# jasperlinthorst/reveal

Measured on AMD Instinct MI355X. Metric: Mbp/s indexed+MUM-anchored (reveal rem), higher is better.
Workload: dtype int32

## Files before the change

include/reveal_amd.h:

```cpp
#ifndef REVEAL_AMD_H
#define REVEAL_AMD_H
#include <stdint.h>

#ifdef __cplusplus
extern "C" {
#endif

typedef struct rv_index rv_index;

const char *rv_last_error(void);
int  rv_abi_version(void);
int  rv_sa_bits(void);
int  rv_device_count(void);

rv_index *rv_new(int device);
void rv_free(rv_index *h);

int rv_add_sample(rv_index *h);
int rv_add_sequence(rv_index *h, const char *seq, int64_t len, int64_t *begin, int64_t *end);
int rv_reset(rv_index *h);
int rv_reserve_text(rv_index *h, int64_t bytes);
int64_t rv_n(const rv_index *h);
int rv_nsamples(const rv_index *h);
int rv_nnodes(const rv_index *h);
// ... 32 lines not shown
int rv_sub_nodes(rv_index *h, int s, int64_t *begin_end );
int rv_sub_mums(rv_index *h, int s, uint32_t *l, int32_t *n, int64_t *off, uint16_t *so, int64_t *pos);
int64_t rv_sub_array(rv_index *h, int s, int which, void *out, int64_t cap);
int rv_sub_split(rv_index *h, int s, uint32_t l, int nsp, const int64_t *sp,
                 const int64_t *lead, int nlead, const int64_t *trail, int ntrail,
                 const int64_t *match, int nmatch, const int64_t *rest, int nrest);
int rv_frontier_commit(rv_index *h, int32_t *children);
int rv_align_end(rv_index *h);

typedef struct {
    int64_t steps;
    int64_t splits;
    int64_t anchored_bp;
    int32_t levels;
    int32_t maxdepth;
    int64_t scanned_ranks;
    double  t_scan, t_host, t_split, t_bubble;
} rv_align_stats;
int rv_align_builtin(rv_index *h, int minl, int minn, rv_align_stats *st);

int rv_align_builtin_until(rv_index *h, int minl, int minn, int stop_subs, rv_align_stats *st);
int rv_align_builtin_resume(rv_index *h, rv_align_stats *st);
int rv_align_builtin_continue(rv_index *h, int stop_subs, rv_align_stats *st);
int rv_frontier_counts(rv_index *h, int64_t *out);
int rv_frontier_export(rv_index *h, int64_t *meta, int64_t *node_first, int64_t *nodes);
int64_t rv_frontier_pack(rv_index *h, const int32_t *subs, int k, void *sa, void *lcp, void *bwt, int on_device);
int rv_frontier_import(rv_index *h, int minl, int minn, uint32_t maxlcp, int level, int nsubs, const int64_t *meta,
                       const int64_t *node_first, const int64_t *nodes, int64_t m,
                       const void *sa, const void *lcp, const void *bwt, int on_device);
int64_t rv_frontier_seeds_export(rv_index *h, const int32_t *subs, int k, int64_t *out, int64_t cap);
int rv_frontier_seeds_import(rv_index *h, int nsubs, const int64_t *words, int64_t nwords);
uint32_t rv_maxlcp(const rv_index *h);
int rv_cascade_info(const rv_index *h, int64_t *out);
const char *rv_cascade_why(const rv_index *h);
int64_t rv_anchor_count(rv_index *h, int64_t *members);
int rv_fetch_anchors(rv_index *h, uint32_t *l, int64_t *off, int64_t *pos);
int rv_set_result_buffers(rv_index *h, uint32_t *l, int64_t l_cap, int64_t *off, int64_t off_cap, int64_t *pos, int64_t pos_cap);
typedef struct {
    int64_t  key, n;
    int32_t  depth, nsamples, nnodes, picked;
    int64_t  nmums;
    uint32_t l; int32_t mn;
    int64_t  sp_min;
    uint64_t h_sa, h_lcp, h_mums;
} rv_trace;
int rv_set_trace(rv_index *h, int on);
int rv_set_preselect(rv_index *h, int64_t maxmums);
int rv_set_option(rv_index *h, const char *name, int64_t value);
int rv_get_option(rv_index *h, const char *name, int64_t *value);
int rv_set_launch_trace(int on);
int rv_option_count(void);
const char *rv_option_name(int k);
int64_t rv_trace_count(rv_index *h);
int rv_fetch_trace(rv_index *h, rv_trace *out, int64_t cap);

typedef struct rv_subindex rv_subindex;
rv_index *rv_clone(rv_index *h);
rv_subindex *rv_sx_main(rv_index *h);
rv_subindex *rv_sx_copy(rv_subindex *x);
void rv_sx_free(rv_subindex *x);
int rv_sx_info(const rv_subindex *x, rv_sub *out);
int rv_sx_nodes(const rv_subindex *x, int64_t *begin_end);
int64_t rv_sx_array(rv_subindex *x, int which, void *out, int64_t cap);
int64_t rv_sx_scan(rv_subindex *x, int minl, int minn, int64_t *members);
int rv_sx_fetch(rv_subindex *x, uint32_t *l, int32_t *n, int64_t *off, uint16_t *so, int64_t *pos);
int rv_sx_split(rv_subindex *x, const int64_t *lead, int nlead, const int64_t *trail, int ntrail,
// ... 103 lines not shown
```

reveal_amd/_index.py:

```python
import ctypes
import mmap
import os
import sys
import numpy as np

from . import _lib
from ._lib import RV_T, RV_SA, RV_SAI, RV_LCP, RV_SO, RV_NSEP


def _page_array(count, dtype):
    nbytes = max(int(count), 1) * np.dtype(dtype).itemsize
    m = mmap.mmap(-1, (nbytes + mmap.PAGESIZE - 1) // mmap.PAGESIZE * mmap.PAGESIZE)
    return np.frombuffer(m, dtype=dtype, count=max(int(count), 1))


def _pairs(iv, sa64):
    a = np.ascontiguousarray(np.array([(int(b), int(e)) for b, e in iv], dtype=np.int64).reshape(-1, 2))
    return a, len(a)


_OPTION_DEFAULTS = {}


def make_index_type(sa64, error):
# ... 544 lines not shown
            na = dll.rv_anchor_count(h, ctypes.byref(mem))
            c = self._result_buffers_free()
            if c is not None and len(c[0]) >= max(na, 1) and len(c[1]) >= na + 1 and len(c[2]) >= max(mem.value, 1):
                l, off, pos = c
            else:
                dll.rv_set_result_buffers(h, None, 0, None, 0, None, 0)
                if os.environ.get("RV_RESULT_BUFS", "") == "heap":
                    l = np.empty(max(na, 1), dtype=np.uint32); off = np.empty(na + 1, dtype=np.int64); pos = np.empty(max(mem.value, 1), dtype=np.int64)
                else:
                    l = _page_array(max(na, 1), np.uint32); off = _page_array(na + 1, np.int64); pos = _page_array(max(mem.value, 1), np.int64)
                self.__dict__["_res_bufs"] = (l, off, pos)
            c = None
            off[0] = 0
            if dll.rv_fetch_anchors(h, l.ctypes.data, off.ctypes.data, pos.ctypes.data) != 0:
                self._fail()
            tr = None
            if trace:
                nt = dll.rv_trace_count(h)
                tr = np.zeros(max(nt, 1), dtype=_lib.TRACE_DTYPE)
                if dll.rv_fetch_trace(h, tr.ctypes.data, len(tr)) != 0:
                    self._fail()
                tr = tr[:nt]
            stats = {f[0]: getattr(st, f[0]) for f in _lib.RvAlignStats._fields_}
            return dict(stats=stats, anchors=(l[:na], off[:na + 1], pos[:mem.value]), trace=tr)

        @property
        def maxlcp(self):
            return int(self._dll.rv_maxlcp(self._h))

        def cascade_info(self):
            o = np.zeros(8, dtype=np.int64)
            self._dll.rv_cascade_info(self._h, o.ctypes.data)
            return dict(done=bool(o[0]), levels=int(o[1]), matches=int(o[2]), witnesses=int(o[3]), subindices=int(o[4]), undecided=int(o[5]), rebuilt_ranks=int(o[6]), decided_from_witnesses=int(o[7]),
                        why=(self._dll.rv_cascade_why(self._h) or b"").decode())

        def align_builtin_until(self, stop_subs, minl=20, minn=2, trace=False):
            if not self._constructed:
                raise error("Index not yet constructed, alignment stopped.")
            self._dll.rv_set_trace(self._h, 1 if trace else 0)
            self._offer_result_buffers()
            self._st = _lib.RvAlignStats()
            self._trace = bool(trace)
            r = self._dll.rv_align_builtin_until(self._h, int(minl), int(minn), int(stop_subs), ctypes.byref(self._st))
            if r < 0:
                self._fail()
            self._pending = r > 0
            return r

        def align_builtin_continue(self, stop_subs):
            if not getattr(self, "_pending", False):
                return 0
            self._offer_result_buffers()
            r = self._dll.rv_align_builtin_continue(self._h, int(stop_subs), ctypes.byref(self._st))
            if r < 0:
                self._fail()
            self._pending = r > 0
            return r

        def frontier(self):
            c = np.zeros(4, dtype=np.int64)
            if self._dll.rv_frontier_counts(self._h, c.ctypes.data) != 0:
                self._fail()
            ns, m, nn, level = (int(x) for x in c)
            meta = np.zeros((max(ns, 1), 6), dtype=np.int64); nf = np.zeros(ns + 1, dtype=np.int64); nodes = np.zeros((max(nn, 1), 2), dtype=np.int64)
            if self._dll.rv_frontier_export(self._h, meta.ctypes.data, nf.ctypes.data, nodes.ctypes.data) != 0:
                self._fail()
# ... 89 lines not shown
```

reveal_amd/_lib.py:

```python
import ctypes
import importlib.util
import os
import sys
import numpy as np

_HERE = os.path.dirname(os.path.abspath(__file__))

RV_T, RV_SA, RV_SAI, RV_LCP, RV_SO, RV_NSEP, RV_NODES = range(7)
K_SCAN_PAIR, K_SCAN_MULTI, K_SA_SORT, K_LCP, K_SPLIT, K_LABEL, K_BUBBLE, K_RADIX_SCATTER, K_RADIX_HIST, K_TEXT_ROUND, K_CASCADE, K_DIAG_TABLE, K_INIT_KEYS, K_PUBLISH = range(14)

c_i64p = ctypes.POINTER(ctypes.c_int64)
V = ctypes.c_void_p


class RvSub(ctypes.Structure):
    _fields_ = [("n", ctypes.c_int64), ("depth", ctypes.c_int32), ("nsamples", ctypes.c_int32),
                ("nnodes", ctypes.c_int32), ("parent", ctypes.c_int32), ("kind", ctypes.c_int32),
                ("reserved", ctypes.c_int32), ("nmums", ctypes.c_int64), ("nmembers", ctypes.c_int64)]


class RvAlignStats(ctypes.Structure):
    _fields_ = [("steps", ctypes.c_int64), ("splits", ctypes.c_int64), ("anchored_bp", ctypes.c_int64),
                ("levels", ctypes.c_int32), ("maxdepth", ctypes.c_int32), ("scanned_ranks", ctypes.c_int64),
                ("t_scan", ctypes.c_double), ("t_host", ctypes.c_double), ("t_split", ctypes.c_double),
# ... 23 lines not shown
    "rv_node_list": (_I, [V, V]),
    "rv_construct": (_I, [V, _I, ctypes.c_char_p, ctypes.c_char_p, _I]),
    "rv_upload": (_I, [V]),
    "rv_upload_again": (_I, [V]),
    "rv_get_array": (_L, [V, _I, V, _L]),
    "rv_getmums": (_L, [V, _I]),
    "rv_fetch_mums": (_I, [V, V, V, V, _L]),
    "rv_getmultimums": (_L, [V, _I, _I, _I, c_i64p]),
    "rv_fetch_multi": (_I, [V, V, V, V, V, V]),
    "rv_align_begin": (_I, [V, _I, _I]),
    "rv_frontier_size": (_I, [V]),
    "rv_frontier_scan": (_I, [V]),
    "rv_sub_skip_scan": (_I, [V, _I]),
    "rv_sub_info": (_I, [V, _I, ctypes.POINTER(RvSub)]),
    "rv_sub_nodes": (_I, [V, _I, V]),
    "rv_sub_mums": (_I, [V, _I, V, V, V, V, V]),
    "rv_sub_array": (_L, [V, _I, _I, V, _L]),
    "rv_sub_split": (_I, [V, _I, ctypes.c_uint32, _I, V, V, _I, V, _I, V, _I, V, _I]),
    "rv_frontier_commit": (_I, [V, V]),
    "rv_align_end": (_I, [V]),
    "rv_align_builtin": (_I, [V, _I, _I, ctypes.POINTER(RvAlignStats)]),
    "rv_align_builtin_until": (_I, [V, _I, _I, _I, ctypes.POINTER(RvAlignStats)]),
    "rv_align_builtin_resume": (_I, [V, ctypes.POINTER(RvAlignStats)]),
    "rv_align_builtin_continue": (_I, [V, _I, ctypes.POINTER(RvAlignStats)]),
    "rv_frontier_counts": (_I, [V, V]),
    "rv_frontier_export": (_I, [V, V, V, V]),
    "rv_frontier_pack": (_L, [V, V, _I, V, V, V, _I]),
    "rv_frontier_import": (_I, [V, _I, _I, ctypes.c_uint32, _I, _I, V, V, V, _L, V, V, V, _I]),
    "rv_frontier_seeds_export": (_L, [V, V, _I, V, _L]),
    "rv_frontier_seeds_import": (_I, [V, _I, V, _L]),
    "rv_maxlcp": (ctypes.c_uint32, [V]),
    "rv_cascade_info": (ctypes.c_int, [V, V]),
    "rv_cascade_why": (ctypes.c_char_p, [V]),
    "rv_anchor_count": (_L, [V, c_i64p]),
    "rv_fetch_anchors": (_I, [V, V, V, V]),
    "rv_set_result_buffers": (_I, [V, V, _L, V, _L, V, _L]),
    "rv_set_trace": (_I, [V, _I]),
    "rv_set_preselect": (_I, [V, _L]),
    "rv_set_option": (_I, [V, ctypes.c_char_p, _L]),
    "rv_set_launch_trace": (_I, [_I]),
    "rv_batch_new": (V, []),
    "rv_batch_add": (_I, [V, V]),
    "rv_batch_run": (_I, [V, _I, _I, _I, V, V]),
    "rv_batch_info": (_I, [V, V]),
    "rv_batch_free": (None, [V]),
    "rv_dev_alloc": (V, [_I, _L]),
    "rv_dev_free": (_I, [_I, V]),
    "rv_ipc_export": (_I, [_I, V, V]),
    "rv_ipc_open": (V, [_I, V]),
    "rv_ipc_close": (_I, [_I, V]),
    "rv_dev_copy": (_I, [_I, V, V, _L]),
    "rv_get_option": (_I, [V, ctypes.c_char_p, c_i64p]),
    "rv_option_count": (_I, []),
    "rv_option_name": (ctypes.c_char_p, [_I]),
    "rv_trace_count": (_L, [V]),
    "rv_fetch_trace": (_I, [V, V, _L]),
    "rv_clone": (V, [V]),
    "rv_sx_main": (V, [V]),
    "rv_sx_copy": (V, [V]),
    "rv_sx_free": (None, [V]),
    "rv_sx_info": (_I, [V, ctypes.POINTER(RvSub)]),
    "rv_sx_nodes": (_I, [V, V]),
    "rv_sx_array": (_L, [V, _I, V, _L]),
    "rv_sx_scan": (_L, [V, _I, _I, c_i64p]),
    "rv_sx_fetch": (_I, [V, V, V, V, V, V]),
    "rv_sx_split": (_I, [V, V, _I, V, _I, V, _I, V, _I, V]),
# ... 124 lines not shown
```

reveal_amd/csrc/rv_align.hip:

```cpp
#include "rv_index.h"
#include "rv_split.h"
#include "rv_decide.h"
static_assert(RV_TSUB_TILE == RV_SPLIT_TILE, "one tile -> sub-index table serves the split passes and the multi-sample picker");
#include "rv_leaf.h"
#include "rv_cascade.h"
#include <string.h>
#include <algorithm>
#include <chrono>
#include <thread>
#include <atomic>
#include "rv_graphrem.h"

namespace {

double now_s() {
    return std::chrono::duration<double>(std::chrono::steady_clock::now().time_since_epoch()).count();
}

u64 hash_step(u64 acc, u64 i, int64_t v) {
    u64 x = (u64)v + (i + 1) * 0x9E3779B97F4A7C15ULL;
    x ^= x >> 30; x *= 0xbf58476d1ce4e5b9ULL;
    x ^= x >> 27; x *= 0x94d049bb133111ebULL;
    x ^= x >> 31;
    return acc + x;
// ... 84 lines not shown
    Level lv, nx;
    Decisions dec;
    bool scanned = false;
    std::vector<uint8_t> skip_scan;
    bool full_only = false;
    const u32 *d_err = nullptr;
    std::vector<RvPairRec> recs;
    std::vector<u32> ml; std::vector<int32_t> mn; std::vector<int64_t> moff, mpos; std::vector<uint16_t> mso;
    std::vector<int64_t> mum_first, nmums;
    int picker = 0; rv_picker_args pargs{};
    struct SeedList {
        std::vector<u32> l; std::vector<int32_t> n; std::vector<int64_t> off; std::vector<uint16_t> so; std::vector<int64_t> pos, score;
        size_t size() const { return l.size(); }
        void clear() { l.clear(); n.clear(); off.assign(1, 0); so.clear(); pos.clear(); score.clear(); }
        void push(u32 l_, int32_t n_, const uint16_t *so_, const int64_t *pos_, int members, int64_t sc) {
            if (off.empty()) off.assign(1, 0);
            l.push_back(l_); n.push_back(n_); score.push_back(sc);
            so.insert(so.end(), so_, so_ + members); pos.insert(pos.end(), pos_, pos_ + members); off.push_back((int64_t)pos.size());
        }
    };
    std::vector<SeedList> seeds_cur, seeds_lead, seeds_trail;
    rv_graph *ggraph = nullptr;
    rv_graph *replay_graph = nullptr; RvReplayFeed *feed = nullptr; size_t fed = 0;
    std::vector<RvGraphIv> g_left, g_right, g_newleft, g_newright;
    RvGraphAlignOut g_out;
    int64_t picker_calls = 0, picker_seeded = 0, picker_ns = 0, picker_list_ns = 0, galign_ns = 0;
    int64_t presel = 0; bool presel_on = false;
    bool pick_filter = false;
    int64_t presel_d2h = 0;
    std::vector<int64_t> sel, sel_first, sel_tmp;
    DBuf dD, dTab, dTile, dList, dFlag, dPar, dDbg, scrSA, scrLCP, scrBWT;
    RvCascadeBufs cas;
    RvCascadeOut cas_out{};
    DBuf dPbReady; u32 pb_epoch = 0;
    DBuf dNextTsub;
    DBuf dTmin;
    HBuf hLeafRoots[2], hLeafOut;
    DBuf dLeaf, dLeafRoots[2];
    hipStream_t leaf_stream = nullptr, leaf_stream2 = nullptr;
    hipStream_t bub_stream = nullptr, bub_stream2 = nullptr;
    hipEvent_t ev_fork = nullptr, ev_join = nullptr, ev_join2 = nullptr;
    hipEvent_t ev_ready = nullptr, ev_leaf[RV_LEVEL_BUFS + 1] = {}, ev_roots[2] = {nullptr, nullptr};
    bool roots_inflight[2] = {false, false};
    bool flag_clean = false;
    DBuf dDec, dErr, dTab0;
    bool next_dev_ok = false, cur_dev_ok = false, early_done = false, early_bubble = false, use_leaf = false;
    int64_t par_min_cur = RV_BUBBLE_PAR_N;
    const sa_t *d_next_nodes = nullptr; const uint8_t *d_next_flags = nullptr;
    std::vector<sa_t> next_nodes; std::vector<uint8_t> next_flags;
    bool leaf_pending[RV_LEVEL_BUFS + 1] = {};
    size_t leaf_anchor_cap = 0, leaf_trace_cap = 0;
    std::vector<uint8_t> leaf_done;
    std::vector<RvLeafRoot> leaf_roots[2];
    Packer pk;
    std::vector<int> stamp; int epoch = 0;
    std::vector<sa_t> cb, ce, mb, me, cut_lo, cut_hi, mend_pos;
    std::vector<uint8_t> cc;
    std::vector<int> ctab_first, mtab_first, cut_first, mend_first, split_subs;
    std::vector<u32> sub_off_h;
    std::vector<int> tile_sub;
    std::vector<int64_t> mpre, sub_start, woff, toff, next_ss;
    const int64_t *d_next_ss = nullptr;
    const int *d_next_want = nullptr;
    const int *d_next_tsub = nullptr;
    std::vector<int> next_tsub;
    std::vector<u32> pick_l; std::vector<sa_t> pick_pos;
// ... 391 lines not shown
        d.child_n = t.child_n; d.child_base = t.child_base; d.sub_off = t.sub_off; d.expect_total = t.expect_total;
        d.err = a->dErr.as<u32>();
        d.kid = kid;
    };
    if (a->multi) {
        RvDecideMultiArgs d;
        outputs(d);
        d.W = W; d.minl = a->minl; d.minn = a->minn;
        d.nodes = a->d_next_nodes; d.want = a->d_next_want;
        d.pick_l = h->ws.misc[13].as<u32>(); d.pick_pos = h->ws.misc[7].as<sa_t>();
        d.cand_count = h->ws.misc[1].as<u32>() + RV_MULTI_REGIONS * 64;
        d.cand_cap = (u32)std::min<size_t>(h->ws.misc[8].cap / RV_MULTI_CAND_BYTES / RV_MULTI_REGIONS, 0xffffffffu);
        RV_TRY(rv_decide_multi_launch(h->ws, d));
    } else {
        RvDecideArgs d;
        outputs(d);
        d.nodes = a->d_next_nodes; d.flags = a->d_next_flags; d.picks = h->hscan.as<RvPairRec>();
        d.ovf_cap = (u32)std::min<size_t>(h->ws.misc[4].cap / sizeof(RvPairRec), 0xffffffffu);
        RV_TRY(rv_decide_launch(h->ws, d));
    }
    RvLabelTabs lt; RvSplitArgs sa;
    split_args(h, t, nxt, lt, sa);
    int64_t biggest = 0;
    for (int s2 = 0; s2 < ns; s2++) biggest = std::max<int64_t>(biggest, lv.n[(size_t)s2]);
    if (biggest > a->par_min_cur) RV_TRY(tmin_preset(h, sa));
    int id = h->prof.begin(q, RV_K_SPLIT, (double)m * (2 * (sizeof(sa_t) + sizeof(lcp_t) + 2)) + (double)m * (sizeof(sa_t) + sizeof(lcp_t) + 1));
    RV_TRY(rv_split_launch(h->ws, cur_sa(h), cur_lcp(h), a->dD.as<uint8_t>(), cur_bwt(h), m, lt, sa, 1));
    h->prof.end(q, id);
    a->early_done = true;
    a->early_bubble = false;
    const bool all_classes = a->multi || ns > 4096;
    if (biggest <= a->par_min_cur && !h->ws.opt.no_early_bubble &&
        (a->multi || (!h->ws.opt.bubble_lds_always && (!all_classes || h->ws.opt.early_bubble_many)))) {
        RV_TRY(rv_lower_ranges_launch(h->ws, h->dT.as<uint8_t>(), t.mb, t.me, W * ns));
        RV_TRY(bubble_flags(h, m));
        RvBubbleArgs ba;
        memset(&ba, 0, sizeof ba);
        ba.flag = a->dFlag.as<uint8_t>();
        ba.SA = sa.SA_out; ba.LCP = sa.LCP_out; ba.BWT = sa.BWT_out; ba.SAi = sa.SAi; ba.cut_lo = t.cut_lo; ba.cut_hi = t.cut_hi; ba.err = a->dErr.as<u32>();
        id = h->prof.begin(q, RV_K_BUBBLE, 0.0);
        if (!all_classes) {
            RV_TRY(rv_bubble_children_dev_launch(h->ws, ba, kid, ns, a->par_min_cur));
        } else {
            RV_TRY(bubble_fork(h, true, true, true));
            Workspace wl, wk; wl.stream = a->bub_stream; wk.stream = a->bub_stream2;
            RV_TRY(rv_bubble_children_dev_classes_launch(wl, wk, ba, kid, ns, a->par_min_cur));
            RV_TRY(bubble_join(h, true, true));
        }
        h->prof.end(q, id);
        a->early_bubble = true;
    }
    return 0;
}

static int level_hook(rv_index *h) {
    Align *a = h->al;
    if (a->hook_early) RV_TRY(early_split(h));
    if (a->leaf_launch_due) RV_TRY(leaf_launch(h));
    return 0;
}

static void build_preselection(Align *a) {
    const int ns = a->lv.size();
    a->sel.clear(); a->sel_first.assign((size_t)ns + 1, 0);
    std::vector<int64_t> &tmp = a->sel_tmp;
    for (int s = 0; s < ns; s++) {
// ... 589 lines not shown
        a->d_next_tsub = a->dNextTsub.as<int>();
    }
    return 0;
}

static int commit_split(rv_index *h, const Commit &cm, RvSplitArgs &sa) {
    Align *a = h->al;
    hipStream_t q = h->ws.stream;
    const Level &lv = a->lv;
    const int nxt = cm.nxt;
    uint8_t *tb = a->dTab.as<uint8_t>();
    RV_TRY(split_reserve(h, nxt, lv.m, cm.m_next));
    RV_TRY(a->dList.reserve((size_t)a->woff.back() * 4 + 64));
    RV_TRY(leaf_wait(h, nxt));
    if (h->ws.opt.bubble_parent_scratch && !a->descs.empty()) RV_TRY(leaf_wait(h, a->level == 0 ? RV_LEVEL_BUFS : a->cur));
    SplitTabs t;
    t.sub_start = (const int64_t *)(tb + cm.o_ss); t.tile_sub = (const int *)(tb + cm.o_tsub);
    t.ctab_first = (int *)(tb + cm.o_ctf); t.mtab_first = (int *)(tb + cm.o_mtf); t.cut_first = (int *)(tb + cm.o_cf); t.mend_first = (int *)(tb + cm.o_mf);
    t.cb = (sa_t *)(tb + cm.o_cb); t.ce = (sa_t *)(tb + cm.o_ce); t.cc = tb + cm.o_cc; t.mb = (sa_t *)(tb + cm.o_mb); t.me = (sa_t *)(tb + cm.o_me);
    t.cut_lo = (sa_t *)(tb + cm.o_clo); t.cut_hi = (sa_t *)(tb + cm.o_chi); t.mend_pos = (sa_t *)(tb + cm.o_mp);
    t.child_n = (u32 *)(tb + cm.o_cn); t.child_base = (u32 *)(tb + cm.o_cbase); t.sub_off = (u32 *)(tb + cm.o_suboff); t.expect_total = (u32 *)(tb + cm.o_expect);
    t.total = (u32 *)(tb + cm.o_total);
    t.nmatch = (int)a->mb.size();
    RvLabelTabs lt;
    split_args(h, t, nxt, lt, sa);
    sa.mend_all = a->dec.host_lists ? 1 : 0;
    int id = a->early_done ? -1 : h->prof.begin(q, RV_K_SPLIT, (double)lv.m * (2 * (sizeof(sa_t) + sizeof(lcp_t) + 2)) + (double)cm.m_next * (sizeof(sa_t) + sizeof(lcp_t) + 1));
    if (!a->early_done) {
        if (!a->descs.empty()) RV_TRY(tmin_preset(h, sa));
        RV_TRY(rv_split_launch(h->ws, cur_sa(h), cur_lcp(h), a->dD.as<uint8_t>(), cur_bwt(h), lv.m, lt, sa, (int)a->split_subs.size()));
    }
    h->prof.end(q, id);
    if (!a->early_bubble) {
        if (lt.nmatch > 256 && a->mpre.back() / lt.nmatch <= 512) RV_TRY(rv_lower_ranges_launch(h->ws, h->dT.as<uint8_t>(), lt.mbegin, lt.mend, lt.nmatch));
        else RV_TRY(rv_lower_launch(h->ws, h->dT.as<uint8_t>(), lt.mbegin, lt.mend, (const int64_t *)(tb + cm.o_mpre), lt.nmatch, a->mpre.back()));
    }
    return 0;
}

static int commit_bubble(rv_index *h, const Commit &cm, const RvSplitArgs &sa) {
    Align *a = h->al;
    hipStream_t q = h->ws.stream;
    uint8_t *tb = a->dTab.as<uint8_t>();
    const int64_t m_next = cm.m_next;
    if (a->descs.empty() && a->kids_small.empty() && a->kids_big.empty() && a->kids_lds.empty()) return 0;
    RvBubbleArgs ba;
    ba.desc = (const RvBubbleDesc *)(tb + cm.o_desc); ba.woff = (const int64_t *)(tb + cm.o_woff);
    ba.cnt = (u32 *)(tb + cm.o_bcnt); ba.list = a->dList.as<u32>();
    RV_TRY(bubble_flags(h, m_next));
    ba.flag = a->dFlag.as<uint8_t>();
    ba.SA = sa.SA_out; ba.LCP = sa.LCP_out; ba.BWT = sa.BWT_out; ba.SAi = sa.SAi; ba.cut_lo = sa.cut_lo; ba.cut_hi = sa.cut_hi; ba.err = sa.err;
    ba.state = (RvBubbleState *)(tb + cm.o_bstate);
    ba.dbg = nullptr;
    if (h->ws.opt.level_log) { if (!a->dDbg.p) { RV_TRY(a->dDbg.reserve(64)); RV_HIP(hipMemsetAsync(a->dDbg.p, 0, 64, q)); } ba.dbg = a->dDbg.as<unsigned long long>(); }
    ba.scrSA = const_cast<sa_t *>(cur_sa(h)); ba.scrLCP = const_cast<lcp_t *>(cur_lcp(h)); ba.scrBWT = const_cast<uint8_t *>(cur_bwt(h));
    if (!a->descs.empty() && !h->ws.opt.bubble_parent_scratch) {
        RV_TRY(a->scrSA.reserve((size_t)(m_next + 64) * sizeof(sa_t)));
        RV_TRY(a->scrLCP.reserve((size_t)(m_next + 64) * sizeof(lcp_t)));
        RV_TRY(a->scrBWT.reserve((size_t)m_next + 64));
        ba.scrSA = a->scrSA.as<sa_t>(); ba.scrLCP = a->scrLCP.as<lcp_t>(); ba.scrBWT = a->scrBWT.as<uint8_t>();
    }
    if (!a->descs.empty()) {
        const size_t W = (size_t)a->woff.back() + 16, TT = (size_t)a->toff.back() + 16;
        RV_TRY(a->dPar.reserve(TT * 4 + W * (8 + 7 * 4 + sizeof(sa_t) + 2) + 256));
        uint8_t *pb = a->dPar.as<uint8_t>();
        ba.par.toff = (const int64_t *)(tb + cm.o_toff);
// ... 498 lines not shown
    }
    RV_HIP(hipStreamSynchronize(q));
    if (a->lv.size() > 0) {
        u32 err = 0;
        RV_HIP(hipMemcpy(&err, a->dErr.p, 4, hipMemcpyDeviceToHost));
        if (err & 1u) { rv_set_error("split: the intervals returned by graphalign do not partition the sub-index (child size mismatch)"); return -1; }
        if (err) { rv_set_error("device-side error %u in the level before the hand-off", err); return -1; }
    }
    return 0;
}

static void fill_offsets(int64_t *off, size_t na, int64_t base) {
    const int nt = na > ((size_t)1 << 18) ? 4 : 1;
    std::vector<std::thread> th;
    for (int t = 1; t < nt; t++) {
        const size_t lo = na / nt * t, hi = t + 1 == nt ? na : na / nt * (t + 1);
        th.emplace_back([=]() { for (size_t k = lo; k < hi; k++) off[k] = base + 2 * (int64_t)(k + 1); });
    }
    for (size_t k = 0; k < na / nt; k++) off[k] = base + 2 * (int64_t)(k + 1);
    for (auto &x : th) x.join();
}
static int builtin_finish(rv_index *h, rv_align_stats *out) {
    Align *a = h->al;
    hipStream_t q = h->ws.stream;
    h->rb.direct = false;
    if (a->use_leaf && a->running) {
        u32 *lf_counters = a->lf_counters; u32 *lf_l = a->lf_l; int64_t *lf_pos = a->lf_pos; rv_trace *lf_tr = a->lf_tr;
        RV_HIP(hipStreamSynchronize(a->leaf_stream));
        RV_HIP(hipStreamSynchronize(a->leaf_stream2));
        for (int k = 0; k <= RV_LEVEL_BUFS; k++) a->leaf_pending[k] = false;
        RV_TRY(a->hLeafOut.reserve(256));
        RV_HIP(hipMemcpyAsync(a->hLeafOut.p, lf_counters, 128, hipMemcpyDeviceToHost, q));
        RV_HIP(hipStreamSynchronize(q));
        u32 cnt[4]; unsigned long long stv[8];
        memcpy(cnt, a->hLeafOut.p, sizeof cnt); memcpy(stv, a->hLeafOut.as<uint8_t>() + 64, sizeof stv);
        if (h->ws.opt.leaf_prof)
            fprintf(stderr, "leaf: steps %llu splits %llu | cycles idle %llu scan %llu split %llu bubble %llu\n", stv[0], stv[1], stv[4], stv[5], stv[6], stv[7]);
        if (cnt[2]) { rv_set_error(cnt[2] & 4u ? "leaf kernel: recursion stack overflow" : "leaf kernel: a sub-index does not match its intervals"); return -1; }
        if (cnt[0] > a->leaf_anchor_cap || cnt[1] > a->leaf_trace_cap) { rv_set_error("leaf kernel: output buffer too small"); return -1; }
        a->leaf_na = 0;
        if (cnt[0]) {
            const size_t na = cnt[0];
            const size_t nl = a->an_l.size(), np = a->an_pos.size();
            rv_index::ResultBufs &rb = h->rb;
            rb.direct = rb.l && (int64_t)(nl + na) <= rb.l_cap && (int64_t)(nl + na + 1) <= rb.off_cap && (int64_t)(np + 2 * na) <= rb.pos_cap;
            int64_t *pp; u32 *pl;
            if (rb.direct) { pp = rb.pos + np; pl = rb.l + nl; }
            else { RV_TRY(a->hLeafOut.reserve(na * 20 + 64)); pp = a->hLeafOut.as<int64_t>(); pl = (u32 *)(pp + 2 * na); }
            RV_HIP(hipMemcpyAsync(pp, lf_pos, na * 16, hipMemcpyDeviceToHost, a->leaf_stream));
            RV_HIP(hipMemcpyAsync(pl, lf_l, na * 4, hipMemcpyDeviceToHost, a->leaf_stream));
            RV_TRY(rv_leaf_lower_launch(h->ws, h->dT.as<uint8_t>(), lf_pos, lf_l, (u32)na));
            if (rb.direct) fill_offsets(rb.off + nl + 1, na, (int64_t)np);
            RV_HIP(hipStreamSynchronize(a->leaf_stream));
            RV_HIP(hipStreamSynchronize(q));
            a->leaf_na = na;
        }
        if (a->trace_on && cnt[1]) {
            const size_t at = a->trace.size();
            a->trace.resize(at + cnt[1]);
            RV_HIP(hipMemcpy(a->trace.data() + at, lf_tr, (size_t)cnt[1] * sizeof(rv_trace), hipMemcpyDeviceToHost));
        }
        a->st.steps += (int64_t)stv[0]; a->st.splits += (int64_t)stv[1]; a->st.anchored_bp += (int64_t)stv[2];
        if ((int64_t)stv[3] > a->st.maxdepth) a->st.maxdepth = (int32_t)stv[3];
    }
    a->running = false;
    if (out) *out = a->st;
    return 0;
}

static int install_frontier(rv_index *h, int level, int nsubs, const int64_t *meta, const int64_t *node_first, const int64_t *nodes, int64_t m,
                            const void *sa, const void *lcp, const void *bwt, int on_device);
static int builtin_cascade(rv_index *h) {
    Align *a = h->al;
    memset(&a->cas_out, 0, sizeof a->cas_out);
    if (a->trace_on || h->rc != 0 || h->n <= RV_LEAF_N || a->minl < 4 || h->ws.opt.no_cascade || a->picker != 0) return 0;
    const bool second_try = !a->multi && a->use_leaf && h->ws.opt.cascade_second == 2;
    auto interval_cascade = [&]() -> int {
        RvCascadeMultiOut mo;
        RV_TRY(rv_cascade_multi_run(h, a->cas, a->minl, &mo));
        a->cas_out.done = mo.done; a->cas_out.levels = mo.levels; a->cas_out.cands = mo.cands; a->cas_out.witnesses = mo.witnesses; a->cas_out.children = mo.children;
        a->cas_out.undecided = mo.undecided; a->cas_out.rebuilt_ranks = mo.rebuilt_ranks; a->cas_out.why = mo.why;
        if (!mo.done) return 0;
        const int k = h->nsamples;
        a->st.splits += (int64_t)mo.an_l.size(); a->st.steps += mo.steps; a->st.levels += mo.levels; a->st.scanned_ranks += h->n;
        if (mo.maxdepth > a->st.maxdepth) a->st.maxdepth = mo.maxdepth;
        h->main_arrays_freed = true;
        if (mo.undecided > 0) {
            RV_TRY(install_frontier(h, 1, (int)mo.undecided, mo.meta.data(), mo.node_first.data(), mo.nodes.data(), mo.rebuilt_ranks, mo.d_sa, mo.d_lcp, mo.d_bwt, 1));
        } else {
            a->lv.clear();
            a->level = 1;
        }
        {
            const size_t na = mo.an_l.size(), l0 = a->an_l.size(), p0 = a->an_pos.size(), o0 = a->an_off.size();
            a->an_l.insert(a->an_l.end(), mo.an_l.begin(), mo.an_l.end());
            a->an_pos.resize(p0 + na * (size_t)k);
            for (size_t x = 0; x < na * (size_t)k; x++) a->an_pos[p0 + x] = (int64_t)mo.an_pos[x];
            a->an_off.resize(o0 + na);
            for (size_t x = 0; x < na; x++) a->an_off[o0 + x] = (int64_t)(p0 + (x + 1) * (size_t)k);
            int64_t bp = 0;
            for (size_t x = 0; x < na; x++) bp += mo.an_l[x];
            a->st.anchored_bp += bp;
            (void)l0;
        }
        return 0;
    };
    if (a->multi || second_try) return interval_cascade();
    if (!a->use_leaf) return 0;
    RvCascadeIO io;
    io.anchor_count = a->lf_counters; io.anchor_cap = (u32)a->leaf_anchor_cap; io.anchor_l = a->lf_l; io.anchor_pos = a->lf_pos;
    io.stats = a->lf_stats; io.leaf_err = a->lf_counters + 2;
    io.stage_cap = (u32)h->ws.opt.leaf_acap;
    io.lvSA = &a->lvSA[0]; io.lvLCP = &a->lvLCP[0]; io.lvBWT = &a->lvBWT[0]; io.roots = &a->dLeafRoots[0];
    const int dmode = (int)h->ws.opt.cascade_danger;
    RV_TRY(rv_cascade_run(h, a->cas, io, a->minl, &a->cas_out, dmode == 2 ? 1 : 0, 0));
    if (!a->cas_out.done && a->cas_out.undecided > 0 && dmode == 1) {
        RV_HIP(hipMemsetAsync(a->dLeaf.p, 0, 256, h->ws.stream));
        RV_TRY(rv_cascade_run(h, a->cas, io, a->minl, &a->cas_out, 1, 1));
    }
    if (!a->cas_out.done) {
        RV_HIP(hipMemsetAsync(a->dLeaf.p, 0, 256, h->ws.stream));
        if (a->cas_out.undecided > 0 && !h->ws.opt.cascade_second_off) return interval_cascade();
        return 0;
    }
    a->st.levels += a->cas_out.levels;
    a->st.scanned_ranks += h->n;
    if (!a->cas.lin_rest.empty() && h->nodes.size() > 2) {
        std::vector<RvIntv> rest, gone;
        for (size_t k = 0; k + 1 < a->cas.lin_rest.size(); k += 2) rest.push_back({a->cas.lin_rest[k], a->cas.lin_rest[k + 1]});
        std::sort(rest.begin(), rest.end(), intv_less);
        for (const RvIntv &v : h->nodes) {
            if (v.end <= v.begin) continue;
            const auto it = std::lower_bound(rest.begin(), rest.end(), v, intv_less);
            if (it == rest.end() || it->begin != v.begin) gone.push_back(v);
        }
        RV_TRY(add_decision(h, 0, 0, nullptr, 0, gone.data(), (int)gone.size(), nullptr, 0, nullptr, 0, rest.data(), (int)rest.size()));
        a->dec.drop_lead = true;
        RV_TRY(rv_frontier_commit(h, nullptr));
        for (size_t s2 = 0; s2 < a->lv.depth.size(); s2++) a->lv.depth[s2] = a->cas.lin_rest_depth;
        return 0;
    }
    h->main_arrays_freed = true;
    a->level = 1;
    a->lv.clear();
    return 0;
}

int rv_cascade_info(const rv_index *h, int64_t *out) {
    for (int k = 0; k < 8; k++) out[k] = 0;
    if (!h->al) return 0;
    const RvCascadeOut &c = h->al->cas_out;
    out[0] = c.done ? 1 : 0; out[1] = c.levels; out[2] = c.cands; out[3] = c.witnesses; out[4] = c.children; out[5] = c.undecided; out[6] = c.rebuilt_ranks; out[7] = c.solved;
    return 0;
}

const char *rv_cascade_why(const rv_index *h) {
    if (!h->al || h->al->cas_out.done || !h->al->cas_out.why) return "";
    return h->al->cas_out.why;
}

int rv_align_builtin(rv_index *h, int minl, int minn, rv_align_stats *out) {
    RV_TRY(builtin_setup(h, minl, minn));
    Align *a = h->al;
    if (a->replay_graph && a->picker == 1) {
        a->feed = rv_replay_feed_start(a->replay_graph);
        a->fed = 0;
        a->replay_graph = nullptr;
        if (!a->feed) return -1;
    }
    int rc = builtin_cascade(h);
    if (rc == 0) rc = builtin_levels(h, 0);
    if (rc == 0) rc = builtin_finish(h, out);
    if (a->feed) {
        RvReplayFeed *f = a->feed; a->feed = nullptr;
        if (rc == 0) { if (rv_replay_feed_finish(f) != 0) return -1; }
        else { const std::string keep = rv_last_error(); (void)rv_replay_feed_finish(f); rv_set_error("%s", keep.c_str()); }
    }
    return rc;
}

int rv_align_builtin_until(rv_index *h, int minl, int minn, int stop_subs, rv_align_stats *out) {
    RV_TRY(builtin_setup(h, minl, minn));
    RV_TRY(builtin_cascade(h));
    RV_TRY(builtin_levels(h, stop_subs));
    Align *a = h->al;
    if (a->lv.size() == 0) { RV_TRY(builtin_finish(h, out)); return 0; }
    if (out) *out = a->st;
// ... 552 lines not shown
```

reveal_amd/csrc/rv_api.hip:

```cpp
#include "rv_index.h"
#include "rv_cascade.h"
#include <limits>
#include <stdarg.h>
#include <stdio.h>
#include <string.h>
#include <limits.h>
#include <algorithm>
#include <thread>

static thread_local char g_err[1024] = "";

void rv_set_error(const char *fmt, ...) {
    va_list ap;
    va_start(ap, fmt);
    vsnprintf(g_err, sizeof g_err, fmt, ap);
    va_end(ap);
}

static std::vector<rv_index *> &live_handles() { static std::vector<rv_index *> v; return v; }
std::mutex &rv_trim_mutex() { static std::mutex *m = new std::mutex(); return *m; }
bool rv_oom_trim() {
    size_t got = 0;
    bool log = false;
    int caller_dev = 0;
// ... 34 lines not shown
    if (nd <= 0) { rv_set_error("no HIP device visible: reveal_amd has no CPU fallback"); return nullptr; }
    if (device < 0 || device >= nd) { rv_set_error("device %d out of range (%d visible)", device, nd); return nullptr; }
    if (hipSetDevice(device) != hipSuccess) { rv_set_error("hipSetDevice(%d) failed", device); return nullptr; }
    hipDeviceProp_t prop;
    if (hipGetDeviceProperties(&prop, device) != hipSuccess) { rv_set_error("hipGetDeviceProperties failed"); return nullptr; }
    if (strncmp(prop.gcnArchName, "gfx950", 6) != 0) {
        rv_set_error("device %d is %s; this library is built for gfx950 (MI355X) only", device, prop.gcnArchName);
        return nullptr;
    }
    rv_index *h = new rv_index();
    h->device = device;
    if (rv_stream_get(&h->ws.stream) != hipSuccess) {
        rv_set_error("hipStreamCreate failed");
        delete h;
        return nullptr;
    }
    h->T.push_back('\0');
    h->ws.prof_ctx = &h->prof;
    h->ws.prof_begin_fn = [](void *c, hipStream_t st, int k, double b) { return ((RvProf *)c)->begin(st, k, b); };
    h->ws.prof_end_fn = [](void *c, hipStream_t st, int id) { ((RvProf *)c)->end(st, id); };
    { std::lock_guard<std::mutex> g(rv_trim_mutex()); live_handles().push_back(h); }
    return h;
}

void rv_free(rv_index *h) {
    if (!h) return;
    { std::lock_guard<std::mutex> g(rv_trim_mutex()); auto &v = live_handles(); v.erase(std::remove(v.begin(), v.end(), h), v.end()); }
    (void)hipSetDevice(h->device);
    if (h->ws.stream) (void)hipStreamSynchronize(h->ws.stream);
    h->rb.direct = false;
    (void)rv_set_result_buffers(h, nullptr, 0, nullptr, 0, nullptr, 0);
    rv_align_free(h);
    h->prof.release();
    h->dT.release(); h->dT0.release(); h->dSA.release(); h->dSAi.release(); h->dLCP.release(); h->dBWT.release(); h->dNsep.release();
    h->ws.release();
    h->hscan.release();
    for (auto &b : h->ps) b.release();
    h->hupload.release();
    if (h->ev_picks) { (void)hipEventDestroy(h->ev_picks); h->ev_picks = nullptr; }
    if (h->ws.stream) rv_stream_put(h->ws.stream);
    delete h;
}

int rv_set_option(rv_index *h, const char *name, int64_t value) {
    if (!h || !name) { rv_set_error("rv_set_option: null argument"); return -1; }
    int64_t *f = h->ws.opt.find(name);
    if (!f) { rv_set_error("rv_set_option: unknown option %s", name); return -1; }
    *f = value;
    return 0;
}
int rv_set_launch_trace(int on) {
    const int was = g_rv_launch_trace;
    g_rv_launch_trace = on != 0;
    return was;
}
int rv_get_option(rv_index *h, const char *name, int64_t *value) {
    if (!h || !name || !value) { rv_set_error("rv_get_option: null argument"); return -1; }
    const int64_t *f = h->ws.opt.find(name);
    if (!f) { rv_set_error("rv_get_option: unknown option %s", name); return -1; }
    *value = *f;
    return 0;
}
int rv_option_count(void) {
    int c = 0;
#define RV_X_(f, nm, def) c++;
    RV_OPTION_LIST(RV_X_)
#undef RV_X_
    return c;
}
const char *rv_option_name(int k) {
    static const char *const names[] = {
#define RV_X_(f, nm, def) nm,
        RV_OPTION_LIST(RV_X_)
#undef RV_X_
    };
    return k >= 0 && k < rv_option_count() ? names[k] : nullptr;
}

rv_index *rv_clone(rv_index *h) {
    if (!h->constructed || h->main_arrays_freed) { rv_set_error("Index not yet constructed."); return nullptr; }
    if (rv_need_sai(h)) return nullptr;
    rv_index *c = rv_new(h->device);
    if (!c) return nullptr;
    try { c->T = h->T; c->nsep = h->nsep; c->nodes = h->nodes; }
    catch (...) { rv_set_error("copy of the index: out of host memory"); rv_free(c); return nullptr; }
    if (c->T.size() != h->T.size()) { rv_free(c); return nullptr; }
    c->nsamples = h->nsamples; c->n = h->n; c->nT = h->nT; c->rc = h->rc;
    c->maxlcp = h->maxlcp; c->sa_stats = h->sa_stats; c->text_dirty = true;
    c->ws.opt = h->ws.opt;
    const int64_t n = h->n;
    hipStream_t q = c->ws.stream;
    bool ok = rv_upload(c) == 0;
    ok = ok && c->dT.reserve((size_t)n + 64) == 0 && c->dSA.reserve((size_t)(n + 64) * sizeof(sa_t)) == 0 && c->dSAi.reserve((size_t)(n + 64) * sizeof(sa_t)) == 0
            && c->dLCP.reserve((size_t)(n + 64) * sizeof(lcp_t)) == 0 && c->dBWT.reserve((size_t)n + 64) == 0 && c->dNsep.reserve((h->nsep.size() + 1) * sizeof(sa_t)) == 0;
    ok = ok && hipStreamSynchronize(h->ws.stream) == hipSuccess;
    ok = ok && hipMemcpyAsync(c->dT.p, h->dT.p, (size_t)n + 64, hipMemcpyDeviceToDevice, q) == hipSuccess;
    ok = ok && hipMemcpyAsync(c->dSA.p, h->dSA.p, (size_t)n * sizeof(sa_t), hipMemcpyDeviceToDevice, q) == hipSuccess;
    ok = ok && hipMemcpyAsync(c->dSAi.p, h->dSAi.p, (size_t)n * sizeof(sa_t), hipMemcpyDeviceToDevice, q) == hipSuccess;
    ok = ok && hipMemcpyAsync(c->dLCP.p, h->dLCP.p, (size_t)n * sizeof(lcp_t), hipMemcpyDeviceToDevice, q) == hipSuccess;
    ok = ok && hipMemcpyAsync(c->dBWT.p, h->dBWT.p, (size_t)n, hipMemcpyDeviceToDevice, q) == hipSuccess;
    ok = ok && hipMemcpyAsync(c->dNsep.p, h->dNsep.p, (h->nsep.size() + 1) * sizeof(sa_t), hipMemcpyDeviceToDevice, q) == hipSuccess;
    ok = ok && hipStreamSynchronize(q) == hipSuccess;
    if (!ok) { rv_set_error("copy of the index failed"); rv_free(c); return nullptr; }
    c->nsep_dev = h->nsep_dev;
    c->constructed = true; c->sai_valid = true;
    return c;
}

int rv_add_sample(rv_index *h) {
    if (h->nsamples > 0) h->nsep.push_back(h->n - 1);
    h->nsamples++;
    h->constructed = false; h->text_only = false;
    return 0;
}

int rv_add_sequence(rv_index *h, const char *seq, int64_t len, int64_t *begin, int64_t *end) {
    if (len < 0 || !seq) { rv_set_error("addsequence: bad sequence"); return -1; }
#ifndef RV_SA64
    if ((uint64_t)h->n + (uint64_t)(len + 1) + 1 > (uint64_t)INT_MAX) {
        rv_set_error("Total amount of sequence too large, use \"reveal <subcommand> --64\" to use 64 bit suffix arrays instead.");
        return -1;
    }
#endif
    const int64_t s = h->n;
    if ((size_t)(h->n + len + 2) > h->T.cap) (void)hipSetDevice(h->device);
    if (h->T.resize((size_t)(h->n + len + 2)) != 0) return -1;
    char *dst = h->T.data() + h->n;
    auto copy_check = [dst, seq](int64_t lo, int64_t hi) -> uint64_t {
        uint64_t acc = 0;
// ... 196 lines not shown
            used[slot] = true;
        }
        RV_HIP(hipStreamSynchronize(q));
    }
    RV_HIP(hipStreamSynchronize(q));
    h->text_dirty = false;
    return 0;
}

int rv_upload_again(rv_index *h) {
    h->text_dirty = true;
    return rv_upload(h);
}

int rv_construct(rv_index *h, int rc, const char *safile, const char *lcpfile, int cache) {
    RV_HIP(hipSetDevice(h->device));
    if (rc == 1) {
        if (h->nsep.empty()) { rv_set_error("construct(rc=1) needs at least two samples"); return -1; }
        h->rc = 1;
        revcomp(h->T.data() + h->nsep[0], h->n - h->nsep[0]);
        h->text_dirty = true;
    } else {
        h->rc = 0;
    }
    if (h->n == 0) { rv_set_error("No text to index."); return -1; }
    const int64_t n = h->n;
    if (n >= ((int64_t)1 << 32) - 2) { rv_set_error("index of %lld positions: this build carries ranks in 32 bits (n < 2^32 - 2)", (long long)n); return -1; }
    if (cache == 1) RV_TRY(write_raw(".reveal.t", h->T.data(), (size_t)n));
    if (h->al) (void)rv_align_end(h);
    h->nT = n;
    hipStream_t q = h->ws.stream;
    RV_TRY(rv_upload(h));
    RV_TRY(h->dT.reserve((size_t)n + 64));
    RV_HIP(hipMemcpyAsync(h->dT.p, h->dT0.p, (size_t)n + 64, hipMemcpyDeviceToDevice, q));
    RV_TRY(h->dSA.reserve((size_t)(n + 64) * sizeof(sa_t)));
    RV_TRY(h->dSAi.reserve((size_t)(n + 64) * sizeof(sa_t)));
    RV_TRY(h->dLCP.reserve((size_t)(n + 64) * sizeof(lcp_t)));
    RV_TRY(h->dBWT.reserve((size_t)n + 64));
    memset(&h->sa_stats, 0, sizeof h->sa_stats);
    RV_TRY(h->ws.misc[0].reserve(64));
    u32 *d_max = h->ws.misc[0].as<u32>();
    const sa_t side_sep = !h->nsep.empty() ? (sa_t)h->nsep[0] : std::numeric_limits<sa_t>::max();
    const bool lcp_from_file = lcpfile && lcpfile[0];
    bool lcp_done = false;
    SaScratchInUse in_use(h->ws);
    if (!safile || !safile[0]) {
        int id = h->prof.begin(q, RV_K_SA_SORT, 5.0 * (double)n);
        if (lcp_from_file) RV_TRY(rv_build_sa(h->ws, h->dT.as<uint8_t>(), n, h->dSA.as<sa_t>(), &h->sa_stats));
        else RV_TRY(rv_build_sa(h->ws, h->dT.as<uint8_t>(), n, h->dSA.as<sa_t>(), &h->sa_stats, h->dLCP.as<lcp_t>(), h->dBWT.as<uint8_t>(), side_sep, d_max, &lcp_done,
                                 h->nsep.data(), (int)h->nsep.size()));
        h->prof.end(q, id);
    } else {
        std::vector<sa_t> tmp((size_t)n);
        RV_TRY(read_raw(safile, tmp.data(), (size_t)n * sizeof(sa_t)));
        RV_HIP(hipMemcpyAsync(h->dSA.p, tmp.data(), (size_t)n * sizeof(sa_t), hipMemcpyHostToDevice, q));
        RV_HIP(hipStreamSynchronize(q));
    }
    h->sai_valid = false;
    if (safile && safile[0]) { RV_TRY(rv_build_inverse_checked(h->ws, h->dSA.as<sa_t>(), h->dSAi.as<sa_t>(), n)); h->sai_valid = true; }
    if (!lcp_from_file) {
        if (!lcp_done) {
            int id = h->prof.begin(q, RV_K_LCP, 13.0 * (double)n);
            RV_TRY(rv_build_lcp(h->ws, h->dT.as<uint8_t>(), h->dSA.as<sa_t>(), false, h->dLCP.as<lcp_t>(), n, d_max, h->dBWT.as<uint8_t>(), side_sep));
            h->prof.end(q, id);
        }
        RV_TRY(rv_read_back(h->ws, &h->maxlcp, d_max, 4));
    } else {
        std::vector<lcp_t> tmp((size_t)n);
        RV_TRY(read_raw(lcpfile, tmp.data(), (size_t)n * sizeof(lcp_t)));
        u32 mx = 0;
        for (int64_t i = 0; i < n; i++) if ((u32)tmp[(size_t)i] > mx) mx = (u32)tmp[(size_t)i];
        h->maxlcp = mx;
        RV_HIP(hipMemcpyAsync(h->dLCP.p, tmp.data(), (size_t)n * sizeof(lcp_t), hipMemcpyHostToDevice, q));
        RV_TRY(rv_build_bwt(h->ws, h->dT.as<uint8_t>(), h->dSA.as<sa_t>(), n, h->dBWT.as<uint8_t>(), side_sep));
        RV_HIP(hipStreamSynchronize(q));
    }
    if (cache == 1) {
        std::vector<sa_t> sa((size_t)n);
        std::vector<lcp_t> lc((size_t)n);
        RV_HIP(hipMemcpy(sa.data(), h->dSA.p, (size_t)n * sizeof(sa_t), hipMemcpyDeviceToHost));
        RV_HIP(hipMemcpy(lc.data(), h->dLCP.p, (size_t)n * sizeof(lcp_t), hipMemcpyDeviceToHost));
        RV_TRY(write_raw(".reveal.sa", sa.data(), (size_t)n * sizeof(sa_t)));
        RV_TRY(write_raw(".reveal.lcp", lc.data(), (size_t)n * sizeof(lcp_t)));
    }
    {
        if (h->nsep_dev != h->nsep || !h->dNsep.p) {
            std::vector<sa_t> ns(h->nsep.size() + 1, 0);
            for (size_t k = 0; k < h->nsep.size(); k++) ns[k] = (sa_t)h->nsep[k];
            RV_TRY(h->dNsep.reserve(ns.size() * sizeof(sa_t)));
            RV_HIP(hipMemcpy(h->dNsep.p, ns.data(), ns.size() * sizeof(sa_t), hipMemcpyHostToDevice));
            h->nsep_dev = h->nsep;
        }
    }
    h->constructed = true;
    h->main_arrays_freed = false;
    h->text_only = false;
    return 0;
}

int64_t rv_get_array(rv_index *h, int which, void *out, int64_t cap) {
    (void)hipSetDevice(h->device);
    const int64_t n = h->n;
    switch (which) {
    case RV_T:
        if (cap < n) { rv_set_error("buffer too small"); return -1; }
        if (h->constructed || h->text_only) {
            if (hipMemcpy(out, h->dT.p, (size_t)n, hipMemcpyDeviceToHost) != hipSuccess) { rv_set_error("D2H failed"); return -1; }
        } else {
            memcpy(out, h->T.data(), (size_t)n);
        }
        return n;
    case RV_SA: case RV_SAI: case RV_LCP: {
        if (!h->constructed || (which != RV_SAI && h->main_arrays_freed)) { rv_set_error("Index not yet constructed."); return -2; }
        if (which == RV_SAI && rv_need_sai(h)) return -2;
        if (cap < h->nT && which == RV_SAI) { rv_set_error("buffer too small"); return -1; }
        if (cap < n && which != RV_SAI) { rv_set_error("buffer too small"); return -1; }
        const void *src = which == RV_SA ? h->dSA.p : which == RV_SAI ? h->dSAi.p : h->dLCP.p;
        const size_t esz = which == RV_LCP ? sizeof(lcp_t) : sizeof(sa_t);
        const int64_t cnt = which == RV_SAI ? h->nT : n;
        (void)hipStreamSynchronize(h->ws.stream);
        if (hipMemcpy(out, src, (size_t)cnt * esz, hipMemcpyDeviceToHost) != hipSuccess) { rv_set_error("D2H failed"); return -1; }
        return cnt;
    }
    case RV_SO: {
        if (!h->constructed || h->nsamples <= 2) { rv_set_error("SO not available."); return -2; }
        if (cap < h->nT) { rv_set_error("buffer too small"); return -1; }
        uint16_t *so = (uint16_t *)out;
        int64_t j = 0;
        for (int i = 0; i < h->nsamples; i++) {
            const int64_t hi = (i == h->nsamples - 1) ? h->nT - 1 : h->nsep[(size_t)i];
            for (; j <= hi; j++) so[j] = (uint16_t)i;
        }
        return h->nT;
    }
    case RV_NSEP:
        if (cap < (int64_t)h->nsep.size()) { rv_set_error("buffer too small"); return -1; }
        for (size_t k = 0; k < h->nsep.size(); k++) ((int64_t *)out)[k] = h->nsep[k];
        return (int64_t)h->nsep.size();
    case RV_NODES:
        if (cap < (int64_t)h->nodes.size() * 2) { rv_set_error("buffer too small"); return -1; }
        for (size_t k = 0; k < h->nodes.size(); k++) { ((int64_t *)out)[2 * k] = h->nodes[k].begin; ((int64_t *)out)[2 * k + 1] = h->nodes[k].end; }
        return (int64_t)h->nodes.size() * 2;
    }
    rv_set_error("unknown array id %d", which);
    return -1;
}

}

int rv_need_sai(rv_index *h) {
    if (h->sai_valid) return 0;
    if (!h->constructed || h->main_arrays_freed) { rv_set_error("the inverse suffix array was not requested before align() consumed the main index"); return -1; }
    RV_HIP(hipSetDevice(h->device));
    RV_TRY(rv_build_inverse(h->ws, h->dSA.as<sa_t>(), h->dSAi.as<sa_t>(), h->n));
    h->sai_valid = true;
    return 0;
}

int rv_text_only(rv_index *h, u32 maxlcp) {
    RV_HIP(hipSetDevice(h->device));
    if (h->n == 0) { rv_set_error("No text to index."); return -1; }
    if (h->nsep.empty()) { rv_set_error("a worker index needs at least two samples"); return -1; }
    const int64_t n = h->n;
    hipStream_t q = h->ws.stream;
    h->rc = 0; h->nT = n;
    RV_TRY(rv_upload(h));
    RV_TRY(h->dT.reserve((size_t)n + 64));
    RV_HIP(hipMemcpyAsync(h->dT.p, h->dT0.p, (size_t)n + 64, hipMemcpyDeviceToDevice, q));
    RV_TRY(h->dSAi.reserve((size_t)(n + 64) * sizeof(sa_t)));
    std::vector<sa_t> ns(h->nsep.size() + 1, 0);
    for (size_t k = 0; k < h->nsep.size(); k++) ns[k] = (sa_t)h->nsep[k];
    RV_TRY(h->dNsep.reserve(ns.size() * sizeof(sa_t)));
    RV_HIP(hipMemcpy(h->dNsep.p, ns.data(), ns.size() * sizeof(sa_t), hipMemcpyHostToDevice));
    h->nsep_dev = h->nsep;
    RV_HIP(hipStreamSynchronize(q));
    h->maxlcp = maxlcp;
    h->constructed = false; h->main_arrays_freed = true; h->text_only = true; h->sai_valid = false;
    return 0;
}

namespace {
__global__ __launch_bounds__(256) void k_ps_keys(const RvPairRec *__restrict__ recs, u32 total, const int64_t *__restrict__ ss, int ns, u64 *__restrict__ keys, u32 *__restrict__ vals) {
    const u32 i = blockIdx.x * 256u + threadIdx.x;
    if (i >= total) return;
    const int64_t r = (int64_t)recs[i].rank;
    int lo = 0, hi = ns;
    while (hi - lo > 1) { const int mid = (lo + hi) >> 1; if (ss[mid] <= r) lo = mid; else hi = mid; }
    keys[i] = ((u64)(u32)lo << 32) | (u64)recs[i].l;
    vals[i] = i;
}
__global__ __launch_bounds__(256) void k_ps_mark(const u64 *__restrict__ skeys, const u32 *__restrict__ svals, u32 total, u32 presel, u32 *__restrict__ flag) {
    const u32 p = blockIdx.x * 256u + threadIdx.x;
    if (p >= total) return;
    const u64 next = ((skeys[p] >> 32) + 1ull) << 32;
    u32 lo = p, hi = total;
    while (hi - lo > 1) { const u32 mid = lo + ((hi - lo) >> 1); if (skeys[mid] < next) lo = mid; else hi = mid; }
    flag[svals[p]] = (hi - p <= presel) ? 1u : 0u;
}
__global__ __launch_bounds__(256) void k_ps_emit(const RvPairRec *__restrict__ recs, const u32 *__restrict__ flag, const u32 *__restrict__ off, u32 total, RvPairRec *__restrict__ out) {
    const u32 i = blockIdx.x * 256u + threadIdx.x;
    if (i < total && flag[i]) out[off[i]] = recs[i];
// ... 588 lines not shown
```

reveal_amd/csrc/rv_cascade.h:

```cpp
#pragma once
#include "rv_common.h"
#include <vector>

struct RvCascadeBufs {
    DBuf d[40];
    HBuf hstage, hstage2;
    u32 M = 0, NW = 0;
    u32 lin_roots = 0, lin_picks = 0, lin_nA = 0, lin_nB = 0;
    int64_t lin_steps = 0; int lin_maxdepth = 0; size_t lin_off[6] = {0, 0, 0, 0, 0, 0};
    std::vector<int64_t> lin_rest; int lin_rest_depth = 0;
    hipStream_t prio_stream = nullptr; hipEvent_t ev_in = nullptr, ev_out = nullptr;
    void release() {
        for (auto &b : d) b.release(); hstage.release(); hstage2.release();
        if (prio_stream) { (void)hipStreamDestroy(prio_stream); prio_stream = nullptr; }
        if (ev_in) { (void)hipEventDestroy(ev_in); ev_in = nullptr; }
        if (ev_out) { (void)hipEventDestroy(ev_out); ev_out = nullptr; }
    }
};

struct RvCascadeIO {
    u32 *anchor_count; u32 anchor_cap; u32 *anchor_l; int64_t *anchor_pos;
    unsigned long long *stats;
    u32 *leaf_err;
    u32 stage_cap;
    DBuf *lvSA, *lvLCP, *lvBWT, *roots;
};

struct RvCascadeOut {
    bool done;
    int levels;
    int64_t cands, witnesses, children, undecided, rebuilt_ranks;
    int64_t solved, unsolved;
    const char *why;
};

#define RV_CASM_K 16
struct RvCascadeMultiOut {
    bool done; int levels; int64_t cands, witnesses, children, undecided, rebuilt_ranks, steps; int maxdepth; const char *why;
    int64_t big, big_ranks;
    std::vector<u32> an_l; std::vector<int64_t> an_pos;
    std::vector<int64_t> meta, node_first, nodes;
    const void *d_sa, *d_lcp, *d_bwt;
};

struct rv_index;
struct RvBatchGroup;
RvBatchGroup *rv_batch_group_new(int device);
void rv_batch_group_begin(RvBatchGroup *g, int total);
void rv_batch_group_leave(RvBatchGroup *g);
void rv_batch_group_free(RvBatchGroup *g);
void rv_batch_group_info(const RvBatchGroup *g, int64_t *out);
int rv_cascade_multi_run(rv_index *h, RvCascadeBufs &cb, int minl, RvCascadeMultiOut *out);
int rv_cascade_run(rv_index *h, RvCascadeBufs &cb, const RvCascadeIO &io, int minl, RvCascadeOut *out, int danger = 0, int reuse = 0);
```

reveal_amd/csrc/rv_cascade.hip:

```cpp
#include "rv_index.h"
#include "rv_cascade.h"
#include "rv_leaf.h"
#include <algorithm>
#include <string.h>
#include <stdio.h>
#include <stdlib.h>
#include <chrono>

namespace {

constexpr int TB = 256;
constexpr u32 NONE = 0xFFFFFFFFu;
#ifdef RV_SA64
constexpr int KEY_SHIFT = 40;
#else
constexpr int KEY_SHIFT = 32;
#endif
constexpr u64 KEY_LOW = (1ull << KEY_SHIFT) - 1;

struct CasIv { sa_t a0, a1, b0, b1; };
struct CasRes { sa_t qa, qb; u32 ql, lead, trail, state; };
enum { C_NCHILD = 0, C_NUND = 1, C_NWIT = 2, C_ERR = 3, C_MAXN = 4, C_LO = 5, C_HI = 6, C_LEVELS = 7, C_NSOLVED = 8, C_NUNSOLVED = 9, C_NRETRY = 10, C_TICKET = 11 };

__device__ inline bool cas_cut(const CasIv &iv, int64_t pa, int64_t pb, int64_t len, int64_t minl, int64_t *qa, int64_t *qb, int64_t *ql) {
    const int64_t ka = (int64_t)iv.a0 - pa, kb = (int64_t)iv.b0 - pb;
    int64_t k = ka > kb ? ka : kb;
    k = k > 0 ? k : 0;
    const int64_t a = pa + k, b = pb + k;
    int64_t l = len - k;
    const int64_t ra = (int64_t)iv.a1 - a, rb = (int64_t)iv.b1 - b;
    l = l < ra ? l : ra;
    l = l < rb ? l : rb;
    *qa = a; *qb = b; *ql = l;
    return l >= minl;
}
__device__ inline u64 cas_key(int64_t qa, int64_t ql) { return ((u64)ql << KEY_SHIFT) | (KEY_LOW - (u64)qa); }

__device__ inline u64 shfl_up64(u64 v, int d) {
    const u32 lo = __shfl_up((u32)v, d, 64), hi = __shfl_up((u32)(v >> 32), d, 64);
    return ((u64)hi << 32) | lo;
}
__device__ inline void seg_atomic_max64(u64 *__restrict__ dst, u32 child, u64 val, bool active) {
    const int lane = threadIdx.x & 63;
    if (!active) { child = NONE; val = 0; }
    val = rv_wave_seg_max_u64(child, val);
    const u32 nc = __shfl_down(child, 1, 64);
    const bool last = lane == 63 || nc != child;
    if (active && last && val > dst[child]) atomicMax((unsigned long long *)&dst[child], (unsigned long long)val);
}
__device__ inline void seg_atomic_max32(u32 *__restrict__ dst, u32 child, u32 val, bool active) {
    const int lane = threadIdx.x & 63;
    if (!active) { child = NONE; val = 0; }
    val = rv_wave_seg_max_u32(child, val);
    const u32 nc = __shfl_down(child, 1, 64);
    const bool last = lane == 63 || nc != child;
// ... 501 lines not shown
                    iv[slot] = c; best[slot] = 0; wmax[slot] = 0; depth[slot] = dp + 1; res[slot] = nr;
                    if (danger) { dg.best[slot] = 0; dg.flag[slot] = 0; dg.ceil[slot] = 0; }
                    r.lead = slot;
                } else atomicOr(&counters[C_ERR], 1u);
                slot++;
            }
            if (trail) {
                if (slot < child_cap) {
                    CasIv c; c.a0 = (sa_t)((int64_t)r.qa + r.ql); c.a1 = p.a1; c.b0 = (sa_t)((int64_t)r.qb + r.ql); c.b1 = p.b1;
                    iv[slot] = c; best[slot] = 0; wmax[slot] = 0; depth[slot] = dp + 1; res[slot] = nr;
                    if (danger) { dg.best[slot] = 0; dg.flag[slot] = 0; dg.ceil[slot] = 0; }
                    r.trail = slot;
                } else atomicOr(&counters[C_ERR], 1u);
            }
            const u32 as = base_a + (u32)__popcll(b_split & lt);
            if (as < io.anchor_cap) { io.anchor_l[as] = r.ql; io.anchor_pos[2 * (size_t)as] = (int64_t)r.qa; io.anchor_pos[2 * (size_t)as + 1] = (int64_t)r.qb; }
            else atomicOr(&counters[C_ERR], 4u);
            r.state = 1;
        } else {
            r.state = 2;
        }
        if (in) res[id] = r;
        if (und) {
            und_list[base_u + (u32)__popcll(b_und & lt)] = id;
            if ((u64)(la + lb) > (u64)leaf_n) atomicMax(&counters[C_MAXN], (u32)((la + lb) > 0xFFFFFFFFll ? 0xFFFFFFFFll : (la + lb)));
        }
        __syncthreads();
    }
    if (threadIdx.x == 0) {
        __threadfence();
        if (atomicAdd(&counters[C_TICKET], 1u) == gridDim.x - 1) {
            if (hi > lo) counters[C_LEVELS]++;
            counters[C_LO] = hi; counters[C_HI] = atomicAdd(&counters[C_NCHILD], 0u);
            counters[C_TICKET] = 0;
        }
    }
}
__global__ __launch_bounds__(TB) void k_cas_stats(const u32 *__restrict__ counters, const int32_t *__restrict__ depth, RvCascadeIO io) {
    __shared__ unsigned long long s_bp[TB / 64];
    __shared__ u32 s_md[TB / 64];
    const u32 nchild = counters[C_NCHILD], na = *io.anchor_count;
    unsigned long long bp = 0; u32 md = 0;
    for (u32 i = blockIdx.x * TB + threadIdx.x; i < na; i += gridDim.x * TB) bp += io.anchor_l[i];
    for (u32 i = blockIdx.x * TB + threadIdx.x; i < nchild; i += gridDim.x * TB) { const u32 d = (u32)depth[i]; md = d > md ? d : md; }
#pragma unroll
    for (int d = 32; d >= 1; d >>= 1) {
        bp += ((unsigned long long)(u32)__shfl_down((u32)(bp >> 32), d, 64) << 32) + (unsigned long long)(u32)__shfl_down((u32)bp, d, 64);
        const u32 om = __shfl_down(md, d, 64);
        md = om > md ? om : md;
    }
    if ((threadIdx.x & 63) == 0) { s_bp[threadIdx.x >> 6] = bp; s_md[threadIdx.x >> 6] = md; }
    __syncthreads();
    if (threadIdx.x == 0) {
        for (int k = 1; k < TB / 64; k++) { bp += s_bp[k]; md = s_md[k] > md ? s_md[k] : md; }
        if (bp) atomicAdd(&io.stats[2], bp);
        if (md) atomicMax(&io.stats[3], (unsigned long long)md);
        if (blockIdx.x == 0) { atomicAdd(&io.stats[0], (unsigned long long)(nchild - counters[C_NUND] - counters[C_NRETRY])); atomicAdd(&io.stats[1], (unsigned long long)na); }
    }
}

__global__ __launch_bounds__(TB) void k_cas_sizes(const u32 *__restrict__ und_list, u32 U, const CasIv *__restrict__ iv, u64 *__restrict__ sizes) {
    const u32 u = blockIdx.x * TB + threadIdx.x;
    if (u < U) { const CasIv p = iv[und_list[u]]; sizes[u] = (u64)(((int64_t)p.a1 - p.a0) + ((int64_t)p.b1 - p.b0)); }
    if (u == U) sizes[u] = 0;
}
__global__ __launch_bounds__(TB) void k_cas_roots(const u32 *__restrict__ und_list, u32 U, const CasIv *__restrict__ iv, const int32_t *__restrict__ depth,
// ... 187 lines not shown
    if (nLiveA + nLiveB > 0) {
        if (stalled || (nLiveA && nLiveB && chain_wmax() >= minl)) {
            for (size_t c = 0; c < nA; c++) if (liveA[c]) { cb.lin_rest.push_back(CA[c].begin); cb.lin_rest.push_back(CA[c].end); }
            for (size_t c = 0; c < nB; c++) if (liveB[c]) { cb.lin_rest.push_back(CB[c].begin); cb.lin_rest.push_back(CB[c].end); }
        } else { steps++; maxdepth = depth; }
    }
    const u32 R = (u32)roots.size(), P = (u32)anl.size();
    RV_TRY(broots.reserve((size_t)std::max<u32>(R, 1) * sizeof(CasIv))); RV_TRY(bdepth.reserve((size_t)std::max<u32>(R, 1) * 4));
    const size_t tab_bytes = (nA + nB) * (sizeof(sa_t) + 4) + (size_t)P * 8 + 64;
    RV_TRY(btabs.reserve(tab_bytes + 64)); RV_TRY(banch.reserve((size_t)P * (4 + 16) + 64));
    std::vector<uint8_t> stage(tab_bytes + 64, 0);
    size_t o = 0;
    auto put = [&](const void *src, size_t bytes) { memcpy(stage.data() + o, src, bytes); const size_t at = o; o += (bytes + 15) / 16 * 16; return at; };
    std::vector<sa_t> bA(nA), bB(nB);
    for (size_t c = 0; c < nA; c++) bA[c] = (sa_t)CA[c].begin;
    for (size_t c = 0; c < nB; c++) bB[c] = (sa_t)CB[c].begin;
    stage.resize((nA + nB) * (sizeof(sa_t) + 4) + (size_t)P * 8 + 16 * 8 + 64);
    const size_t oA = put(bA.data(), nA * sizeof(sa_t)), oB = put(bB.data(), nB * sizeof(sa_t)), opA = put(pickA.data(), nA * 4), opB = put(pickB.data(), nB * 4),
                 oL = put(rootLead.data(), (size_t)P * 4), oT = put(rootTrail.data(), (size_t)P * 4);
    RV_TRY(btabs.reserve(o + 64));
    RV_HIP(hipMemcpyAsync(btabs.p, stage.data(), o, hipMemcpyHostToDevice, q));
    if (R) {
        RV_HIP(hipMemcpyAsync(broots.p, roots.data(), (size_t)R * sizeof(CasIv), hipMemcpyHostToDevice, q));
        RV_HIP(hipMemcpyAsync(bdepth.p, rdepth.data(), (size_t)R * 4, hipMemcpyHostToDevice, q));
    }
    RV_HIP(hipMemcpyAsync(banch.p, anp.data(), (size_t)P * 16, hipMemcpyHostToDevice, q));
    RV_HIP(hipMemcpyAsync((uint8_t *)banch.p + (size_t)P * 16, anl.data(), (size_t)P * 4, hipMemcpyHostToDevice, q));
    RV_HIP(hipStreamSynchronize(q));
    cb.lin_roots = R; cb.lin_picks = P; cb.lin_nA = (u32)nA; cb.lin_nB = (u32)nB; cb.lin_steps = steps; cb.lin_maxdepth = maxdepth;
    cb.lin_off[0] = oA; cb.lin_off[1] = oB; cb.lin_off[2] = opA; cb.lin_off[3] = opB; cb.lin_off[4] = oL; cb.lin_off[5] = oT;
    return 0;
}

int rv_cascade_run(rv_index *h, RvCascadeBufs &cb, const RvCascadeIO &io, int minl_in, RvCascadeOut *out, int danger, int reuse) {
    memset(out, 0, sizeof *out);
    out->done = false;
    Workspace &ws = h->ws;
    hipStream_t q = ws.stream;
    const int64_t n = h->n;
    const u32 minl = (u32)std::max(minl_in, 1);
    const bool verbose = (ws.opt.cascade_log != 0);
    double tp[6] = {0, 0, 0, 0, 0, 0};
    if (verbose) { (void)hipStreamSynchronize(q); tp[0] = cas_now(); }
#define GIVE_UP(msg) do { out->why = msg; if (verbose) fprintf(stderr, "cascade: gave up: %s\n", msg); return 0; } while (0)
    if (h->nsamples != 2 || h->nsep.size() != 1 || h->nodes.size() < 2) GIVE_UP("not two samples");
    std::vector<RvIntv> CA, CB;
    for (const RvIntv &v : h->nodes) if (v.end > v.begin) (v.begin < h->nsep[0] ? CA : CB).push_back(v);
    std::sort(CA.begin(), CA.end(), [](const RvIntv &x, const RvIntv &y) { return x.begin < y.begin; });
    std::sort(CB.begin(), CB.end(), [](const RvIntv &x, const RvIntv &y) { return x.begin < y.begin; });
    if (CA.empty() || CB.empty()) GIVE_UP("an empty sample");
    const bool chain = CA.size() > 1 || CB.size() > 1;
    if (chain && ws.opt.no_cascade_chain) GIVE_UP("several sequences per sample (switched off)");
    if (n >= ((int64_t)1 << 32) - 2) GIVE_UP("index above 2^32 positions");
#ifdef RV_SA64
    if ((u64)h->maxlcp >= (1ull << 24) || n >= ((int64_t)1 << 40)) GIVE_UP("bid word too narrow");
#endif
    CasIv root; root.a0 = root.a1 = root.b0 = root.b1 = 0;
    root.a0 = (sa_t)CA[0].begin; root.a1 = (sa_t)CA[0].end; root.b0 = (sa_t)CB[0].begin; root.b1 = (sa_t)CB[0].end;
    if (root.a0 >= root.a1 || root.b0 >= root.b1 || (int64_t)root.a1 > h->nsep[0] || (int64_t)root.b0 <= h->nsep[0]) GIVE_UP("an empty sample");

    const sa_t *SA = h->dSA.as<sa_t>(); const lcp_t *LCP = h->dLCP.as<lcp_t>(); const uint8_t *BWT = h->dBWT.as<uint8_t>();

    const int64_t ntile = ceil_div(n, RV_PAIR_TILE);
    DBuf &bcnt = ws.misc[14], &btab = ws.misc[2], &bslot = ws.misc[3], &bovf = ws.misc[4], &bout = ws.misc[5];
    if (bcnt.cap == 0) { RV_TRY(bcnt.reserve(64)); RV_HIP(hipMemsetAsync(bcnt.p, 0, 64, q)); }
    RV_TRY(btab.reserve((size_t)(ntile + 1) * 3 * sizeof(u32)));
    RV_TRY(bslot.reserve((size_t)ntile * RV_PAIR_SLOTS * sizeof(RvPairRec)));
// ... 161 lines not shown
        RV_HIP(hipMemcpyAsync(io.anchor_pos, cb.d[33].p, (size_t)P * 16, hipMemcpyDeviceToDevice, q));
        RV_HIP(hipMemcpyAsync(io.anchor_l, (const uint8_t *)cb.d[33].p + (size_t)P * 16, (size_t)P * 4, hipMemcpyDeviceToDevice, q));
        RV_HIP(hipMemcpyAsync(io.anchor_count, &cb.lin_picks, 4, hipMemcpyHostToDevice, q));
    }

    if (verbose) { (void)hipStreamSynchronize(q); tp[2] = cas_now(); }
    const unsigned agrid = (unsigned)(ceil_div((int64_t)M, TB * CAS_ITEMS) + ceil_div((int64_t)NW, TB * CAS_ITEMS));
    const int batch = std::max(1, (int)ws.opt.cascade_batch);
    int queued = 0;
    struct PrioScope {
        Workspace &w; hipStream_t home; RvCascadeBufs &cb; bool on = false;
        ~PrioScope() { leave(); }
        void leave() {
            if (!on) return;
            on = false;
            (void)hipEventRecord(cb.ev_out, w.stream);
            w.stream = home;
            (void)hipStreamWaitEvent(home, cb.ev_out, 0);
        }
    } prio{ws, q, cb};
    if (ws.opt.cascade_prio) {
        if (!cb.prio_stream) {
            int plo = 0, phi = 0;
            RV_HIP(hipDeviceGetStreamPriorityRange(&plo, &phi));
            RV_HIP(hipStreamCreateWithPriority(&cb.prio_stream, hipStreamNonBlocking, phi));
            RV_HIP(hipEventCreateWithFlags(&cb.ev_in, hipEventDisableTiming));
            RV_HIP(hipEventCreateWithFlags(&cb.ev_out, hipEventDisableTiming));
        }
        RV_HIP(hipEventRecord(cb.ev_in, q));
        RV_HIP(hipStreamWaitEvent(cb.prio_stream, cb.ev_in, 0));
        ws.stream = cb.prio_stream; prio.on = true;
        q = cb.prio_stream;
    }
    for (;;) {
        for (int b = 0; b < batch; b++, queued++) {
            hipLaunchKernelGGL(k_cas_assign, dim3(agrid), dim3(TB), 0, q, (const sa_t *)bpa.as<sa_t>(), (const sa_t *)bpb.as<sa_t>(), (const u32 *)blen.as<u32>(), bcc.as<u32>(), M,
                               wp, wv, bwc.as<u32>(), NW, (const CasIv *)biv.as<CasIv>(), (const CasRes *)bres.as<CasRes>(),
                               bbest.as<u64>(), bwm.as<u32>(), (int64_t)minl, queued == 0 ? 1 : 0, (const u64 *)((danger && NW) ? dg.ceil : nullptr));
            RV_LAUNCH_CHECK();
            hipLaunchKernelGGL(k_cas_winner, dim3((unsigned)ceil_div((int64_t)M, TB)), dim3(TB), 0, q, (const sa_t *)bpa.as<sa_t>(), (const sa_t *)bpb.as<sa_t>(),
                               (const u32 *)blen.as<u32>(), (const u32 *)bcc.as<u32>(), M, (const CasIv *)biv.as<CasIv>(), bres.as<CasRes>(), (const u64 *)bbest.as<u64>(), (int64_t)minl);
            RV_LAUNCH_CHECK();
            if (danger && NW) {
                const unsigned wb = (unsigned)ceil_div((int64_t)NW, TB);
                hipLaunchKernelGGL(k_cas_dmark, dim3(256), dim3(TB), 0, q, (const CasIv *)biv.as<CasIv>(), (const u64 *)bbest.as<u64>(), (const u32 *)bwm.as<u32>(), minl, (const u32 *)counters, dg);
                RV_LAUNCH_CHECK();
                hipLaunchKernelGGL(k_cas_dwalk, dim3(wb), dim3(TB), 0, q, wp, wv, (const u32 *)bwc.as<u32>(), NW, (const CasIv *)biv.as<CasIv>(), (const u64 *)bbest.as<u64>(),
                                   (const u32 *)bwm.as<u32>(), minl, dg);
                RV_LAUNCH_CHECK();
                if (dwalk_nmed) {
                    hipLaunchKernelGGL(k_cas_dwalk_blk, dim3((unsigned)dwalk_nmed), dim3(TB), 0, q, wp, wv, (const u32 *)bwc.as<u32>(), dwalk_boff, dwalk_mlist, dwalk_nmed,
                                       (const CasIv *)biv.as<CasIv>(), (const u64 *)bbest.as<u64>(), (const u32 *)bwm.as<u32>(), minl, dg);
                    RV_LAUNCH_CHECK();
                }
                hipLaunchKernelGGL(k_cas_dpick, dim3(wb), dim3(TB), 0, q, wp, wv, (const u32 *)bwc.as<u32>(), NW, (const CasIv *)biv.as<CasIv>(), (const CasRes *)bres.as<CasRes>(),
                                   (const u64 *)bbest.as<u64>(), (const u32 *)bwm.as<u32>(), minl, dg);
                RV_LAUNCH_CHECK();
                hipLaunchKernelGGL(k_cas_dwrite, dim3(wb), dim3(TB), 0, q, wp, (const u32 *)bwc.as<u32>(), NW, dg);
                RV_LAUNCH_CHECK();
            }
            hipLaunchKernelGGL(k_cas_decide, dim3(256), dim3(TB), 0, q, biv.as<CasIv>(), bbest.as<u64>(), bwm.as<u32>(), bdep.as<int32_t>(),
                               bres.as<CasRes>(), minl, counters, ccap, bund.as<u32>(), (u32)RV_LEAF_N, io, dg, (danger && NW) ? 1 : 0);
            RV_LAUNCH_CHECK();
        }
        RV_TRY(rv_read_back(ws, hc, counters, sizeof hc));
        if (hc[C_ERR] & ~5u) { rv_set_error("cascade: device error %u", hc[C_ERR]); return -1; }
        if (hc[C_ERR]) GIVE_UP("the cascade's tables are full");
        if (hc[C_MAXN] > (u32)RV_LEAF_N) break;
        if (hc[C_HI] == hc[C_LO]) break;
        if (queued > 1000000) { rv_set_error("cascade: no progress"); return -1; }
    }
    prio.leave(); q = ws.stream;
    const int level = (int)hc[C_LEVELS];
    const u32 hi = hc[C_NCHILD];
    if (verbose) tp[3] = cas_now();
    out->levels = level; out->children = hi; out->solved = hc[C_NSOLVED]; out->unsolved = hc[C_NUNSOLVED];
    const u32 U = hc[C_NUND];
    out->undecided = U;
    if (hc[C_MAXN] > (u32)RV_LEAF_N) {
        out->why = "an undecided sub-index above the leaf kernel's size";
        if (verbose) fprintf(stderr, "cascade%s: gave up: %s (%u ranks; %u levels, %u sub-indices, %u undecided, %u decided from witnesses, %u not)\n", danger ? " (second attempt)" : "", out->why, hc[C_MAXN], level, hi, U, hc[C_NSOLVED], hc[C_NUNSOLVED]);
        return 0;
    }
    hipLaunchKernelGGL(k_cas_stats, dim3(256), dim3(TB), 0, q, (const u32 *)counters, (const int32_t *)bdep.as<int32_t>(), io);
    RV_LAUNCH_CHECK();
    if (chain) {
        hipLaunchKernelGGL(k_cas_lineage_stats, dim3(1), dim3(64), 0, q, io.stats, (unsigned long long)cb.lin_steps, (unsigned long long)cb.lin_maxdepth);
        RV_LAUNCH_CHECK();
    }
    if (U > 0) {
        RV_TRY(bsz.reserve((size_t)(U + 1) * 8));
        u64 *sizes = bsz.as<u64>();
        hipLaunchKernelGGL(k_cas_sizes, dim3((unsigned)ceil_div((int64_t)U + 1, TB)), dim3(TB), 0, q, (const u32 *)bund.as<u32>(), U, (const CasIv *)biv.as<CasIv>(), sizes);
        RV_LAUNCH_CHECK();
        RV_TRY(rv_exclusive_sum_u64(ws, sizes, sizes, (int64_t)U + 1));
        u64 mu = 0;
        RV_TRY(rv_read_back(ws, &mu, sizes + U, 8));
        out->rebuilt_ranks = (int64_t)mu;
        RV_TRY(io.lvSA->reserve((size_t)(mu + 64) * sizeof(sa_t))); RV_TRY(io.lvLCP->reserve((size_t)(mu + 64) * sizeof(lcp_t))); RV_TRY(io.lvBWT->reserve((size_t)mu + 64));
        RV_TRY(io.roots->reserve((size_t)U * sizeof(RvLeafRoot)));
        RvLeafRoot *roots = io.roots->as<RvLeafRoot>();
        hipLaunchKernelGGL(k_cas_roots, dim3((unsigned)ceil_div((int64_t)U, TB)), dim3(TB), 0, q, (const u32 *)bund.as<u32>(), U, (const CasIv *)biv.as<CasIv>(),
                           (const int32_t *)bdep.as<int32_t>(), (const u64 *)sizes, roots);
        RV_LAUNCH_CHECK();
        DBuf &bord = cb.d[26];
        RV_TRY(bord.reserve((size_t)(mu + 64) * 2));
        hipLaunchKernelGGL(k_cas_rank, dim3(U, BN / TB), dim3(TB), 0, q, (const RvLeafRoot *)roots, (const uint8_t *)h->dT0.as<uint8_t>(), bord.as<uint16_t>());
        RV_LAUNCH_CHECK();
        hipLaunchKernelGGL(k_cas_emit, dim3(U, BN / TB), dim3(TB), 0, q, (const RvLeafRoot *)roots, (const uint8_t *)h->dT0.as<uint8_t>(), (const uint16_t *)bord.as<uint16_t>(),
                           io.lvSA->as<sa_t>(), io.lvLCP->as<lcp_t>(), io.lvBWT->as<uint8_t>(), h->nsep[0], (int64_t)root.a0, (int64_t)root.b0,
                           d_beginA, cb.lin_nA, d_beginB, cb.lin_nB);
        RV_LAUNCH_CHECK();
        RvLeafArgs la;
        la.roots = roots;
        la.SA = io.lvSA->as<sa_t>(); la.LCP = io.lvLCP->as<lcp_t>(); la.BWT = io.lvBWT->as<uint8_t>();
        la.nsep0 = h->nsep[0]; la.minl = minl_in; la.lcap = h->maxlcp;
        la.stage_cap = io.stage_cap;
        la.anchor_count = io.anchor_count; la.anchor_cap = io.anchor_cap; la.anchor_l = io.anchor_l; la.anchor_pos = io.anchor_pos;
        la.stats = io.stats;
        la.trace = 0; la.trace_count = io.anchor_count + 1; la.trace_cap = 0; la.trace_out = nullptr;
        la.err = io.leaf_err;
        RV_TRY(rv_leaf_launch(ws, la, (int)U));
    }
    if (verbose) {
        (void)hipStreamSynchronize(q); tp[4] = cas_now();
        fprintf(stderr, "cascade%s: %u matches, %u witnesses, %d levels, %u sub-indices, %u undecided (%lld ranks rebuilt), %lld decided from witnesses | ms: scan %.2f witnesses+sort %.2f levels %.2f rebuild+leaf %.2f\n",
                danger ? " (second attempt)" : "", M, NW, level, hi, U, (long long)out->rebuilt_ranks, (long long)out->solved, (tp[1] - tp[0]) * 1e3, (tp[2] - tp[1]) * 1e3, (tp[3] - tp[2]) * 1e3, (tp[4] - tp[3]) * 1e3);
    }
    out->done = true;
    return 0;
#undef GIVE_UP
}
```

reveal_amd/csrc/rv_cascade_multi.hip:

```cpp
#include "rv_index.h"
#include "rv_cascade.h"
#include "rv_leaf.h"
#include <algorithm>
#include <chrono>
#include <condition_variable>
#include <mutex>
#include <string.h>
#include <stdio.h>
#include <stdlib.h>

namespace {

constexpr int TB = 256;
constexpr u32 NONE = 0xFFFFFFFFu;
#ifdef RV_SA64
constexpr int KEY_SHIFT = 40;
#else
constexpr int KEY_SHIFT = 32;
#endif
constexpr u64 KEY_LOW = (1ull << KEY_SHIFT) - 1;
enum { C_NCHILD = 0, C_NUND = 1, C_NWIT = 2, C_ERR = 3, C_MAXN = 4, C_LO = 5, C_HI = 6, C_LEVELS = 7, C_NCAND = 8, C_NANCH = 9, C_STEPS = 10, C_MAXDEPTH = 11, C_TICKET = 12, C_BIGERR = 13, C_BIGTOT = 14  };

__device__ inline int cm_sample(const sa_t *__restrict__ nsep, int k, sa_t pos) {
    int s = 0;
// ... 1179 lines not shown
    u32 M = 0, rmaxc = 0;
    for (int r = 0; r < CM_REGIONS; r++) { hreg[CM_REGIONS + r] = M; M += hreg[r]; rmaxc = std::max(rmaxc, hreg[r]); }
    const u32 NW = hc[C_NWIT];
    out->cands = M; out->witnesses = NW;
    if (rmaxc > rcap) GIVE_UP("more full matches than the list holds");
    if (NW > wcap) GIVE_UP("too many repeat witnesses (a repetitive input)");
    if (M == 0) GIVE_UP("no full match at the top level");
    struct ProfSpan { Workspace &w; int id; ~ProfSpan() { w.prof_end(id); } } span{ws, ws.prof_begin(RV_K_CASCADE, 5.0 * (double)n)};
    RV_TRY(bk0.reserve((size_t)M * 8)); RV_TRY(bk1.reserve((size_t)M * 8)); RV_TRY(bv0.reserve((size_t)M * 4)); RV_TRY(bv1.reserve((size_t)M * 4));
    RV_TRY(bcl.reserve((size_t)M * 4)); RV_TRY(bcp.reserve((size_t)M * k * sizeof(sa_t))); RV_TRY(bcc.reserve((size_t)M * 4));
    {
        const unsigned mb = (unsigned)ceil_div((int64_t)M, TB);
        RV_HIP(hipMemcpyAsync(region_off, hreg + CM_REGIONS, CM_REGIONS * 4, hipMemcpyHostToDevice, q));
        RV_HIP(hipStreamSynchronize(q));
        hipLaunchKernelGGL(k_casm_keys, dim3((unsigned)std::max<int64_t>(1, ceil_div((int64_t)rmaxc, TB)), CM_REGIONS), dim3(TB), 0, q, (const sa_t *)bcp0.as<sa_t>(), k, rcap,
                           (const u32 *)region_cnt, (const u32 *)region_off, bk0.as<u64>(), bv0.as<u32>());
        RV_LAUNCH_CHECK();
        int in1 = 0;
        RV_TRY(rv_radix_sort_pairs<u32>(ws, bk0.as<u64>(), bv0.as<u32>(), bk1.as<u64>(), bv1.as<u32>(), (int64_t)M, 0, bitlen64m((u64)n), &in1));
        hipLaunchKernelGGL(k_casm_gather, dim3(mb), dim3(TB), 0, q, (const u32 *)bcl0.as<u32>(), (const sa_t *)bcp0.as<sa_t>(), (const u32 *)(in1 ? bv1.as<u32>() : bv0.as<u32>()), k, M,
                           bcl.as<u32>(), bcp.as<sa_t>(), bcc.as<u32>());
        RV_LAUNCH_CHECK();
    }
    const bool no_big = ws.opt.casm_no_big != 0;
    const int64_t big_min = (!no_big && ws.opt.casm_big_min >= 0 && ws.opt.casm_big_min < BN) ? ws.opt.casm_big_min : BN;
    auto too_big = [&](const u32 *c) {
        unsigned long long tot; memcpy(&tot, c + C_BIGTOT, 8);
        return no_big ? c[C_MAXN] > (u32)BN : ((int64_t)c[C_MAXN] > ws.opt.casm_big_root || (int64_t)tot > ws.opt.casm_big_total);
    };
    bool joint = false;
    RvBatchJob bjob;
    if (h->batch && !h->batch_settled) {
        h->batch_settled = true; ticket.settled = true;
        bjob.k = k; bjob.minl = minl; bjob.M = M; bjob.NW = std::min(NW, wcap); bjob.ccap = ccap; bjob.acap = acap;
        bjob.c_len = bcl.as<u32>(); bjob.c_pos = bcp.as<sa_t>(); bjob.w_pos = bwp.as<sa_t>(); bjob.w_val = bwv.as<u32>();
        bjob.nsep = nsep; bjob.dT = h->dT.as<uint8_t>();
        bjob.rb = rb; bjob.re = re;
        for (int s2 = 0; s2 + 1 < k; s2++) bjob.sep.push_back((sa_t)h->nsep[(size_t)s2]);
        bjob.big_min = big_min; bjob.big_root = ws.opt.casm_big_root; bjob.big_total = ws.opt.casm_big_total; bjob.no_big = no_big;
        bjob.stream = q;
        if (!cb.ev_in) RV_HIP(hipEventCreateWithFlags(&cb.ev_in, hipEventDisableTiming));
        bjob.ready = cb.ev_in;
        RV_HIP(hipEventRecord(cb.ev_in, q));
        batch_join(h->batch, &bjob, ws);
        joint = bjob.ok;
        if (joint) {
            RV_HIP(hipStreamWaitEvent(q, h->batch->ev_done, 0));
            t = h->batch->t;
            memset(hc, 0, sizeof hc);
            hc[C_LEVELS] = bjob.levels; hc[C_NCHILD] = bjob.nchild; hc[C_NUND] = (u32)bjob.und_id.size(); hc[C_NANCH] = bjob.na;
            hc[C_STEPS] = bjob.steps; hc[C_MAXDEPTH] = bjob.maxdepth; hc[C_MAXN] = bjob.maxn;
        }
    }
    if (!joint) {
    struct PrioScope {
        Workspace &w; hipStream_t home; RvCascadeBufs &cb; bool on = false;
        ~PrioScope() { leave(); }
        void leave() {
            if (!on) return;
            on = false;
            (void)hipEventRecord(cb.ev_out, w.stream);
            w.stream = home;
            (void)hipStreamWaitEvent(home, cb.ev_out, 0);
        }
    } prio{ws, q, cb};
    if (ws.opt.cascade_prio) {
// ... 38 lines not shown
    const u32 U = hc[C_NUND], NA = hc[C_NANCH];
    out->undecided = U;
    if (joint ? bjob.too_big : too_big(hc)) {
        out->why = "an undecided sub-index above the size that is rebuilt from the text";
        if (verbose) fprintf(stderr, "cascade (%d samples): gave up: %s (%u ranks; %u levels, %u sub-indices, %u undecided)\n", k, out->why, hc[C_MAXN], hc[C_LEVELS], hc[C_NCHILD], U);
        return 0;
    }
    if (U == 1 && hc[C_NCHILD] == 1 && n > (int64_t)BN)
        GIVE_UP("the index' longest match of all samples is no longer than its repeats");
    out->steps = hc[C_STEPS]; out->maxdepth = (int)hc[C_MAXDEPTH];
    const size_t b_anl = 0, b_anp = b_anl + (((size_t)NA * 4 + 15) & ~(size_t)15), b_rows = b_anp + (((size_t)NA * k * sizeof(sa_t) + 15) & ~(size_t)15);
    const size_t rowbytes = (size_t)U * 8 + (size_t)U * k * sizeof(sa_t) * 2;
    RV_TRY(cb.hstage.reserve(b_rows + rowbytes + 64));
    uint8_t *hs = cb.hstage.as<uint8_t>();
    const u32 *d_anl = joint ? bjob.d_anl : (const u32 *)banl.as<u32>();
    const sa_t *d_anp = joint ? bjob.d_anp : (const sa_t *)banp.as<sa_t>();
    if (joint) {
        if (NA) {
            RV_HIP(hipMemcpyAsync(hs + b_anl, d_anl, (size_t)NA * 4, hipMemcpyDeviceToHost, q));
            RV_HIP(hipMemcpyAsync(hs + b_anp, d_anp, (size_t)NA * k * sizeof(sa_t), hipMemcpyDeviceToHost, q));
        }
        if (U) {
            uint8_t *hr = hs + b_rows;
            memcpy(hr, bjob.und_id.data(), (size_t)U * 4); memcpy(hr + (size_t)U * 4, bjob.und_dep.data(), (size_t)U * 4);
            memcpy(hr + (size_t)U * 8, bjob.und_b.data(), (size_t)U * k * sizeof(sa_t)); memcpy(hr + (size_t)U * 8 + (size_t)U * k * sizeof(sa_t), bjob.und_e.data(), (size_t)U * k * sizeof(sa_t));
        }
    } else {
    if (NA) {
        RV_HIP(hipMemcpyAsync(hs + b_anl, banl.p, (size_t)NA * 4, hipMemcpyDeviceToHost, q));
        RV_HIP(hipMemcpyAsync(hs + b_anp, banp.p, (size_t)NA * k * sizeof(sa_t), hipMemcpyDeviceToHost, q));
        RV_TRY(bexp.reserve((size_t)NA * k * 4));
        hipLaunchKernelGGL(k_casm_expand_l, dim3((unsigned)ceil_div((int64_t)NA * k, TB)), dim3(TB), 0, q, (const u32 *)banl.as<u32>(), NA, k, bexp.as<u32>());
        RV_LAUNCH_CHECK();
        hipLaunchKernelGGL(k_casm_lower, dim3((unsigned)ceil_div((int64_t)NA * k * 64, TB)), dim3(TB), 0, q, h->dT.as<uint8_t>(), (const u32 *)bexp.as<u32>(), (const sa_t *)banp.as<sa_t>(), NA * (u32)k);
        RV_LAUNCH_CHECK();
    }
    if (U) {
        RV_TRY(brows.reserve(rowbytes + 64));
        u32 *d_id = brows.as<u32>(); int32_t *d_dep = (int32_t *)(d_id + U);
        sa_t *d_b = (sa_t *)(d_dep + U), *d_e = d_b + (size_t)U * k;
        hipLaunchKernelGGL(k_casm_rows, dim3((unsigned)ceil_div((int64_t)U * k, TB)), dim3(TB), 0, q, (const u32 *)bund.as<u32>(), U, t, k, d_id, d_dep, d_b, d_e);
        RV_LAUNCH_CHECK();
        RV_HIP(hipMemcpyAsync(hs + b_rows, brows.p, rowbytes, hipMemcpyDeviceToHost, q));
    }
    }
    if (NA || U) RV_HIP(hipStreamSynchronize(q));
    if (U) {
        const uint8_t *hrows = hs + b_rows;
        const u32 *r_id = (const u32 *)hrows; const int32_t *r_dep = (const int32_t *)(r_id + U);
        const sa_t *r_b = (const sa_t *)(r_dep + U), *r_e = r_b + (size_t)U * k;
        std::vector<u32> order(U);
        for (u32 x = 0; x < U; x++) order[x] = x;
        std::sort(order.begin(), order.end(), [&](u32 a, u32 b) { return r_id[a] < r_id[b]; });
        std::vector<u32> ids(U);
        std::vector<sa_t> hb((size_t)U * k), he((size_t)U * k);
        std::vector<int32_t> hd(U);
        for (u32 x = 0; x < U; x++) {
            const u32 o = order[x];
            ids[x] = r_id[o]; hd[x] = r_dep[o];
            for (int s2 = 0; s2 < k; s2++) { hb[(size_t)x * k + s2] = r_b[(size_t)o * k + s2]; he[(size_t)x * k + s2] = r_e[(size_t)o * k + s2]; }
        }
        std::vector<CmRoot> roots;
        std::vector<CmBig> bigs;
        int64_t m = 0, mL = 0;
        out->node_first.assign(1, 0);
        for (u32 x = 0; x < U; x++) {
// ... 35 lines not shown
        if (!roots.empty()) {
            if (h->ws.opt.casm_rank_count)
                hipLaunchKernelGGL(k_casm_rank, dim3((unsigned)slices.size()), dim3(TB), 0, q, (const CmRoot *)d_roots, (const CmSlice *)d_slices, t, k, (const uint8_t *)h->dT0.as<uint8_t>(), bexp.as<u32>());
            else
                hipLaunchKernelGGL(k_casm_rank_sort, dim3((unsigned)roots.size()), dim3(RK_TB), 0, q, (const CmRoot *)d_roots, t, k, (const uint8_t *)h->dT0.as<uint8_t>(), bexp.as<u32>());
            RV_LAUNCH_CHECK();
            hipLaunchKernelGGL(k_casm_emit, dim3((unsigned)slices.size()), dim3(TB), 0, q, (const CmRoot *)d_roots, (const CmSlice *)d_slices, t, k, (const uint8_t *)h->dT0.as<uint8_t>(),
                               (const u32 *)bexp.as<u32>(), bsa.as<sa_t>(), blcp.as<lcp_t>(), bbwt.as<uint8_t>(), h->nsep[0], d_rb);
            RV_LAUNCH_CHECK();
        }
        if (!bigs.empty()) {
            int rootbits = 1;
            while (((size_t)1 << rootbits) < bigs.size()) rootbits++;
            const int kb = std::min(6, (64 - rootbits) / 8);
            RV_TRY(bk0.reserve((size_t)(mL + 64) * 8)); RV_TRY(bk1.reserve((size_t)(mL + 64) * 8)); RV_TRY(bv0.reserve((size_t)(mL + 64) * 8)); RV_TRY(bv1.reserve((size_t)(mL + 64) * 8));
            hipLaunchKernelGGL(k_casmb_keys, dim3((unsigned)bslices.size()), dim3(TB), 0, q, (const CmBig *)d_bigs, (const CmSlice *)d_bslices, t, k, (const uint8_t *)h->dT0.as<uint8_t>(), kb,
                               bk0.as<u64>(), bv0.as<u64>());
            RV_LAUNCH_CHECK();
            int in1 = 0;
            RV_TRY(rv_radix_sort_pairs<u64>(ws, bk0.as<u64>(), bv0.as<u64>(), bk1.as<u64>(), bv1.as<u64>(), mL, 0, 8 * kb + rootbits, &in1));
            hipLaunchKernelGGL(k_casmb_place, dim3((unsigned)ceil_div(mL, TB)), dim3(TB), 0, q, (const CmBig *)d_bigs, (const u64 *)(in1 ? bk1.as<u64>() : bk0.as<u64>()),
                               (const u64 *)(in1 ? bv1.as<u64>() : bv0.as<u64>()), mL, kb, (const uint8_t *)h->dT0.as<uint8_t>(), bsa.as<sa_t>(), bexp.as<u32>(), counters + C_BIGERR);
            RV_LAUNCH_CHECK();
            hipLaunchKernelGGL(k_casmb_emit, dim3((unsigned)bslices.size()), dim3(TB), 0, q, (const CmBig *)d_bigs, (const CmSlice *)d_bslices, t, k, (const uint8_t *)h->dT0.as<uint8_t>(),
                               (const u32 *)bexp.as<u32>(), (const sa_t *)bsa.as<sa_t>(), blcp.as<lcp_t>(), bbwt.as<uint8_t>(), h->nsep[0], d_rb, (const u32 *)(counters + C_BIGERR));
            RV_LAUNCH_CHECK();
            u32 berr = 0;
            RV_TRY(rv_read_back(ws, &berr, counters + C_BIGERR, 4));
            if (berr) {
                if (NA) {
                    RV_TRY(bcl0.reserve((size_t)NA * k * 4));
                    hipLaunchKernelGGL(k_casm_expand_l, dim3((unsigned)ceil_div((int64_t)NA * k, TB)), dim3(TB), 0, q, d_anl, NA, k, bcl0.as<u32>());
                    RV_LAUNCH_CHECK();
                    hipLaunchKernelGGL(k_casm_unlower, dim3((unsigned)ceil_div((int64_t)NA * k * 64, TB)), dim3(TB), 0, q, h->dT.as<uint8_t>(), (const uint8_t *)h->dT0.as<uint8_t>(),
                                       (const u32 *)bcl0.as<u32>(), d_anp, NA * (u32)k);
                    RV_LAUNCH_CHECK();
                    RV_HIP(hipStreamSynchronize(q));
                }
                out->meta.clear(); out->node_first.clear(); out->nodes.clear(); out->rebuilt_ranks = 0;
                GIVE_UP("an undecided sub-index with more suffixes sharing their first bytes than are compared one by one");
            }
            out->big = (int64_t)bigs.size(); out->big_ranks = mL;
        }
        out->d_sa = bsa.p; out->d_lcp = blcp.p; out->d_bwt = bbwt.p;
    }
    if (NA) {
        const u32 *pl = (const u32 *)(hs + b_anl); const sa_t *pp = (const sa_t *)(hs + b_anp);
        out->an_l.assign(pl, pl + NA);
        out->an_pos.assign(pp, pp + (size_t)NA * k);
    }
    if (verbose) fprintf(stderr, "cascade (%d samples): %u full matches, %u witnesses, %d levels, %u sub-indices, %u anchors, %u undecided (%lld ranks rebuilt; %lld of them above %lld ranks: %lld)\n", k, M, NW,
                         out->levels, hc[C_NCHILD], NA, U, (long long)out->rebuilt_ranks, (long long)out->big, (long long)big_min, (long long)out->big_ranks);
    out->done = true;
    return 0;
#undef GIVE_UP
}
```

reveal_amd/csrc/rv_common.h:

```cpp
#pragma once
#include <mutex>
#include <thread>
#include <vector>
#include <utility>
#include <hip/hip_runtime.h>
#include <stdint.h>
#include <string.h>
#include <stddef.h>
#include <vector>
#include <string>

#ifdef RV_SA64
typedef int64_t  sa_t;
typedef uint32_t lcp_t;
#else
typedef int32_t  sa_t;
typedef int32_t  lcp_t;
#endif

typedef unsigned long long u64;
typedef unsigned int       u32;

void rv_set_error(const char *fmt, ...);

// ... 41 lines not shown
    X(lcp_by_rank, "RV_LCP_BY_RANK", 0) \
    X(no_tiny_sa, "RV_NO_TINY_SA", 0) \
    X(no_short_alphabet, "RV_NO_SHORT_ALPHABET", 0) \
    X(no_fused_lcp, "RV_NO_FUSED_LCP", 0) \
    X(no_diag, "RV_NO_DIAG", 0) \
    X(no_packed_text, "RV_NO_PACKED_TEXT", 0) \
    X(no_heads_fusion, "RV_NO_HEADS_FUSION", 0) \
    X(no_twin_collapse, "RV_NO_TWIN_COLLAPSE", 0) \
    X(no_far_twins, "RV_NO_FAR_TWINS", 0) \
    X(no_lcp_list, "RV_NO_LCP_LIST", 0) \
    X(no_text_jump, "RV_NO_TEXT_JUMP", 0) \
    X(far_table, "RV_FAR_TABLE", 0) \
    X(no_slow_class, "RV_NO_SLOW_CLASS", 0) \
    X(no_dwalk_blocks, "RV_NO_DWALK_BLOCKS", 0) \
    X(no_pub_twins, "RV_NO_PUB_TWINS", 0) \
    X(sa_no_text, "RV_SA_NO_TEXT", 0) \
    X(text_mode, "RV_TEXT_MODE", -1) \
    X(carry_ch, "RV_CARRY_CH", -1) \
    X(rs_bits, "RV_RS_BITS", 8) \
    X(rs_xcd, "RV_RS_XCD", 1) \
    X(rs_cnt16, "RV_RS_CNT16", 1) \
    X(rs_no_digit_bytes, "RV_RS_NO_DIGIT_BYTES", 0) \
    X(diag_table, "RV_DIAG_TABLE", -1) \
    X(no_cascade_chain, "RV_NO_CASCADE_CHAIN", 0) \
    X(casm_rank_count, "RV_CASM_RANK_COUNT", 0) \
    X(casm_big_min, "RV_CASM_BIG_MIN", -1) \
    X(casm_no_big, "RV_CASM_NO_BIG", 0) \
    X(casm_big_root, "RV_CASM_BIG_ROOT", 1 << 22) \
    X(casm_big_total, "RV_CASM_BIG_TOTAL", 1 << 26) \
    X(lock_any, "RV_LOCK_ANY", 0) \
    X(presel_dev_min, "RV_PRESEL_DEV_MIN", 65536) \
    X(scan_v1, "RV_SCAN_V1", 0) \
    X(pick_threads, "RV_PICK_THREADS", 0) \
    X(cascade_prio, "RV_CASCADE_PRIO", 0)
struct RvOptions {
#define RV_X_(f, name, def) int64_t f = def;
    RV_OPTION_LIST(RV_X_)
#undef RV_X_
    int64_t *find(const char *name) {
#define RV_X_(f, nm, def) if (strcmp(name, nm) == 0) return &f;
        RV_OPTION_LIST(RV_X_)
#undef RV_X_
        return nullptr;
    }
};
extern int g_rv_launch_trace;
static inline bool rv_launch_trace_on() { return g_rv_launch_trace != 0; }
#define RV_LAUNCH_CHECK()                                                                      \
    do {                                                                                       \
        RV_HIP(hipGetLastError());                                                             \
        if (rv_launch_trace_on()) {                                                            \
            fprintf(stderr, "launch %s:%d\n", __FILE__, __LINE__);                             \
            fflush(stderr);                                                                    \
            RV_HIP(hipDeviceSynchronize());                                                    \
        }                                                                                      \
    } while (0)

static inline int64_t ceil_div(int64_t a, int64_t b) { return (a + b - 1) / b; }

#define RV_BWT_SIDE 0x80u
#define RV_BWT_CHAR 0x7fu

#ifdef __HIPCC__
__device__ inline u32 rv_wave_min_u32(u32 v) {
    const int inf = -1;
    int x = (int)v, y;
#define RV_DPP_MIN(ctrl, rmask)                                                        \
// ... 167 lines not shown
    int prof_begin(int k, double bytes) { return prof_begin_fn ? prof_begin_fn(prof_ctx, stream, k, bytes) : -1; }
    void prof_end(int id) { if (prof_end_fn && id >= 0) prof_end_fn(prof_ctx, stream, id); }
    bool sa_in_use = false;
    size_t trim_sa() {
        size_t got = 0;
        for (auto &b : sa) { got += b.cap; b.release(); }
        return got;
    }
    void release() {
        hpin.release();
        if (ev_rb) { (void)hipEventDestroy(ev_rb); ev_rb = nullptr; }
        for (auto &b : scan_tmp) b.release();
        rs_hist.release(); rs_digits.release();
        for (auto &b : misc) b.release();
        for (auto &b : sa) b.release();
    }
};

std::mutex &rv_trim_mutex();
struct SaScratchInUse {
    Workspace &w; bool was;
    SaScratchInUse(Workspace &x) : w(x) { std::lock_guard<std::mutex> g(rv_trim_mutex()); was = w.sa_in_use; w.sa_in_use = true; }
    ~SaScratchInUse() { std::lock_guard<std::mutex> g(rv_trim_mutex()); w.sa_in_use = was; }
};

int rv_exclusive_sum_u32(Workspace &ws, const u32 *in, u32 *out, int64_t n);
int rv_exclusive_sum_u64(Workspace &ws, const u64 *in, u64 *out, int64_t n);
int rv_inclusive_max_u32(Workspace &ws, const u32 *in, u32 *out, int64_t n);
int rv_inclusive_max_u64(Workspace &ws, const u64 *in, u64 *out, int64_t n);

int rv_radix_passes(const Workspace &ws, int nbits);
template <class V>
int rv_radix_sort_pairs(Workspace &ws, u64 *k0, V *v0, u64 *k1, V *v1, int64_t n,
                        int bit_lo, int bit_hi, int *result_in_1);

int rv_read_back(Workspace &ws, void *dst, const void *dsrc, size_t bytes);

int rv_h2d_copy(Workspace &ws, const void *pinned_src, void *dst, size_t bytes);

struct RvSaStats {
    int    sigma, bits, k0;
    int    rounds;
    int64_t sorted_elems;
    int    radix_passes;
    int    diag_table;
    int64_t far_pairs;
    int64_t lcp_list;
};
int rv_build_sa(Workspace &ws, const uint8_t *T, int64_t n, sa_t *SA, RvSaStats *st,
                lcp_t *LCP = nullptr, uint8_t *BWT = nullptr, sa_t side_sep = 0, u32 *d_maxlcp = nullptr, bool *fused_done = nullptr,
                const int64_t *seps = nullptr, int nseps = 0);
int rv_build_inverse(Workspace &ws, const sa_t *SA, sa_t *SAi, int64_t n);
int rv_build_inverse_checked(Workspace &ws, const sa_t *SA, sa_t *SAi, int64_t n);
int rv_build_lcp(Workspace &ws, const uint8_t *T, const sa_t *SA, bool by_rank, lcp_t *LCP, int64_t n, u32 *d_maxlcp, uint8_t *BWT, sa_t side_sep);
int rv_build_bwt(Workspace &ws, const uint8_t *T, const sa_t *SA, int64_t n, uint8_t *BWT, sa_t side_sep);
```

reveal_amd/csrc/rv_construct.hip:

```cpp
#include "rv_common.h"
#include <string.h>
#include <stdlib.h>
#include <algorithm>
#include <limits>

#ifdef RV_SA64
typedef u64 sav_t;
#else
typedef u32 sav_t;
#endif

namespace {

constexpr int TB = 256;

__device__ inline u64 swar_eq(u64 v, uint8_t c) {
    const u64 t = v ^ (0x0101010101010101ull * c);
    return ~(((t & 0x7f7f7f7f7f7f7f7full) + 0x7f7f7f7f7f7f7f7full) | t) & 0x8080808080808080ull;
}
__device__ inline u64 swar_acgt(u64 v) { return swar_eq(v, 'A') | swar_eq(v, 'C') | swar_eq(v, 'G') | swar_eq(v, 'T'); }
__device__ inline u32 swar_code2(u64 v) {
    u64 y = ((v >> 1) ^ (v >> 2)) & 0x0303030303030303ull;
    y = (y | (y >> 6)) & 0x000f000f000f000full;
    y = (y | (y >> 12)) & 0x000000ff000000ffull;
// ... 299 lines not shown
#pragma unroll
            for (int r = 0; r < N; r++) lo[r] |= v[r] << sh;
            if (sh + kp.fb > 32) {
#pragma unroll
                for (int r = 0; r < N; r++) hi[r] |= v[r] >> (32 - sh);
            }
        }
    }
#pragma unroll
    for (int r = 0; r < N; r++) lo[r] |= ((u32)s_tf[p + r] * kp.lastmul) >> 20;
}
struct IkFetch { u32 raw0, raw1, pb; u64 ds, de, dl; };
__device__ inline u32 ik_text_word(const uint8_t *__restrict__ T, int64_t n, int64_t i, bool whole) {
    if (whole) return *reinterpret_cast<const u32 *>(T + i);
    u32 raw = 0;
    for (int r = 0; r < 4; r++) if (i + r < n) raw |= (u32)T[i + r] << (8 * r);
    return raw;
}
__device__ inline void ik_fetch(IkFetch &f, const uint8_t *__restrict__ T, int64_t n, const DiagBits &dg, bool hint, int64_t tile, bool aligned) {
    const int64_t base = tile * KEY_TILE;
    const bool whole = aligned && base + KEY_TILE + IK_AHEAD <= n;
    f.raw0 = ik_text_word(T, n, base + 4 * (int64_t)threadIdx.x, whole);
    f.raw1 = (int)threadIdx.x < IK_WORDS - TB ? ik_text_word(T, n, base + 4 * (int64_t)(TB + threadIdx.x), whole) : 0u;
    f.pb = (threadIdx.x == 0 && base > 0) ? (u32)T[base - 1] : (u32)'$';
    f.ds = ~0ull; f.de = ~0ull; f.dl = 0ull;
    if (hint && (int)threadIdx.x <= ND_WORDS) {
        const int64_t w = base / 64 - 1 + threadIdx.x, nwords = (n + 63) / 64;
        if (w >= 0 && w < nwords) { f.ds = dg.stop[w]; if (threadIdx.x) { f.de = dg.exc[w]; f.dl = dg.lt[w]; } }
    }
}
template <int G>
__global__ __launch_bounds__(TB) void k_init_keys(const uint8_t *__restrict__ T, int64_t n, const uint8_t *__restrict__ lut, int K, KeyPack kp,
                                                  u64 *__restrict__ keys, sav_t *__restrict__ vals, int pay, u32 stop0, u32 stop1,
                                                  KeyLayout ly, DiagBits dg, const u32 *__restrict__ tw_off , int64_t ntiles) {
    __shared__ u32 code32[IK_WORDS + 2];
    __shared__ u32 s_sc[IK_WORDS / 8 + 3];
    __shared__ uint8_t slut[256], sstop[256];
    __shared__ __align__(8) uint16_t s_tf[IK_FPOS];
    __shared__ u64 s_stop0[ND_WORDS + 1], s_exc[ND_WORDS], s_lt[ND_WORDS];
    __shared__ u64 s_tw[KEY_TILE / 64], s_keep[KEY_TILE / 64];
    __shared__ u32 s_kpre[KEY_TILE / 64 + 1];
    __shared__ uint16_t s_list[KEY_TILE];
    __shared__ u32 s_nm[64];
    __shared__ u32 s_raw32[KEY_TILE / 4 + 1];
    u64 *const s_stop = s_stop0 + 1;
    uint8_t *const s_raw = reinterpret_cast<uint8_t *>(s_raw32);
    const bool hint = ly.nd_bits > 0;
    const bool aligned = (reinterpret_cast<uintptr_t>(T) & 3u) == 0;
    auto tile_of = [&](int64_t x) { return x; };
    IkFetch fx;
    int64_t x = blockIdx.x;
    if (x < ntiles) ik_fetch(fx, T, n, dg, hint, tile_of(x), aligned);
    {
        const u32 c = lut[threadIdx.x];
        slut[threadIdx.x] = (uint8_t)c;
        sstop[threadIdx.x] = ((c == stop0) | (c == stop1) | (c == 0u)) ? 1 : 0;
        if (threadIdx.x < 2) code32[IK_WORDS + threadIdx.x] = 0u;
        if (threadIdx.x < 3) s_sc[IK_WORDS / 8 + threadIdx.x] = ~0u;
    }
    __syncthreads();
    const u32 at_none = (1u << ly.at_bits) - 1u;
    const int nd_none = hint ? (int)((1u << ly.nd_bits) - 1u) : 0;
    for (; x < ntiles; x += gridDim.x) {
    const int64_t tile = tile_of(x);
    const int64_t base = tile * KEY_TILE;
#pragma unroll
    for (int turn = 0; turn < 2; turn++) {
// ... 61 lines not shown
    __syncthreads();
    if (tw_off && base >= dg.D) {
        {
            const int t = (int)threadIdx.x, xw = t >> 4, b = (t & 15) * 4;
            const u64 kw = s_keep[xw];
            u32 nib = (u32)(kw >> b) & 15u;
            if (nib) {
                u32 at = s_kpre[xw] + (u32)__popcll(kw & ((1ull << b) - 1ull));
                while (nib) { s_list[at++] = (uint16_t)(4 * t + __builtin_ctz(nib)); nib &= nib - 1u; }
            }
        }
        __syncthreads();
        const u32 total = s_kpre[KEY_TILE / 64];
        const int64_t obase = dg.D + (int64_t)tw_off[tile];
        for (u32 j = threadIdx.x; j < total; j += TB) {
            const int k = (int)s_list[j];
            const int64_t i = base + k;
            u32 lo[1], hi[1];
            ik_fields<G, 1>(s_tf, k, kp, lo, hi);
            u64 key = ((u64)hi[0] << 32) | lo[0];
            if (pay) key |= ((u64)s_raw[k + 3] << 56) | ((u64)ik_first_stop(s_sc, k, K, at_none) << ly.at_shift);
            if (hint) {
                const int wi = k >> 6, sft = k & 63;
                const u64 A = s_stop[wi] >> sft;
                const u32 nx = s_nm[wi + 1];
                const bool has = A != 0ull;
                const int d = has ? __builtin_ctzll(A) : (int)(nx >> 2) - k;
                const int at = (sft + d) & 63;
                const u32 f = has ? ((u32)((s_lt[wi] >> at) & 1ull) << 1) | (u32)((s_exc[wi] >> at) & 1ull) : nx & 3u;
                const bool known = (d < nd_none) & !(f & 1u);
                key |= (u64)(known ? (u32)d | ((f >> 1) << ly.nd_bits) : (u32)nd_none) << ly.nd_shift;
            }
            keys[obase + j] = key; vals[obase + j] = (sav_t)i;
        }
    } else {
    constexpr int PER = KEY_TILE / TB;
    static_assert(PER == 4, "four bytes in front of four positions");
    const int k0 = (int)threadIdx.x * PER;
    const int64_t i0 = base + k0;
    u64 okey[PER];
    {
        u32 lo[PER], hi[PER];
        ik_fields<G, PER>(s_tf, k0, kp, lo, hi);
#pragma unroll
        for (int r = 0; r < PER; r++) okey[r] = ((u64)hi[r] << 32) | lo[r];
    }
    if (pay) {
        const u32 prevb = (u32)s_raw[k0 + 3] | (s_raw32[threadIdx.x + 1] << 8);
        const bool clear = K <= 29 && (__funnelshift_r(s_sc[k0 >> 5], s_sc[(k0 >> 5) + 1], (u32)(k0 & 31)) & ((1u << (K + 3)) - 1u)) == 0u;
#pragma unroll
        for (int r = 0; r < PER; r++)
            okey[r] |= ((u64)((prevb >> (8 * r)) & 0xffu) << 56) | ((u64)(clear ? at_none : ik_first_stop(s_sc, k0 + r, K, at_none)) << ly.at_shift);
    }
    if (hint) {
        const int wi = k0 >> 6, sft = k0 & 63;
        const u64 A = s_stop[wi] >> sft, E = s_exc[wi] >> sft, Lt = s_lt[wi] >> sft;
        const u32 nx = s_nm[wi + 1];
        const u64 Ah = A >> 3;
        const bool hh = Ah != 0ull;
        const int dh = hh ? 3 + __builtin_ctzll(Ah) : (int)(nx >> 2) - k0;
        const u32 fh = hh ? ((u32)((Lt >> (dh & 63)) & 1ull) << 1) | (u32)((E >> (dh & 63)) & 1ull) : nx & 3u;
        const u32 a3 = (u32)A & 7u, e3 = (u32)E & 7u, l3 = (u32)Lt & 7u;
#pragma unroll
        for (int r = 0; r < PER; r++) {
            const u32 t = a3 >> r;
            const int m = t ? r + __builtin_ctz(t) : dh;
            const u32 f = t ? (((l3 >> m) & 1u) << 1) | ((e3 >> m) & 1u) : fh;
            const int nd = m - r;
            const bool known = (nd < nd_none) & !(f & 1u);
            okey[r] |= (u64)(known ? (u32)nd | ((f >> 1) << ly.nd_bits) : (u32)nd_none) << ly.nd_shift;
        }
    }
    if (!tw_off || i0 + PER <= dg.D) {
        const u32 twn = tw_off ? (u32)(s_tw[k0 >> 6] >> (k0 & 63)) & 15u : 0u;
        sav_t oval[PER];
#pragma unroll
        for (int r = 0; r < PER; r++) oval[r] = (sav_t)(i0 + r) | (((twn >> r) & 1u) ? TW_FLAG : (sav_t)0);
        if (i0 + PER <= n) {
            ulonglong2 *kd2 = reinterpret_cast<ulonglong2 *>(keys + i0);
            kd2[0] = make_ulonglong2(okey[0], okey[1]); kd2[1] = make_ulonglong2(okey[2], okey[3]);
            if constexpr (sizeof(sav_t) == 4) *reinterpret_cast<uint4 *>(vals + i0) = make_uint4((u32)oval[0], (u32)oval[1], (u32)oval[2], (u32)oval[3]);
            else {
                ulonglong2 *vd2 = reinterpret_cast<ulonglong2 *>(vals + i0);
                vd2[0] = make_ulonglong2((u64)oval[0], (u64)oval[1]); vd2[1] = make_ulonglong2((u64)oval[2], (u64)oval[3]);
            }
        } else {
#pragma unroll
            for (int r = 0; r < PER; r++) if (i0 + r < n) { keys[i0 + r] = okey[r]; vals[i0 + r] = oval[r]; }
        }
    } else {
#pragma unroll
        for (int r = 0; r < PER; r++) {
            const int k = k0 + r;
            const int64_t i = base + k;
            if (i >= n) continue;
            const int xw = k >> 6, b = k & 63;
            const bool twin = (s_tw[xw] >> b) & 1ull;
            if (i < dg.D) { keys[i] = okey[r]; vals[i] = (sav_t)i | (twin ? TW_FLAG : (sav_t)0); }
            else if (!twin) {
                const int64_t o = dg.D + (int64_t)tw_off[tile] + s_kpre[xw] + (u32)__popcll(s_keep[xw] & ((b == 0) ? 0ull : (~0ull >> (64 - b))));
                keys[o] = okey[r]; vals[o] = (sav_t)i;
            }
        }
    }
    }
    __syncthreads();
    }
}

constexpr int HINT_K = 16;
struct KeyDigits { int K; u32 stop0, stop1; KeyPack kp; KeyLayout ly; int64_t D; int ns; int64_t sep[HINT_K - 1], Ds[HINT_K];
                   const int32_t *dtab; };
__device__ inline u32 key_first_stop(u64 key, const KeyDigits &kd) {
    const u32 none = (1u << kd.ly.at_bits) - 1u;
    const u32 at = (u32)(key >> kd.ly.at_shift) & none;
    return at == none ? 0xFFFFFFFFu : at;
}
__device__ inline bool key_hint(u64 key, const KeyDigits &kd, u32 *nd, bool *lt) {
    const u32 none = (1u << kd.ly.nd_bits) - 1u;
    const u32 v = (u32)(key >> kd.ly.nd_shift) & none;
    *nd = v; *lt = (key >> (kd.ly.nd_shift + kd.ly.nd_bits)) & 1ull;
    return kd.ly.nd_bits > 0 && v != none;
}
__device__ inline int hint_sample(const KeyDigits &kd, int64_t p) {
    int s = 0;
    for (int q = 0; q < kd.ns - 1; q++) s += kd.sep[q] < p ? 1 : 0;
    return s;
}
__device__ inline bool hint_cmp(const KeyDigits &kd, int64_t u, u64 key_u, int64_t v, u64 key_v, int *c, u32 *l, bool linked = false) {
    if (kd.ly.nd_bits <= 0) return false;
    const int su = hint_sample(kd, u), sv = hint_sample(kd, v);
    if (su >= HINT_K || sv >= HINT_K) return false;
    if (kd.dtab) {
        if (su == sv) return false;
// ... 1710 lines not shown
            const int64_t mseeds = nw * SEED_SLOTS;
            DBuf &bdt = ws.sa[25];
            const int64_t ndt = (n >> DT_SHIFT) + 1;
            SA_TRY(bdt.reserve((size_t)ndt * 8 + 64));
            int32_t *raw = bdt.as<int32_t>(), *tab = raw + ndt;
            const int did = ws.prof_begin(11 , (double)n + (double)mseeds * 12.0);
            hipLaunchKernelGGL(k_seed_sample, dim3((unsigned)ceil_div(nw, TB)), dim3(TB), 0, q, T, n, bk0.as<u64>(), bv0.as<sav_t>(), nw);
            SA_HIP(hipGetLastError());
            int sin1 = 0;
            SA_TRY(rv_radix_sort_pairs<sav_t>(ws, bk0.as<u64>(), bv0.as<sav_t>(), bk1.as<u64>(), bv1.as<sav_t>(), mseeds, 0, 40, &sin1));
            SA_HIP(hipMemsetAsync(raw, 0x7f, (size_t)ndt * 4, q));
            hipLaunchKernelGGL(k_seed_pairs, dim3((unsigned)ceil_div(mseeds, TB)), dim3(TB), 0, q, (const u64 *)(sin1 ? bk1.as<u64>() : bk0.as<u64>()),
                               (const sav_t *)(sin1 ? bv1.as<sav_t>() : bv0.as<sav_t>()), mseeds, kd.D, kd.D, raw);
            SA_HIP(hipGetLastError());
            hipLaunchKernelGGL(k_dtab_fill, dim3((unsigned)ceil_div(ndt, TB)), dim3(TB), 0, q, T, n, kd.D, kd.D, (const int32_t *)raw, tab, ndt);
            SA_HIP(hipGetLastError());
            DiagTab dt; dt.dtab = tab; dt.S2 = kd.D; dt.D = kd.D;
            hipLaunchKernelGGL(k_diag_bits_tab, dim3((unsigned)ceil_div(nw, TB)), dim3(TB), 0, q, T, n, dt, ws.sa[20].as<u64>(), ws.sa[21].as<u64>(), ws.sa[22].as<u64>(), nw);
            SA_HIP(hipGetLastError());
            ws.prof_end(did);
            u32 kept_tab = 0;
            SA_TRY(count_kept(1, &kept_tab));
            if (dt_mode == 1 || (int64_t)kept_tab * 5 < (int64_t)kept * 4) { kept = kept_tab; kd.dtab = tab; dg.tab = 1; }
            else {
                hipLaunchKernelGGL(k_diag_bits, dim3((unsigned)ceil_div(nw, TB)), dim3(TB), 0, q, T, n, dsm, ws.sa[20].as<u64>(), ws.sa[21].as<u64>(), ws.sa[22].as<u64>(), nw);
                SA_HIP(hipGetLastError());
                SA_TRY(count_kept(0, &kept));
            }
        }
        nsort = kd.D + (int64_t)kept;
        tw_off = tc;
        s.diag_table = dg.tab;
    }
    {
        const int64_t iktiles = ceil_div(n, KEY_TILE);
        const dim3 ig((unsigned)std::min<int64_t>(iktiles, 256 * 8));
#define RV_IK_(G) hipLaunchKernelGGL(k_init_keys<G>, ig, dim3(TB), 0, q, T, n, d_lut.as<uint8_t>(), K, kp, bk0.as<u64>(), bv0.as<sav_t>(), fused ? 1 : 0, \
                                     kd.stop0, kd.stop1, kd.ly, dg, tw_off, iktiles)
        const int ikid = ws.prof_begin(12 , (double)n + (double)nsort * (8.0 + sizeof(sav_t) + 1.0));
        switch (kp.g) { case 1: RV_IK_(1); break; case 2: RV_IK_(2); break; case 3: RV_IK_(3); break; case 4: RV_IK_(4); break; default: RV_IK_(5); break; }
        ws.prof_end(ikid);
#undef RV_IK_
    }
    SA_HIP(hipGetLastError());
    int in1 = 0;
    SA_TRY(rv_radix_sort_pairs<sav_t>(ws, bk0.as<u64>(), bv0.as<sav_t>(), bk1.as<u64>(), bv1.as<sav_t>(), nsort, 0, bits, &in1));
    s.radix_passes += rv_radix_passes(ws, bits); s.sorted_elems += nsort;
    u64 *ks = in1 ? bk1.as<u64>() : bk0.as<u64>();
    sav_t *vs = in1 ? bv1.as<sav_t>() : bv0.as<sav_t>();
    u64 *kt = in1 ? bk0.as<u64>() : bk1.as<u64>();
    sav_t *vt = in1 ? bv0.as<sav_t>() : bv1.as<sav_t>();

    uint8_t *head = bhead.as<uint8_t>();
    if (!collapse) SA_TRY(need_seed_grp(n));
    u32 *seed = bseed.as<u32>(), *grp = bgrp.as<u32>(), *ISA = bisa.as<u32>();
    const u64 *keys_by_rank = ks;
    const sav_t *vals_by_rank = vs;
    if (collapse) {
        const int64_t nb = ceil_div(nsort, TC_TILE);
        u32 *bc = ws.sa[23].as<u32>();
        hipLaunchKernelGGL(k_tw_flags, dim3((unsigned)nb), dim3(TB), 0, q, (const sav_t *)vs, nsort, bc);
        SA_HIP(hipGetLastError());
        SA_TRY(rv_exclusive_sum_u32(ws, bc, bc, nb));
        sav_t *vexp = reinterpret_cast<sav_t *>(bisa.p);
        if (sizeof(sav_t) > 4) { SA_TRY(ws.sa[24].reserve((size_t)n * sizeof(sav_t))); vexp = ws.sa[24].as<sav_t>(); }
        const int pbid = ws.prof_begin(13 , (double)nsort * 2.0 * (8.0 + sizeof(sav_t)) + (double)n * (1.0 + sizeof(sa_t) + sizeof(lcp_t) + 1.0));
        hipLaunchKernelGGL(k_heads_publish_tc, dim3((unsigned)nb), dim3(TB), 0, q, (const u64 *)ks, (const sav_t *)vs, nsort, (const u32 *)bc, head, LCP, SA, BWT,
                           side_sep, kd, d_maxlcp, ws.opt.no_pub_twins ? 0 : 1, kt, vexp);
        ws.prof_end(pbid);
        SA_HIP(hipGetLastError());
        keys_by_rank = kt; vals_by_rank = vexp;
    } else if (fused && kd.ly.nd_bits > 0 && !ws.opt.no_heads_fusion) {
        hipLaunchKernelGGL(k_heads_publish, dim3((unsigned)ceil_div(n, (int64_t)HP_ITEMS * TB)), dim3(TB), 0, q, (const u64 *)ks, (const sav_t *)vs, n, head, seed, LCP, SA, BWT, side_sep, kd, d_maxlcp,
                           ws.opt.no_pub_twins ? 0 : 1);
        SA_HIP(hipGetLastError());
        SA_TRY(rv_inclusive_max_u32(ws, seed, grp, n));
    } else {
        hipLaunchKernelGGL(k_heads, dim3(nblk), dim3(TB), 0, q, (const u64 *)ks, n, head, seed, fused ? LCP : (lcp_t *)nullptr, kd, fused ? d_maxlcp : (u32 *)nullptr);
        SA_HIP(hipGetLastError());
// ... 260 lines not shown
```

reveal_amd/csrc/rv_index.h:

```cpp
#pragma once
#include "rv_common.h"
#include "rv_scan.h"
#include "../../include/reveal_amd.h"
#include <utility>

struct RvIntv { int64_t begin, end; };

struct RvProf {
    bool on = false;
    u32 mask = 0xFFFFFFFFu;
    struct Span { hipEvent_t a, b; int k; double bytes; };
    std::vector<Span> spans;
    std::vector<hipEvent_t> pool;
    int64_t launches[RV_K_COUNT] = {0};
    double ms[RV_K_COUNT] = {0};
    double bytes[RV_K_COUNT] = {0};
    hipEvent_t get() {
        if (!pool.empty()) { hipEvent_t e = pool.back(); pool.pop_back(); return e; }
        hipEvent_t e = nullptr;
        (void)hipEventCreate(&e);
        return e;
    }
    int begin(hipStream_t s, int k, double nbytes) {
        if (!on || !((mask >> k) & 1u)) return -1;
// ... 62 lines not shown
            else (void)hipGetLastError();
        }
        if (!q) q = (char *)malloc(grow);
        if (!q) { rv_set_error("out of host memory for %zu bytes of text", grow); return -1; }
        if (n) memcpy(q, p, n);
        if (p) { if (pinned) (void)hipHostFree(p); else free(p); }
        p = q; cap = grow; pinned = pin;
        return 0;
    }
    int resize(size_t m) { if (reserve(m) != 0) return -1; n = m; return 0; }
    void push_back(char c) { if (resize(n + 1) == 0) p[n - 1] = c; }
    char *data() { return p; }
    const char *data() const { return p; }
    size_t size() const { return n; }
    char &operator[](size_t k) { return p[k]; }
    const char &operator[](size_t k) const { return p[k]; }
};

struct rv_index {
    int device = 0;
    Workspace ws;
    RvProf prof;
    HostText T;
    std::vector<int64_t> nsep;
    std::vector<int64_t> nsep_dev;
    std::vector<RvIntv> nodes;
    int nsamples = 0;
    int64_t n = 0, nT = 0;
    int rc = 0;
    bool constructed = false, main_arrays_freed = false;
    bool sai_valid = false;
    DBuf dT, dT0, dSA, dSAi, dLCP, dBWT, dNsep;
    bool text_dirty = true;
    bool text_only = false;
    HBuf hscan;
    HBuf hupload;
    hipEvent_t ev_picks = nullptr;
    size_t scan_guess = 4096;
    DBuf ps[7];
    u32 maxlcp = 0;
    RvSaStats sa_stats{};
    std::vector<u32> m_l; std::vector<int64_t> m_a, m_b;
    std::vector<u32> mm_l; std::vector<int32_t> mm_n; std::vector<int64_t> mm_off, mm_pos; std::vector<uint16_t> mm_so;
    struct Align *al = nullptr;
    struct RvBatchGroup *batch = nullptr;
    bool batch_settled = false;
    struct ResultBufs {
        uint32_t *l = nullptr; int64_t *off = nullptr, *pos = nullptr;
        int64_t l_cap = 0, off_cap = 0, pos_cap = 0;
        bool direct = false;
    } rb;
};

int rv_run_multi_pick(rv_index *h, const sa_t *SA, const lcp_t *LCP, const uint8_t *BWT, int64_t m, int minl, int minn,
                      const int64_t *d_sub_start, const int *d_sub_want, int nsubs, const int *d_tile_sub, std::vector<u32> &pick_l, std::vector<sa_t> &pick_pos,
                      int (*after_pick)(rv_index *) = nullptr, bool *redo = nullptr);
int rv_run_pair_scan(rv_index *h, const sa_t *SA, const lcp_t *LCP, const uint8_t *BWT, int64_t m, int minl, std::vector<RvPairRec> &out,
                     const u32 *d_err, u32 *err_out, const int64_t *d_sub_start, int nsubs,
                     int (*after_pick)(rv_index *), bool use_hook,
                     const int *d_tile_sub = nullptr,
                     const int64_t *d_presel_start = nullptr, int presel_subs = 0, int64_t presel = 0);

int rv_text_only(rv_index *h, u32 maxlcp);

int rv_need_sai(rv_index *h);

void rv_align_free(rv_index *h);
```

reveal_amd/csrc/rv_leaf.h:

```cpp
#pragma once
#include "rv_common.h"
#include "../../include/reveal_amd.h"

#ifndef RV_LEAF_N
#define RV_LEAF_N 2048
#endif

struct RvLeafRoot {
    int64_t off;
    int32_t n, depth;
    int64_t a0, a1, b0, b1;
};

struct RvLeafArgs {
    const RvLeafRoot *roots;
    const sa_t *SA; const lcp_t *LCP; const uint8_t *BWT;
    int64_t nsep0;
    int minl;
    u32 lcap;
    u32 stage_cap;
    u32 *anchor_count; u32 anchor_cap; u32 *anchor_l; int64_t *anchor_pos;
    unsigned long long *stats;
    int trace; u32 *trace_count; u32 trace_cap; rv_trace *trace_out;
    u32 *err;
};

int rv_leaf_launch(Workspace &ws, const RvLeafArgs &a, int nroots);
int rv_leaf_lower_launch(Workspace &ws, uint8_t *T, const int64_t *pos, const u32 *len, u32 na);
```

reveal_amd/csrc/rv_leaf.hip:

```cpp
#include "rv_common.h"
#include "rv_leaf.h"
#include <type_traits>

namespace {

constexpr int NT = 256;
constexpr int LN = RV_LEAF_N;
constexpr u32 INF = 0xFFFFFFFFu;
constexpr int NW = NT / 64;
constexpr int MAXSTACK = 128;
constexpr int ACAP = 256;

typedef std::make_unsigned<sa_t>::type usa_t;
struct Frame { int start, len, depth, buf; int64_t a0, a1, b0, b1; };

__device__ inline bool is_lower_c(uint8_t c) { return c >= 'a' && c <= 'z'; }
__device__ inline bool left_maximal(uint8_t ca, uint8_t cb) { return (ca != cb) || ca == 'N' || ca == '$' || is_lower_c(ca); }

__device__ inline u64 hash_step(u64 acc, u64 i, int64_t v) {
    u64 x = (u64)v + (i + 1) * 0x9E3779B97F4A7C15ULL;
    x ^= x >> 30; x *= 0xbf58476d1ce4e5b9ULL;
    x ^= x >> 27; x *= 0x94d049bb133111ebULL;
    x ^= x >> 31;
    return acc + x;
// ... 375 lines not shown
    for (int64_t j = (l & ~(int64_t)15) + h; j < l; j += 8) { const uint8_t ch = p[j]; if (ch >= 'A' && ch <= 'Z') p[j] = ch + 32; }
}
__global__ __launch_bounds__(NT) void k_leaf_lower_long(uint8_t *__restrict__ T, const int64_t *__restrict__ pos, const u32 *__restrict__ len, const u32 *__restrict__ lng) {
    const u32 cnt = lng[0] < LOWER_LONG_MAX ? lng[0] : LOWER_LONG_MAX;
    for (u32 k = 0; k < cnt; k++) {
        const u32 e = lng[4 + k];
        const int64_t l = (int64_t)len[e];
        for (int side = 0; side < 2; side++) {
            uint8_t *const p = T + pos[2 * (size_t)e + side];
            for (int64_t j0 = LOWER_CAP + (int64_t)blockIdx.x * (NT * 16); j0 < l; j0 += (int64_t)gridDim.x * (NT * 16)) {
                const int64_t j = j0 + (int64_t)threadIdx.x * 16;
                if (j + 16 <= l) {
                    u64 x[2];
                    __builtin_memcpy(x, p + j, 16);
                    x[0] = lower8(x[0]); x[1] = lower8(x[1]);
                    __builtin_memcpy(p + j, x, 16);
                } else {
                    for (int64_t i = j; i < l; i++) { const uint8_t ch = p[i]; if (ch >= 'A' && ch <= 'Z') p[i] = ch + 32; }
                }
            }
        }
    }
}

}

int rv_leaf_launch(Workspace &ws, const RvLeafArgs &a, int nroots) {
    if (nroots <= 0) return 0;
    hipLaunchKernelGGL(k_leaf, dim3((unsigned)nroots), dim3(NT), 0, ws.stream, a);
    RV_LAUNCH_CHECK();
    return 0;
}

int rv_leaf_lower_launch(Workspace &ws, uint8_t *T, const int64_t *pos, const u32 *len, u32 na) {
    if (na == 0) return 0;
    RV_TRY(ws.misc[15].reserve((size_t)(4 + LOWER_LONG_MAX) * 4));
    u32 *lng = ws.misc[15].as<u32>();
    RV_HIP(hipMemsetAsync(lng, 0, 16, ws.stream));
    hipLaunchKernelGGL(k_leaf_lower, dim3((unsigned)ceil_div((int64_t)na * 16, NT)), dim3(NT), 0, ws.stream, T, pos, len, na, lng);
    RV_LAUNCH_CHECK();
    hipLaunchKernelGGL(k_leaf_lower_long, dim3(1024), dim3(NT), 0, ws.stream, T, pos, len, (const u32 *)lng);
    RV_LAUNCH_CHECK();
    return 0;
}
```

reveal_amd/csrc/rv_many.hip:

```cpp
#include "rv_index.h"
#include "rv_leaf.h"
#include <algorithm>
#include <limits.h>
#include <new>
#include <stdexcept>

namespace {

constexpr int MT = 256;
constexpr int CAP_L = RV_LEAF_N;
constexpr int CAP_S = 512;
static_assert(CAP_L <= 2048, "local ranks are packed in 12 bits, positions in 16");

struct ManyDevJob { int64_t abeg, bbeg, off; int32_t la, lb; };

#define MANY_WSYNC() do { __builtin_amdgcn_fence(__ATOMIC_ACQ_REL, "workgroup"); __builtin_amdgcn_wave_barrier(); } while (0)

__device__ inline u32 many_wave_incl_max(u32 v) {
    const int lane = threadIdx.x & 63;
#define MANY_STEP_(CTRL, RM, TAKE) { const u32 o = rv_dpp_u32<CTRL, RM>(v); v = ((TAKE) && o > v) ? o : v; }
    RV_WAVE_SCAN_STEPS(MANY_STEP_)
#undef MANY_STEP_
    return v;
}
// ... 276 lines not shown
    if (nsmall < J) {
        hipLaunchKernelGGL((k_many_build<CAP_L, MT>), dim3((unsigned)(J - nsmall)), dim3(MT), 0, q, djobs + nsmall, (int)(J - nsmall), dT,
                           m->dSA.as<sa_t>(), m->dLCP.as<lcp_t>(), m->dBWT.as<uint8_t>(), d_max, d_err);
        RV_LAUNCH_CHECK();
        m->info[4]++;
    }
    u32 cnt[2] = {0, 0};
    RV_TRY(rv_read_back(h->ws, cnt, d_max, 8));
    if (cnt[1]) { rv_set_error("rv_many_run: the index build refused a job (error bits %u)", cnt[1]); return -1; }
    if (m->keep) {
        std::vector<sa_t> sa((size_t)n); std::vector<lcp_t> lc((size_t)n);
        RV_HIP(hipMemcpy(sa.data(), m->dSA.p, (size_t)n * sizeof(sa_t), hipMemcpyDeviceToHost));
        RV_HIP(hipMemcpy(lc.data(), m->dLCP.p, (size_t)n * sizeof(lcp_t), hipMemcpyDeviceToHost));
        const size_t base = m->keep_sa.size();
        m->keep_sa.resize(base + (size_t)n); m->keep_lcp.resize(base + (size_t)n);
        for (size_t s = 0; s < J; s++) {
            m->jobs[(size_t)ord[s]].arr_off = (int64_t)base + dj[s].off;
            for (int64_t r = 0; r < la[s] + lb[s] + 2; r++) {
                const int64_t p = (int64_t)sa[(size_t)(dj[s].off + r)];
                m->keep_sa[base + (size_t)(dj[s].off + r)] = (sa_t)(p >= bbeg[s] ? p - bbeg[s] + la[s] + 1 : p - abeg[s]);
                m->keep_lcp[base + (size_t)(dj[s].off + r)] = lc[(size_t)(dj[s].off + r)];
            }
        }
    }
    RV_TRY(rv_frontier_import(h, minl, minn, cnt[0], 0, (int)J, meta.data(), node_first.data(), nodes.data(), n, m->dSA.p, m->dLCP.p, m->dBWT.p, 1));
    rv_align_stats st;
    memset(&st, 0, sizeof st);
    RV_TRY(rv_align_builtin_resume(h, &st));
    many_add_stats(total, st);
    const size_t rec0 = m->recs.size();
    RV_TRY(many_collect(m, h, -1, ord, abeg, bbeg));
    m->info[4] += st.levels + (m->recs.size() > rec0 ? 2 : 0);
    std::vector<char> txt((size_t)n);
    RV_HIP(hipMemcpy(txt.data(), h->dT.p, (size_t)n, hipMemcpyDeviceToHost));
    for (size_t s = 0; s < J; s++) {
        ManyJob &jb = m->jobs[(size_t)ord[s]];
        jb.text_off = (int64_t)m->out_text.size();
        jb.shared = true;
        m->out_text.insert(m->out_text.end(), txt.begin() + (ptrdiff_t)abeg[s], txt.begin() + (ptrdiff_t)(abeg[s] + la[s] + 1));
        m->out_text.insert(m->out_text.end(), txt.begin() + (ptrdiff_t)bbeg[s], txt.begin() + (ptrdiff_t)(bbeg[s] + lb[s] + 1));
    }
    m->info[1] += (int64_t)J; m->info[3]++;
    return 0;
}

int many_ordinary(rv_many *m, int job, int minl, int minn, rv_align_stats *total) {
    RV_TRY(many_handle(m, &m->ho));
    rv_index *h = m->ho;
    ManyJob &jb = m->jobs[(size_t)job];
    RV_TRY(rv_reset(h));
    for (int s = 0; s < jb.k; s++) {
        RV_TRY(rv_add_sample(h));
        RV_TRY(rv_add_sequence(h, m->in.data() + m->starts[jb.seq0 + (size_t)s], m->lens[jb.seq0 + (size_t)s], nullptr, nullptr));
    }
    RV_TRY(rv_construct(h, 0, nullptr, nullptr, 0));
    rv_align_stats st;
    memset(&st, 0, sizeof st);
    RV_TRY(rv_align_builtin(h, minl, minn, &st));
    many_add_stats(total, st);
    static const std::vector<int> none; static const std::vector<int64_t> none64;
    RV_TRY(many_collect(m, h, job, none, none64, none64));
    jb.text_off = (int64_t)m->out_text.size();
    jb.shared = false;
    m->out_text.resize(m->out_text.size() + (size_t)jb.ranks);
    if (rv_get_array(h, RV_T, m->out_text.data() + jb.text_off, jb.ranks) != jb.ranks) return -1;
    m->info[2]++;
// ... 164 lines not shown
```

reveal_amd/csrc/rv_prims.hip:

```cpp
#include "rv_common.h"
#include <string.h>

namespace {

constexpr int SCAN_THREADS = 256;
constexpr int SCAN_ITEMS   = 8;
constexpr int SCAN_TILE    = SCAN_THREADS * SCAN_ITEMS;

template <class T> struct OpSum {
    __device__ static T id() { return (T)0; }
    __device__ static T f(T a, T b) { return a + b; }
};
template <class T> struct OpMax {
    __device__ static T id() { return (T)0; }
    __device__ static T f(T a, T b) { return a > b ? a : b; }
};

template <class T> __device__ inline T shfl_up_t(T v, int d) { return __shfl_up(v, d, 64); }
template <> __device__ inline u64 shfl_up_t<u64>(u64 v, int d) {
    u32 lo = __shfl_up((u32)v, d, 64), hi = __shfl_up((u32)(v >> 32), d, 64);
    return ((u64)hi << 32) | lo;
}

template <class T, class Op>
// ... 251 lines not shown
            const u32 d = (u32)(key[r] >> shift) & dmask;
            const u32 li = (u32)dstart[d] + (u32)cnt[w][d] + rnk[r];
            skey[li] = key[r];
            sval[li] = val[r];
        }
    }
    __syncthreads();
    const int64_t tbase = (int64_t)tile * RS_TILE;
    const u32 nvalid = (u32)((n - tbase) < (int64_t)RS_TILE ? (n - tbase) : (int64_t)RS_TILE);
    for (u32 li = threadIdx.x; li < nvalid; li += RS_THREADS) {
        const u64 k = skey[li];
        const u32 d = (u32)(k >> shift) & dmask;
        const size_t dst = (size_t)gbase[d] + (li - (u32)dstart[d]);
        kout[dst] = k;
        vout[dst] = sval[li];
        if (dnext) dnext[dst] = (uint8_t)((u32)(k >> nshift) & nmask);
    }
}

template <class V, int BITS, bool XCD, class CNT>
static void rs_scatter_launch(hipStream_t q, u32 nb, const u64 *ki, const V *vi, u64 *ko, V *vo, int64_t n, int shift, u32 dmask, const u32 *bh,
                              uint8_t *dnext, int nshift, u32 nmask) {
    const u32 grid = XCD ? RS_XCDS * ((nb + RS_XCDS - 1) / RS_XCDS) : nb;
    hipLaunchKernelGGL((k_rs_scatter<V, BITS, XCD, CNT>), dim3(grid), dim3(RS_THREADS), 0, q, ki, vi, ko, vo, n, shift, dmask, bh, nb, dnext, nshift, nmask);
}

}

int rv_radix_passes(const Workspace &ws, int nbits) {
    const int w = ws.opt.rs_bits == 10 ? 10 : 8;
    return nbits <= 0 ? 0 : (nbits + w - 1) / w;
}

template <class V>
int rv_radix_sort_pairs(Workspace &ws, u64 *k0, V *v0, u64 *k1, V *v1, int64_t n, int bit_lo, int bit_hi, int *result_in_1) {
    *result_in_1 = 0;
    if (n <= 1 || bit_hi <= bit_lo) return 0;
    if (n >= ((int64_t)1 << 32)) { rv_set_error("radix sort: n >= 2^32 not supported"); return -1; }
    const int width = ws.opt.rs_bits == 10 ? 10 : 8;
    const bool xcd = ws.opt.rs_xcd != 0, c16 = ws.opt.rs_cnt16 != 0;
    const u32 nb = (u32)ceil_div(n, RS_TILE);
    RV_TRY(ws.rs_hist.reserve(((size_t)1 << width) * nb * sizeof(u32)));
    u32 *bh = ws.rs_hist.as<u32>();
    const bool bytes = width == 8 && !ws.opt.rs_no_digit_bytes && n >= ((int64_t)1 << 20) && bit_hi - bit_lo > width;
    if (bytes) RV_TRY(ws.rs_digits.reserve((size_t)n + 64));
    uint8_t *dig = bytes ? ws.rs_digits.as<uint8_t>() : nullptr;
    bool have_digits = false;
    u64 *ki = k0, *ko = k1;
    V *vi = v0, *vo = v1;
    int flip = 0;
    for (int shift = bit_lo; shift < bit_hi; shift += width) {
        const int wbits = bit_hi - shift < width ? bit_hi - shift : width;
        const u32 dmask = (1u << wbits) - 1u;
        int pid = ws.prof_begin(8 , (have_digits ? 1.0 : 8.0) * (double)n);
        const u32 hgrid = xcd ? RS_XCDS * ((nb + RS_XCDS - 1) / RS_XCDS) : nb;
        if (have_digits) {
            if (xcd) hipLaunchKernelGGL((k_rs_hist_bytes<true>), dim3(hgrid), dim3(RS_THREADS), 0, ws.stream, (const uint8_t *)dig, n, bh, nb);
            else hipLaunchKernelGGL((k_rs_hist_bytes<false>), dim3(hgrid), dim3(RS_THREADS), 0, ws.stream, (const uint8_t *)dig, n, bh, nb);
        } else if (width == 10) { if (xcd) hipLaunchKernelGGL((k_rs_hist<10, true>), dim3(hgrid), dim3(RS_THREADS), 0, ws.stream, (const u64 *)ki, n, shift, dmask, bh, nb);
                           else hipLaunchKernelGGL((k_rs_hist<10, false>), dim3(hgrid), dim3(RS_THREADS), 0, ws.stream, (const u64 *)ki, n, shift, dmask, bh, nb); }
        else             { if (xcd) hipLaunchKernelGGL((k_rs_hist<8, true>), dim3(hgrid), dim3(RS_THREADS), 0, ws.stream, (const u64 *)ki, n, shift, dmask, bh, nb);
                           else hipLaunchKernelGGL((k_rs_hist<8, false>), dim3(hgrid), dim3(RS_THREADS), 0, ws.stream, (const u64 *)ki, n, shift, dmask, bh, nb); }
        RV_LAUNCH_CHECK();
        ws.prof_end(pid);
        RV_TRY(rv_exclusive_sum_u32(ws, bh, bh, ((int64_t)1 << width) * nb));
        const int nshift = shift + width;
        const bool more = nshift < bit_hi;
        const u32 nmask = more ? ((1u << (bit_hi - nshift < width ? bit_hi - nshift : width)) - 1u) : 0u;
        uint8_t *dn = (bytes && more) ? dig : nullptr;
        pid = ws.prof_begin(7 , (2.0 * (8.0 + sizeof(V)) + (dn ? 1.0 : 0.0)) * (double)n);
#define RS_GO(B_, X_, C_) rs_scatter_launch<V, B_, X_, C_>(ws.stream, nb, (const u64 *)ki, (const V *)vi, ko, vo, n, shift, dmask, (const u32 *)bh, dn, nshift, nmask)
        if (width == 10) { if (xcd) { if (c16) RS_GO(10, true, uint16_t); else RS_GO(10, true, u32); } else { if (c16) RS_GO(10, false, uint16_t); else RS_GO(10, false, u32); } }
        else             { if (xcd) { if (c16) RS_GO(8, true, uint16_t); else RS_GO(8, true, u32); } else { if (c16) RS_GO(8, false, uint16_t); else RS_GO(8, false, u32); } }
#undef RS_GO
        RV_LAUNCH_CHECK();
        ws.prof_end(pid);
        have_digits = dn != nullptr;
        u64 *tk = ki; ki = ko; ko = tk;
        V *tv = vi; vi = vo; vo = tv;
        flip ^= 1;
    }
    *result_in_1 = flip;
    return 0;
}

__global__ __launch_bounds__(256) void k_h2d_copy(const uint4 *__restrict__ src, uint4 *__restrict__ dst, size_t n16) {
    for (size_t i = (size_t)blockIdx.x * 256 + threadIdx.x; i < n16; i += (size_t)gridDim.x * 256) dst[i] = src[i];
}
int rv_read_back(Workspace &ws, void *dst, const void *dsrc, size_t bytes) {
    RV_TRY(ws.hpin.reserve(bytes < 4096 ? 4096 : bytes));
    if (!ws.ev_rb) RV_HIP(hipEventCreateWithFlags(&ws.ev_rb, hipEventDisableTiming));
    RV_HIP(hipMemcpyAsync(ws.hpin.p, dsrc, bytes, hipMemcpyDeviceToHost, ws.stream));
    RV_HIP(hipEventRecord(ws.ev_rb, ws.stream));
    const hipError_t e = rv_event_wait(ws.ev_rb);
    if (e != hipSuccess) { rv_set_error("rv_read_back: %s", hipGetErrorString(e)); return -1; }
    memcpy(dst, ws.hpin.p, bytes);
    return 0;
}

int rv_h2d_copy(Workspace &ws, const void *pinned_src, void *dst, size_t bytes) {
    const size_t n16 = (bytes + 15) / 16;
    if (n16 == 0) return 0;
    size_t blocks = (n16 + 255) / 256;
    if (blocks > 512) blocks = 512;
    hipLaunchKernelGGL(k_h2d_copy, dim3((unsigned)blocks), dim3(256), 0, ws.stream, (const uint4 *)pinned_src, (uint4 *)dst, n16);
    RV_LAUNCH_CHECK();
    return 0;
}

template int rv_radix_sort_pairs<u32>(Workspace &, u64 *, u32 *, u64 *, u32 *, int64_t, int, int, int *);
template int rv_radix_sort_pairs<u64>(Workspace &, u64 *, u64 *, u64 *, u64 *, int64_t, int, int, int *);
```

Measured before the change: 22450.

## Stream cascade anchor tail, defer text copy, and emit first radix digits in key init

Several independent changes land together. The device text copy (dT from dT0) is made lazy through rv_need_text, with an event for cross-stream ordering, and SA/LCP/BWT construction reads dT0 directly. For two-genome runs, the cascade streams finished anchor chunks to host result buffers and lowers them on a side stream while it is still running, so less tail work remains at the end. The key-init kernel also writes the first radix digit bytes, which lets the first sort pass skip a full key read for its histogram. The cost is added stream/event coordination and correctness risk around text staleness and partially streamed results.

```diff
diff --git a/include/reveal_amd.h b/include/reveal_amd.h
--- a/include/reveal_amd.h
+++ b/include/reveal_amd.h
@@ -88,6 +88,7 @@
 int rv_frontier_seeds_import(rv_index *h, int nsubs, const int64_t *words, int64_t nwords);
 uint32_t rv_maxlcp(const rv_index *h);
 int rv_cascade_info(const rv_index *h, int64_t *out);
+int64_t rv_cascade_streamed(const rv_index *h);
 const char *rv_cascade_why(const rv_index *h);
 int64_t rv_anchor_count(rv_index *h, int64_t *members);
 int rv_fetch_anchors(rv_index *h, uint32_t *l, int64_t *off, int64_t *pos);
diff --git a/reveal_amd/_index.py b/reveal_amd/_index.py
--- a/reveal_amd/_index.py
+++ b/reveal_amd/_index.py
@@ -600,6 +600,7 @@
             o = np.zeros(8, dtype=np.int64)
             self._dll.rv_cascade_info(self._h, o.ctypes.data)
             return dict(done=bool(o[0]), levels=int(o[1]), matches=int(o[2]), witnesses=int(o[3]), subindices=int(o[4]), undecided=int(o[5]), rebuilt_ranks=int(o[6]), decided_from_witnesses=int(o[7]),
+                        streamed=int(self._dll.rv_cascade_streamed(self._h)),
                         why=(self._dll.rv_cascade_why(self._h) or b"").decode())
 
         def align_builtin_until(self, stop_subs, minl=20, minn=2, trace=False):
diff --git a/reveal_amd/_lib.py b/reveal_amd/_lib.py
--- a/reveal_amd/_lib.py
+++ b/reveal_amd/_lib.py
@@ -79,6 +79,7 @@
     "rv_maxlcp": (ctypes.c_uint32, [V]),
     "rv_cascade_info": (ctypes.c_int, [V, V]),
     "rv_cascade_why": (ctypes.c_char_p, [V]),
+    "rv_cascade_streamed": (ctypes.c_int64, [V]),
     "rv_anchor_count": (_L, [V, c_i64p]),
     "rv_fetch_anchors": (_I, [V, V, V, V]),
     "rv_set_result_buffers": (_I, [V, V, _L, V, _L, V, _L]),
diff --git a/reveal_amd/csrc/rv_align.hip b/reveal_amd/csrc/rv_align.hip
--- a/reveal_amd/csrc/rv_align.hip
+++ b/reveal_amd/csrc/rv_align.hip
@@ -140,6 +140,8 @@
     DBuf dD, dTab, dTile, dList, dFlag, dPar, dDbg, scrSA, scrLCP, scrBWT;
     RvCascadeBufs cas;
     RvCascadeOut cas_out{};
+    u32 cas_streamed_last = 0;
+    u32 cas_streamed = 0;
     DBuf dPbReady; u32 pb_epoch = 0;
     DBuf dNextTsub;
     DBuf dTmin;
@@ -597,6 +599,7 @@
     const bool all_classes = a->multi || ns > 4096;
     if (biggest <= a->par_min_cur && !h->ws.opt.no_early_bubble &&
         (a->multi || (!h->ws.opt.bubble_lds_always && (!all_classes || h->ws.opt.early_bubble_many)))) {
+        RV_TRY(rv_need_text(h, h->ws.stream));
         RV_TRY(rv_lower_ranges_launch(h->ws, h->dT.as<uint8_t>(), t.mb, t.me, W * ns));
         RV_TRY(bubble_flags(h, m));
         RvBubbleArgs ba;
@@ -1252,6 +1255,7 @@
     }
     h->prof.end(q, id);
     if (!a->early_bubble) {
+        RV_TRY(rv_need_text(h, h->ws.stream));
         if (lt.nmatch > 256 && a->mpre.back() / lt.nmatch <= 512) RV_TRY(rv_lower_ranges_launch(h->ws, h->dT.as<uint8_t>(), lt.mbegin, lt.mend, lt.nmatch));
         else RV_TRY(rv_lower_launch(h->ws, h->dT.as<uint8_t>(), lt.mbegin, lt.mend, (const int64_t *)(tb + cm.o_mpre), lt.nmatch, a->mpre.back()));
     }
@@ -1816,6 +1820,7 @@
         RV_TRY(a->hLeafOut.reserve(256));
         RV_HIP(hipMemcpyAsync(a->hLeafOut.p, lf_counters, 128, hipMemcpyDeviceToHost, q));
         RV_HIP(hipStreamSynchronize(q));
+        h->text_stream = nullptr;
         u32 cnt[4]; unsigned long long stv[8];
         memcpy(cnt, a->hLeafOut.p, sizeof cnt); memcpy(stv, a->hLeafOut.as<uint8_t>() + 64, sizeof stv);
         if (h->ws.opt.leaf_prof)
@@ -1828,13 +1833,17 @@
             const size_t nl = a->an_l.size(), np = a->an_pos.size();
             rv_index::ResultBufs &rb = h->rb;
             rb.direct = rb.l && (int64_t)(nl + na) <= rb.l_cap && (int64_t)(nl + na + 1) <= rb.off_cap && (int64_t)(np + 2 * na) <= rb.pos_cap;
+            const size_t done = std::min<size_t>(a->cas_streamed, na), from = rb.direct ? done : 0;
             int64_t *pp; u32 *pl;
             if (rb.direct) { pp = rb.pos + np; pl = rb.l + nl; }
             else { RV_TRY(a->hLeafOut.reserve(na * 20 + 64)); pp = a->hLeafOut.as<int64_t>(); pl = (u32 *)(pp + 2 * na); }
-            RV_HIP(hipMemcpyAsync(pp, lf_pos, na * 16, hipMemcpyDeviceToHost, a->leaf_stream));
-            RV_HIP(hipMemcpyAsync(pl, lf_l, na * 4, hipMemcpyDeviceToHost, a->leaf_stream));
-            RV_TRY(rv_leaf_lower_launch(h->ws, h->dT.as<uint8_t>(), lf_pos, lf_l, (u32)na));
-            if (rb.direct) fill_offsets(rb.off + nl + 1, na, (int64_t)np);
+            if (na > from) {
+                RV_HIP(hipMemcpyAsync(pp + 2 * from, lf_pos + 2 * from, (na - from) * 16, hipMemcpyDeviceToHost, a->leaf_stream));
+                RV_HIP(hipMemcpyAsync(pl + from, lf_l + from, (na - from) * 4, hipMemcpyDeviceToHost, a->leaf_stream));
+            }
+            RV_TRY(rv_need_text(h, q));
+            RV_TRY(rv_leaf_lower_launch(h->ws, h->dT.as<uint8_t>(), lf_pos + 2 * done, lf_l + done, (u32)(na - done)));
+            if (rb.direct) fill_offsets(rb.off + nl + 1 + from, na - from, (int64_t)(np + 2 * from));
             RV_HIP(hipStreamSynchronize(a->leaf_stream));
             RV_HIP(hipStreamSynchronize(q));
             a->leaf_na = na;
@@ -1848,8 +1857,35 @@
         if ((int64_t)stv[3] > a->st.maxdepth) a->st.maxdepth = (int32_t)stv[3];
     }
     a->running = false;
+    a->cas_streamed_last = a->cas_streamed;
+    a->cas_streamed = 0;
     if (out) *out = a->st;
     return 0;
+}
+
+static int cascade_tail_chunk(rv_index *h, u32 from, u32 to) {
+    Align *a = h->al;
+    const rv_index::ResultBufs &rb = h->rb;
+    const size_t nl = a->an_l.size(), np = a->an_pos.size();
+    if (!rb.l || (int64_t)(nl + to) > rb.l_cap || (int64_t)(nl + to + 1) > rb.off_cap || (int64_t)(np + 2 * (size_t)to) > rb.pos_cap) return 0;
+    hipStream_t side = a->leaf_stream;
+    RV_HIP(hipMemcpyAsync(rb.pos + np + 2 * (size_t)from, a->lf_pos + 2 * (size_t)from, (size_t)(to - from) * 16, hipMemcpyDeviceToHost, side));
+    RV_HIP(hipMemcpyAsync(rb.l + nl + from, a->lf_l + from, (size_t)(to - from) * 4, hipMemcpyDeviceToHost, side));
+    RV_TRY(rv_need_text(h, side));
+    RV_TRY(rv_leaf_lower_launch(h->ws, h->dT.as<uint8_t>(), a->lf_pos + 2 * (size_t)from, a->lf_l + from, to - from, side));
+    a->cas_streamed = to;
+    return 1;
+}
+static void cascade_tail_host(rv_index *h, u32 from, u32 to) {
+    Align *a = h->al;
+    fill_offsets(h->rb.off + a->an_l.size() + 1 + from, to - from, (int64_t)(a->an_pos.size() + 2 * (size_t)from));
+}
+static void cascade_tail_cancel(rv_index *h) {
+    Align *a = h->al;
+    if (!a->cas_streamed) return;
+    (void)hipStreamSynchronize(a->leaf_stream);
+    h->text_stale = true; h->text_stream = nullptr;
+    a->cas_streamed = 0;
 }
 
 static int install_frontier(rv_index *h, int level, int nsubs, const int64_t *meta, const int64_t *node_first, const int64_t *nodes, int64_t m,
@@ -1896,11 +1932,15 @@
     io.stats = a->lf_stats; io.leaf_err = a->lf_counters + 2;
     io.stage_cap = (u32)h->ws.opt.leaf_acap;
     io.lvSA = &a->lvSA[0]; io.lvLCP = &a->lvLCP[0]; io.lvBWT = &a->lvBWT[0]; io.roots = &a->dLeafRoots[0];
+    RvCascadeTail tail;
+    tail.side = a->leaf_stream;
+    if (h->nodes.size() == 2) { tail.chunk = cascade_tail_chunk; tail.host = cascade_tail_host; tail.cancel = cascade_tail_cancel; }
+    a->cas_streamed = 0;
     const int dmode = (int)h->ws.opt.cascade_danger;
-    RV_TRY(rv_cascade_run(h, a->cas, io, a->minl, &a->cas_out, dmode == 2 ? 1 : 0, 0));
+    RV_TRY(rv_cascade_run(h, a->cas, io, a->minl, &a->cas_out, dmode == 2 ? 1 : 0, 0, &tail));
     if (!a->cas_out.done && a->cas_out.undecided > 0 && dmode == 1) {
         RV_HIP(hipMemsetAsync(a->dLeaf.p, 0, 256, h->ws.stream));
-        RV_TRY(rv_cascade_run(h, a->cas, io, a->minl, &a->cas_out, 1, 1));
+        RV_TRY(rv_cascade_run(h, a->cas, io, a->minl, &a->cas_out, 1, 1, &tail));
     }
     if (!a->cas_out.done) {
         RV_HIP(hipMemsetAsync(a->dLeaf.p, 0, 256, h->ws.stream));
@@ -1937,6 +1977,8 @@
     out[0] = c.done ? 1 : 0; out[1] = c.levels; out[2] = c.cands; out[3] = c.witnesses; out[4] = c.children; out[5] = c.undecided; out[6] = c.rebuilt_ranks; out[7] = c.solved;
     return 0;
 }
+
+int64_t rv_cascade_streamed(const rv_index *h) { return h->al ? (int64_t)h->al->cas_streamed_last : 0; }
 
 const char *rv_cascade_why(const rv_index *h) {
     if (!h->al || h->al->cas_out.done || !h->al->cas_out.why) return "";
diff --git a/reveal_amd/csrc/rv_api.hip b/reveal_amd/csrc/rv_api.hip
--- a/reveal_amd/csrc/rv_api.hip
+++ b/reveal_amd/csrc/rv_api.hip
@@ -90,6 +90,7 @@
     (void)rv_set_result_buffers(h, nullptr, 0, nullptr, 0, nullptr, 0);
     rv_align_free(h);
     h->prof.release();
+    if (h->ev_text) { (void)hipEventDestroy(h->ev_text); h->ev_text = nullptr; }
     h->dT.release(); h->dT0.release(); h->dSA.release(); h->dSAi.release(); h->dLCP.release(); h->dBWT.release(); h->dNsep.release();
     h->ws.release();
     h->hscan.release();
@@ -152,7 +153,8 @@
     ok = ok && c->dT.reserve((size_t)n + 64) == 0 && c->dSA.reserve((size_t)(n + 64) * sizeof(sa_t)) == 0 && c->dSAi.reserve((size_t)(n + 64) * sizeof(sa_t)) == 0
             && c->dLCP.reserve((size_t)(n + 64) * sizeof(lcp_t)) == 0 && c->dBWT.reserve((size_t)n + 64) == 0 && c->dNsep.reserve((h->nsep.size() + 1) * sizeof(sa_t)) == 0;
     ok = ok && hipStreamSynchronize(h->ws.stream) == hipSuccess;
-    ok = ok && hipMemcpyAsync(c->dT.p, h->dT.p, (size_t)n + 64, hipMemcpyDeviceToDevice, q) == hipSuccess;
+    c->text_stale = h->text_stale;
+    if (!h->text_stale) ok = ok && hipMemcpyAsync(c->dT.p, h->dT.p, (size_t)n + 64, hipMemcpyDeviceToDevice, q) == hipSuccess;
     ok = ok && hipMemcpyAsync(c->dSA.p, h->dSA.p, (size_t)n * sizeof(sa_t), hipMemcpyDeviceToDevice, q) == hipSuccess;
     ok = ok && hipMemcpyAsync(c->dSAi.p, h->dSAi.p, (size_t)n * sizeof(sa_t), hipMemcpyDeviceToDevice, q) == hipSuccess;
     ok = ok && hipMemcpyAsync(c->dLCP.p, h->dLCP.p, (size_t)n * sizeof(lcp_t), hipMemcpyDeviceToDevice, q) == hipSuccess;
@@ -415,7 +417,7 @@
     hipStream_t q = h->ws.stream;
     RV_TRY(rv_upload(h));
     RV_TRY(h->dT.reserve((size_t)n + 64));
-    RV_HIP(hipMemcpyAsync(h->dT.p, h->dT0.p, (size_t)n + 64, hipMemcpyDeviceToDevice, q));
+    h->text_stale = true; h->text_stream = nullptr;
     RV_TRY(h->dSA.reserve((size_t)(n + 64) * sizeof(sa_t)));
     RV_TRY(h->dSAi.reserve((size_t)(n + 64) * sizeof(sa_t)));
     RV_TRY(h->dLCP.reserve((size_t)(n + 64) * sizeof(lcp_t)));
@@ -429,8 +431,8 @@
     SaScratchInUse in_use(h->ws);
     if (!safile || !safile[0]) {
         int id = h->prof.begin(q, RV_K_SA_SORT, 5.0 * (double)n);
-        if (lcp_from_file) RV_TRY(rv_build_sa(h->ws, h->dT.as<uint8_t>(), n, h->dSA.as<sa_t>(), &h->sa_stats));
-        else RV_TRY(rv_build_sa(h->ws, h->dT.as<uint8_t>(), n, h->dSA.as<sa_t>(), &h->sa_stats, h->dLCP.as<lcp_t>(), h->dBWT.as<uint8_t>(), side_sep, d_max, &lcp_done,
+        if (lcp_from_file) RV_TRY(rv_build_sa(h->ws, h->dT0.as<uint8_t>(), n, h->dSA.as<sa_t>(), &h->sa_stats));
+        else RV_TRY(rv_build_sa(h->ws, h->dT0.as<uint8_t>(), n, h->dSA.as<sa_t>(), &h->sa_stats, h->dLCP.as<lcp_t>(), h->dBWT.as<uint8_t>(), side_sep, d_max, &lcp_done,
                                  h->nsep.data(), (int)h->nsep.size()));
         h->prof.end(q, id);
     } else {
@@ -444,7 +446,7 @@
     if (!lcp_from_file) {
         if (!lcp_done) {
             int id = h->prof.begin(q, RV_K_LCP, 13.0 * (double)n);
-            RV_TRY(rv_build_lcp(h->ws, h->dT.as<uint8_t>(), h->dSA.as<sa_t>(), false, h->dLCP.as<lcp_t>(), n, d_max, h->dBWT.as<uint8_t>(), side_sep));
+            RV_TRY(rv_build_lcp(h->ws, h->dT0.as<uint8_t>(), h->dSA.as<sa_t>(), false, h->dLCP.as<lcp_t>(), n, d_max, h->dBWT.as<uint8_t>(), side_sep));
             h->prof.end(q, id);
         }
         RV_TRY(rv_read_back(h->ws, &h->maxlcp, d_max, 4));
@@ -455,7 +457,7 @@
         for (int64_t i = 0; i < n; i++) if ((u32)tmp[(size_t)i] > mx) mx = (u32)tmp[(size_t)i];
         h->maxlcp = mx;
         RV_HIP(hipMemcpyAsync(h->dLCP.p, tmp.data(), (size_t)n * sizeof(lcp_t), hipMemcpyHostToDevice, q));
-        RV_TRY(rv_build_bwt(h->ws, h->dT.as<uint8_t>(), h->dSA.as<sa_t>(), n, h->dBWT.as<uint8_t>(), side_sep));
+        RV_TRY(rv_build_bwt(h->ws, h->dT0.as<uint8_t>(), h->dSA.as<sa_t>(), n, h->dBWT.as<uint8_t>(), side_sep));
         RV_HIP(hipStreamSynchronize(q));
     }
     if (cache == 1) {
@@ -488,6 +490,7 @@
     case RV_T:
         if (cap < n) { rv_set_error("buffer too small"); return -1; }
         if (h->constructed || h->text_only) {
+            if (rv_need_text(h, h->ws.stream) != 0 || hipStreamSynchronize(h->ws.stream) != hipSuccess) { rv_set_error("D2H failed"); return -1; }
             if (hipMemcpy(out, h->dT.p, (size_t)n, hipMemcpyDeviceToHost) != hipSuccess) { rv_set_error("D2H failed"); return -1; }
         } else {
             memcpy(out, h->T.data(), (size_t)n);
@@ -531,6 +534,19 @@
 
 }
 
+int rv_need_text(rv_index *h, hipStream_t stream) {
+    if (h->text_stale) {
+        RV_TRY(h->dT.reserve((size_t)h->n + 64));
+        if (!h->ev_text) RV_HIP(hipEventCreateWithFlags(&h->ev_text, hipEventDisableTiming));
+        RV_HIP(hipMemcpyAsync(h->dT.p, h->dT0.p, (size_t)h->n + 64, hipMemcpyDeviceToDevice, stream));
+        RV_HIP(hipEventRecord(h->ev_text, stream));
+        h->text_stale = false; h->text_stream = stream;
+    } else if (h->text_stream && stream != h->text_stream) {
+        RV_HIP(hipStreamWaitEvent(stream, h->ev_text, 0));
+    }
+    return 0;
+}
+
 int rv_need_sai(rv_index *h) {
     if (h->sai_valid) return 0;
     if (!h->constructed || h->main_arrays_freed) { rv_set_error("the inverse suffix array was not requested before align() consumed the main index"); return -1; }
@@ -549,7 +565,7 @@
     h->rc = 0; h->nT = n;
     RV_TRY(rv_upload(h));
     RV_TRY(h->dT.reserve((size_t)n + 64));
-    RV_HIP(hipMemcpyAsync(h->dT.p, h->dT0.p, (size_t)n + 64, hipMemcpyDeviceToDevice, q));
+    h->text_stale = true; h->text_stream = nullptr;
     RV_TRY(h->dSAi.reserve((size_t)(n + 64) * sizeof(sa_t)));
     std::vector<sa_t> ns(h->nsep.size() + 1, 0);
     for (size_t k = 0; k < h->nsep.size(); k++) ns[k] = (sa_t)h->nsep[k];
diff --git a/reveal_amd/csrc/rv_cascade.h b/reveal_amd/csrc/rv_cascade.h
--- a/reveal_amd/csrc/rv_cascade.h
+++ b/reveal_amd/csrc/rv_cascade.h
@@ -10,11 +10,13 @@
     int64_t lin_steps = 0; int lin_maxdepth = 0; size_t lin_off[6] = {0, 0, 0, 0, 0, 0};
     std::vector<int64_t> lin_rest; int lin_rest_depth = 0;
     hipStream_t prio_stream = nullptr; hipEvent_t ev_in = nullptr, ev_out = nullptr;
+    hipEvent_t ev_levels = nullptr;
     void release() {
         for (auto &b : d) b.release(); hstage.release(); hstage2.release();
         if (prio_stream) { (void)hipStreamDestroy(prio_stream); prio_stream = nullptr; }
         if (ev_in) { (void)hipEventDestroy(ev_in); ev_in = nullptr; }
         if (ev_out) { (void)hipEventDestroy(ev_out); ev_out = nullptr; }
+        if (ev_levels) { (void)hipEventDestroy(ev_levels); ev_levels = nullptr; }
     }
 };
 
@@ -24,6 +26,14 @@
     u32 *leaf_err;
     u32 stage_cap;
     DBuf *lvSA, *lvLCP, *lvBWT, *roots;
+};
+
+struct rv_index;
+struct RvCascadeTail {
+    hipStream_t side = nullptr;
+    int (*chunk)(rv_index *h, u32 from, u32 to) = nullptr;
+    void (*host)(rv_index *h, u32 from, u32 to) = nullptr;
+    void (*cancel)(rv_index *h) = nullptr;
 };
 
 struct RvCascadeOut {
@@ -51,4 +61,4 @@
 void rv_batch_group_free(RvBatchGroup *g);
 void rv_batch_group_info(const RvBatchGroup *g, int64_t *out);
 int rv_cascade_multi_run(rv_index *h, RvCascadeBufs &cb, int minl, RvCascadeMultiOut *out);
-int rv_cascade_run(rv_index *h, RvCascadeBufs &cb, const RvCascadeIO &io, int minl, RvCascadeOut *out, int danger = 0, int reuse = 0);
+int rv_cascade_run(rv_index *h, RvCascadeBufs &cb, const RvCascadeIO &io, int minl, RvCascadeOut *out, int danger = 0, int reuse = 0, const RvCascadeTail *tail = nullptr);
diff --git a/reveal_amd/csrc/rv_cascade.hip b/reveal_amd/csrc/rv_cascade.hip
--- a/reveal_amd/csrc/rv_cascade.hip
+++ b/reveal_amd/csrc/rv_cascade.hip
@@ -20,7 +20,8 @@
 
 struct CasIv { sa_t a0, a1, b0, b1; };
 struct CasRes { sa_t qa, qb; u32 ql, lead, trail, state; };
-enum { C_NCHILD = 0, C_NUND = 1, C_NWIT = 2, C_ERR = 3, C_MAXN = 4, C_LO = 5, C_HI = 6, C_LEVELS = 7, C_NSOLVED = 8, C_NUNSOLVED = 9, C_NRETRY = 10, C_TICKET = 11 };
+enum { C_NCHILD = 0, C_NUND = 1, C_NWIT = 2, C_ERR = 3, C_MAXN = 4, C_LO = 5, C_HI = 6, C_LEVELS = 7, C_NSOLVED = 8, C_NUNSOLVED = 9, C_NRETRY = 10, C_TICKET = 11,
+       C_NANCH = 12 };
 
 __device__ inline bool cas_cut(const CasIv &iv, int64_t pa, int64_t pb, int64_t len, int64_t minl, int64_t *qa, int64_t *qb, int64_t *ql) {
     const int64_t ka = (int64_t)iv.a0 - pa, kb = (int64_t)iv.b0 - pb;
@@ -588,6 +589,7 @@
         if (atomicAdd(&counters[C_TICKET], 1u) == gridDim.x - 1) {
             if (hi > lo) counters[C_LEVELS]++;
             counters[C_LO] = hi; counters[C_HI] = atomicAdd(&counters[C_NCHILD], 0u);
+            counters[C_NANCH] = atomicAdd(io.anchor_count, 0u);
             counters[C_TICKET] = 0;
         }
     }
@@ -841,7 +843,7 @@
     return 0;
 }
 
-int rv_cascade_run(rv_index *h, RvCascadeBufs &cb, const RvCascadeIO &io, int minl_in, RvCascadeOut *out, int danger, int reuse) {
+int rv_cascade_run(rv_index *h, RvCascadeBufs &cb, const RvCascadeIO &io, int minl_in, RvCascadeOut *out, int danger, int reuse, const RvCascadeTail *tail) {
     memset(out, 0, sizeof *out);
     out->done = false;
     Workspace &ws = h->ws;
@@ -1069,6 +1071,21 @@
         ws.stream = cb.prio_stream; prio.on = true;
         q = cb.prio_stream;
     }
+    if (tail && tail->side && h->text_stale) {
+        if (!cb.ev_levels) RV_HIP(hipEventCreateWithFlags(&cb.ev_levels, hipEventDisableTiming));
+        RV_HIP(hipEventRecord(cb.ev_levels, q));
+        RV_HIP(hipStreamWaitEvent(tail->side, cb.ev_levels, 0));
+        RV_TRY(rv_need_text(h, tail->side));
+    }
+    constexpr u32 TAIL_MIN = 2048;
+    struct TailScope {
+        rv_index *h; const RvCascadeTail *t; bool keep = false;
+        ~TailScope() { if (t && t->cancel && !keep) t->cancel(h); }
+    } tscope{h, tail};
+    bool streaming = tail && tail->chunk;
+    u32 streamed = 0, pend_from = 0, pend_to = 0;
+    const int give_up_after = (int)ws.opt.cascade_give_up_after;
+    bool hook_gave_up = false;
     for (;;) {
         for (int b = 0; b < batch; b++, queued++) {
             hipLaunchKernelGGL(k_cas_assign, dim3(agrid), dim3(TB), 0, q, (const sa_t *)bpa.as<sa_t>(), (const sa_t *)bpb.as<sa_t>(), (const u32 *)blen.as<u32>(), bcc.as<u32>(), M,
@@ -1100,12 +1117,24 @@
                                bres.as<CasRes>(), minl, counters, ccap, bund.as<u32>(), (u32)RV_LEAF_N, io, dg, (danger && NW) ? 1 : 0);
             RV_LAUNCH_CHECK();
         }
+        if (pend_to > pend_from) {
+            const int r = tail->chunk(h, pend_from, pend_to);
+            if (r < 0) return -1;
+            if (r == 0) streaming = false;
+            else if (tail->host) tail->host(h, pend_from, pend_to);
+            pend_from = pend_to;
+        }
         RV_TRY(rv_read_back(ws, hc, counters, sizeof hc));
         if (hc[C_ERR] & ~5u) { rv_set_error("cascade: device error %u", hc[C_ERR]); return -1; }
         if (hc[C_ERR]) GIVE_UP("the cascade's tables are full");
+        if (give_up_after > 0 && (int)hc[C_LEVELS] >= give_up_after) { hook_gave_up = true; break; }
         if (hc[C_MAXN] > (u32)RV_LEAF_N) break;
         if (hc[C_HI] == hc[C_LO]) break;
         if (queued > 1000000) { rv_set_error("cascade: no progress"); return -1; }
+        if (streaming) {
+            const u32 to = std::min(hc[C_NANCH], io.anchor_cap);
+            if (to >= streamed + TAIL_MIN) { pend_from = streamed; pend_to = to; streamed = to; }
+        }
     }
     prio.leave(); q = ws.stream;
     const int level = (int)hc[C_LEVELS];
@@ -1114,6 +1143,7 @@
     out->levels = level; out->children = hi; out->solved = hc[C_NSOLVED]; out->unsolved = hc[C_NUNSOLVED];
     const u32 U = hc[C_NUND];
     out->undecided = U;
+    if (hook_gave_up) { out->why = "RV_CASCADE_GIVE_UP_AFTER"; return 0; }
     if (hc[C_MAXN] > (u32)RV_LEAF_N) {
         out->why = "an undecided sub-index above the leaf kernel's size";
         if (verbose) fprintf(stderr, "cascade%s: gave up: %s (%u ranks; %u levels, %u sub-indices, %u undecided, %u decided from witnesses, %u not)\n", danger ? " (second attempt)" : "", out->why, hc[C_MAXN], level, hi, U, hc[C_NSOLVED], hc[C_NUNSOLVED]);
@@ -1165,6 +1195,7 @@
                 danger ? " (second attempt)" : "", M, NW, level, hi, U, (long long)out->rebuilt_ranks, (long long)out->solved, (tp[1] - tp[0]) * 1e3, (tp[2] - tp[1]) * 1e3, (tp[3] - tp[2]) * 1e3, (tp[4] - tp[3]) * 1e3);
     }
     out->done = true;
+    tscope.keep = true;
     return 0;
 #undef GIVE_UP
 }
diff --git a/reveal_amd/csrc/rv_cascade_multi.hip b/reveal_amd/csrc/rv_cascade_multi.hip
--- a/reveal_amd/csrc/rv_cascade_multi.hip
+++ b/reveal_amd/csrc/rv_cascade_multi.hip
@@ -1235,6 +1235,7 @@
     RvBatchJob bjob;
     if (h->batch && !h->batch_settled) {
         h->batch_settled = true; ticket.settled = true;
+        RV_TRY(rv_need_text(h, q));
         bjob.k = k; bjob.minl = minl; bjob.M = M; bjob.NW = std::min(NW, wcap); bjob.ccap = ccap; bjob.acap = acap;
         bjob.c_len = bcl.as<u32>(); bjob.c_pos = bcp.as<sa_t>(); bjob.w_pos = bwp.as<sa_t>(); bjob.w_val = bwv.as<u32>();
         bjob.nsep = nsep; bjob.dT = h->dT.as<uint8_t>();
@@ -1339,6 +1340,7 @@
         RV_TRY(bexp.reserve((size_t)NA * k * 4));
         hipLaunchKernelGGL(k_casm_expand_l, dim3((unsigned)ceil_div((int64_t)NA * k, TB)), dim3(TB), 0, q, (const u32 *)banl.as<u32>(), NA, k, bexp.as<u32>());
         RV_LAUNCH_CHECK();
+        RV_TRY(rv_need_text(h, q));
         hipLaunchKernelGGL(k_casm_lower, dim3((unsigned)ceil_div((int64_t)NA * k * 64, TB)), dim3(TB), 0, q, h->dT.as<uint8_t>(), (const u32 *)bexp.as<u32>(), (const sa_t *)banp.as<sa_t>(), NA * (u32)k);
         RV_LAUNCH_CHECK();
     }
@@ -1440,6 +1442,7 @@
                     RV_TRY(bcl0.reserve((size_t)NA * k * 4));
                     hipLaunchKernelGGL(k_casm_expand_l, dim3((unsigned)ceil_div((int64_t)NA * k, TB)), dim3(TB), 0, q, d_anl, NA, k, bcl0.as<u32>());
                     RV_LAUNCH_CHECK();
+                    RV_TRY(rv_need_text(h, q));
                     hipLaunchKernelGGL(k_casm_unlower, dim3((unsigned)ceil_div((int64_t)NA * k * 64, TB)), dim3(TB), 0, q, h->dT.as<uint8_t>(), (const uint8_t *)h->dT0.as<uint8_t>(),
                                        (const u32 *)bcl0.as<u32>(), d_anp, NA * (u32)k);
                     RV_LAUNCH_CHECK();
diff --git a/reveal_amd/csrc/rv_common.h b/reveal_amd/csrc/rv_common.h
--- a/reveal_amd/csrc/rv_common.h
+++ b/reveal_amd/csrc/rv_common.h
@@ -97,7 +97,8 @@
     X(presel_dev_min, "RV_PRESEL_DEV_MIN", 65536) \
     X(scan_v1, "RV_SCAN_V1", 0) \
     X(pick_threads, "RV_PICK_THREADS", 0) \
-    X(cascade_prio, "RV_CASCADE_PRIO", 0)
+    X(cascade_prio, "RV_CASCADE_PRIO", 0) \
+    X(cascade_give_up_after, "RV_CASCADE_GIVE_UP_AFTER", 0)
 struct RvOptions {
 #define RV_X_(f, name, def) int64_t f = def;
     RV_OPTION_LIST(RV_X_)
@@ -331,7 +332,8 @@
 int rv_radix_passes(const Workspace &ws, int nbits);
 template <class V>
 int rv_radix_sort_pairs(Workspace &ws, u64 *k0, V *v0, u64 *k1, V *v1, int64_t n,
-                        int bit_lo, int bit_hi, int *result_in_1);
+                        int bit_lo, int bit_hi, int *result_in_1, bool first_digits = false);
+bool rv_radix_digit_bytes(const Workspace &ws, int64_t n, int bit_lo, int bit_hi);
 
 int rv_read_back(Workspace &ws, void *dst, const void *dsrc, size_t bytes);
 
diff --git a/reveal_amd/csrc/rv_construct.hip b/reveal_amd/csrc/rv_construct.hip
--- a/reveal_amd/csrc/rv_construct.hip
+++ b/reveal_amd/csrc/rv_construct.hip
@@ -355,7 +355,8 @@
 template <int G>
 __global__ __launch_bounds__(TB) void k_init_keys(const uint8_t *__restrict__ T, int64_t n, const uint8_t *__restrict__ lut, int K, KeyPack kp,
                                                   u64 *__restrict__ keys, sav_t *__restrict__ vals, int pay, u32 stop0, u32 stop1,
-                                                  KeyLayout ly, DiagBits dg, const u32 *__restrict__ tw_off , int64_t ntiles) {
+                                                  KeyLayout ly, DiagBits dg, const u32 *__restrict__ tw_off , int64_t ntiles,
+                                                  uint8_t *__restrict__ dig0 ) {
     __shared__ u32 code32[IK_WORDS + 2];
     __shared__ u32 s_sc[IK_WORDS / 8 + 3];
     __shared__ uint8_t slut[256], sstop[256];
@@ -483,6 +484,7 @@
                 key |= (u64)(known ? (u32)d | ((f >> 1) << ly.nd_bits) : (u32)nd_none) << ly.nd_shift;
             }
             keys[obase + j] = key; vals[obase + j] = (sav_t)i;
+            if (dig0) dig0[obase + j] = (uint8_t)key;
         }
     } else {
     constexpr int PER = KEY_TILE / TB;
@@ -535,9 +537,10 @@
                 ulonglong2 *vd2 = reinterpret_cast<ulonglong2 *>(vals + i0);
                 vd2[0] = make_ulonglong2((u64)oval[0], (u64)oval[1]); vd2[1] = make_ulonglong2((u64)oval[2], (u64)oval[3]);
             }
+            if (dig0) *reinterpret_cast<u32 *>(dig0 + i0) = ((u32)okey[0] & 0xffu) | (((u32)okey[1] & 0xffu) << 8) | (((u32)okey[2] & 0xffu) << 16) | ((u32)okey[3] << 24);
         } else {
 #pragma unroll
-            for (int r = 0; r < PER; r++) if (i0 + r < n) { keys[i0 + r] = okey[r]; vals[i0 + r] = oval[r]; }
+            for (int r = 0; r < PER; r++) if (i0 + r < n) { keys[i0 + r] = okey[r]; vals[i0 + r] = oval[r]; if (dig0) dig0[i0 + r] = (uint8_t)okey[r]; }
         }
     } else {
 #pragma unroll
@@ -547,10 +550,11 @@
             if (i >= n) continue;
             const int xw = k >> 6, b = k & 63;
             const bool twin = (s_tw[xw] >> b) & 1ull;
-            if (i < dg.D) { keys[i] = okey[r]; vals[i] = (sav_t)i | (twin ? TW_FLAG : (sav_t)0); }
+            if (i < dg.D) { keys[i] = okey[r]; vals[i] = (sav_t)i | (twin ? TW_FLAG : (sav_t)0); if (dig0) dig0[i] = (uint8_t)okey[r]; }
             else if (!twin) {
                 const int64_t o = dg.D + (int64_t)tw_off[tile] + s_kpre[xw] + (u32)__popcll(s_keep[xw] & ((b == 0) ? 0ull : (~0ull >> (64 - b))));
                 keys[o] = okey[r]; vals[o] = (sav_t)i;
+                if (dig0) dig0[o] = (uint8_t)okey[r];
             }
         }
     }
@@ -2327,19 +2331,23 @@
         tw_off = tc;
         s.diag_table = dg.tab;
     }
+    bool first_digits = false;
     {
         const int64_t iktiles = ceil_div(n, KEY_TILE);
         const dim3 ig((unsigned)std::min<int64_t>(iktiles, 256 * 8));
+        first_digits = rv_radix_digit_bytes(ws, nsort, 0, bits);
+        if (first_digits) SA_TRY(ws.rs_digits.reserve((size_t)nsort + 64));
+        uint8_t *dig0 = first_digits ? ws.rs_digits.as<uint8_t>() : nullptr;
 #define RV_IK_(G) hipLaunchKernelGGL(k_init_keys<G>, ig, dim3(TB), 0, q, T, n, d_lut.as<uint8_t>(), K, kp, bk0.as<u64>(), bv0.as<sav_t>(), fused ? 1 : 0, \
-                                     kd.stop0, kd.stop1, kd.ly, dg, tw_off, iktiles)
-        const int ikid = ws.prof_begin(12 , (double)n + (double)nsort * (8.0 + sizeof(sav_t) + 1.0));
+                                     kd.stop0, kd.stop1, kd.ly, dg, tw_off, iktiles, dig0)
+        const int ikid = ws.prof_begin(12 , (double)n + (double)nsort * (8.0 + sizeof(sav_t) + 1.0 + (dig0 ? 1.0 : 0.0)));
         switch (kp.g) { case 1: RV_IK_(1); break; case 2: RV_IK_(2); break; case 3: RV_IK_(3); break; case 4: RV_IK_(4); break; default: RV_IK_(5); break; }
         ws.prof_end(ikid);
 #undef RV_IK_
     }
     SA_HIP(hipGetLastError());
     int in1 = 0;
-    SA_TRY(rv_radix_sort_pairs<sav_t>(ws, bk0.as<u64>(), bv0.as<sav_t>(), bk1.as<u64>(), bv1.as<sav_t>(), nsort, 0, bits, &in1));
+    SA_TRY(rv_radix_sort_pairs<sav_t>(ws, bk0.as<u64>(), bv0.as<sav_t>(), bk1.as<u64>(), bv1.as<sav_t>(), nsort, 0, bits, &in1, first_digits));
     s.radix_passes += rv_radix_passes(ws, bits); s.sorted_elems += nsort;
     u64 *ks = in1 ? bk1.as<u64>() : bk0.as<u64>();
     sav_t *vs = in1 ? bv1.as<sav_t>() : bv0.as<sav_t>();
diff --git a/reveal_amd/csrc/rv_index.h b/reveal_amd/csrc/rv_index.h
--- a/reveal_amd/csrc/rv_index.h
+++ b/reveal_amd/csrc/rv_index.h
@@ -118,6 +118,9 @@
     bool sai_valid = false;
     DBuf dT, dT0, dSA, dSAi, dLCP, dBWT, dNsep;
     bool text_dirty = true;
+    bool text_stale = false;
+    hipStream_t text_stream = nullptr;
+    hipEvent_t ev_text = nullptr;
     bool text_only = false;
     HBuf hscan;
     HBuf hupload;
@@ -149,6 +152,8 @@
 
 int rv_text_only(rv_index *h, u32 maxlcp);
 
+int rv_need_text(rv_index *h, hipStream_t stream);
+
 int rv_need_sai(rv_index *h);
 
 void rv_align_free(rv_index *h);
diff --git a/reveal_amd/csrc/rv_leaf.h b/reveal_amd/csrc/rv_leaf.h
--- a/reveal_amd/csrc/rv_leaf.h
+++ b/reveal_amd/csrc/rv_leaf.h
@@ -26,4 +26,4 @@
 };
 
 int rv_leaf_launch(Workspace &ws, const RvLeafArgs &a, int nroots);
-int rv_leaf_lower_launch(Workspace &ws, uint8_t *T, const int64_t *pos, const u32 *len, u32 na);
+int rv_leaf_lower_launch(Workspace &ws, uint8_t *T, const int64_t *pos, const u32 *len, u32 na, hipStream_t st = nullptr);
diff --git a/reveal_amd/csrc/rv_leaf.hip b/reveal_amd/csrc/rv_leaf.hip
--- a/reveal_amd/csrc/rv_leaf.hip
+++ b/reveal_amd/csrc/rv_leaf.hip
@@ -431,14 +431,15 @@
     return 0;
 }
 
-int rv_leaf_lower_launch(Workspace &ws, uint8_t *T, const int64_t *pos, const u32 *len, u32 na) {
+int rv_leaf_lower_launch(Workspace &ws, uint8_t *T, const int64_t *pos, const u32 *len, u32 na, hipStream_t st) {
     if (na == 0) return 0;
+    if (!st) st = ws.stream;
     RV_TRY(ws.misc[15].reserve((size_t)(4 + LOWER_LONG_MAX) * 4));
     u32 *lng = ws.misc[15].as<u32>();
-    RV_HIP(hipMemsetAsync(lng, 0, 16, ws.stream));
-    hipLaunchKernelGGL(k_leaf_lower, dim3((unsigned)ceil_div((int64_t)na * 16, NT)), dim3(NT), 0, ws.stream, T, pos, len, na, lng);
+    RV_HIP(hipMemsetAsync(lng, 0, 16, st));
+    hipLaunchKernelGGL(k_leaf_lower, dim3((unsigned)ceil_div((int64_t)na * 16, NT)), dim3(NT), 0, st, T, pos, len, na, lng);
     RV_LAUNCH_CHECK();
-    hipLaunchKernelGGL(k_leaf_lower_long, dim3(1024), dim3(NT), 0, ws.stream, T, pos, len, (const u32 *)lng);
+    hipLaunchKernelGGL(k_leaf_lower_long, dim3(1024), dim3(NT), 0, st, T, pos, len, (const u32 *)lng);
     RV_LAUNCH_CHECK();
     return 0;
 }
diff --git a/reveal_amd/csrc/rv_many.hip b/reveal_amd/csrc/rv_many.hip
--- a/reveal_amd/csrc/rv_many.hip
+++ b/reveal_amd/csrc/rv_many.hip
@@ -332,6 +332,8 @@
     RV_TRY(many_collect(m, h, -1, ord, abeg, bbeg));
     m->info[4] += st.levels + (m->recs.size() > rec0 ? 2 : 0);
     std::vector<char> txt((size_t)n);
+    RV_TRY(rv_need_text(h, h->ws.stream));
+    RV_HIP(hipStreamSynchronize(h->ws.stream));
     RV_HIP(hipMemcpy(txt.data(), h->dT.p, (size_t)n, hipMemcpyDeviceToHost));
     for (size_t s = 0; s < J; s++) {
         ManyJob &jb = m->jobs[(size_t)ord[s]];
diff --git a/reveal_amd/csrc/rv_prims.hip b/reveal_amd/csrc/rv_prims.hip
--- a/reveal_amd/csrc/rv_prims.hip
+++ b/reveal_amd/csrc/rv_prims.hip
@@ -307,8 +307,13 @@
     return nbits <= 0 ? 0 : (nbits + w - 1) / w;
 }
 
+bool rv_radix_digit_bytes(const Workspace &ws, int64_t n, int bit_lo, int bit_hi) {
+    const int width = ws.opt.rs_bits == 10 ? 10 : 8;
+    return width == 8 && !ws.opt.rs_no_digit_bytes && n >= ((int64_t)1 << 20) && n < ((int64_t)1 << 32) && bit_hi - bit_lo > width;
+}
+
 template <class V>
-int rv_radix_sort_pairs(Workspace &ws, u64 *k0, V *v0, u64 *k1, V *v1, int64_t n, int bit_lo, int bit_hi, int *result_in_1) {
+int rv_radix_sort_pairs(Workspace &ws, u64 *k0, V *v0, u64 *k1, V *v1, int64_t n, int bit_lo, int bit_hi, int *result_in_1, bool first_digits) {
     *result_in_1 = 0;
     if (n <= 1 || bit_hi <= bit_lo) return 0;
     if (n >= ((int64_t)1 << 32)) { rv_set_error("radix sort: n >= 2^32 not supported"); return -1; }
@@ -317,10 +322,11 @@
     const u32 nb = (u32)ceil_div(n, RS_TILE);
     RV_TRY(ws.rs_hist.reserve(((size_t)1 << width) * nb * sizeof(u32)));
     u32 *bh = ws.rs_hist.as<u32>();
-    const bool bytes = width == 8 && !ws.opt.rs_no_digit_bytes && n >= ((int64_t)1 << 20) && bit_hi - bit_lo > width;
+    const bool bytes = rv_radix_digit_bytes(ws, n, bit_lo, bit_hi);
+    if (first_digits && !bytes) { rv_set_error("radix sort: first-pass digits given to a sort that reads none"); return -1; }
     if (bytes) RV_TRY(ws.rs_digits.reserve((size_t)n + 64));
     uint8_t *dig = bytes ? ws.rs_digits.as<uint8_t>() : nullptr;
-    bool have_digits = false;
+    bool have_digits = first_digits;
     u64 *ki = k0, *ko = k1;
     V *vi = v0, *vo = v1;
     int flip = 0;
@@ -383,5 +389,5 @@
     return 0;
 }
 
-template int rv_radix_sort_pairs<u32>(Workspace &, u64 *, u32 *, u64 *, u32 *, int64_t, int, int, int *);
-template int rv_radix_sort_pairs<u64>(Workspace &, u64 *, u64 *, u64 *, u64 *, int64_t, int, int, int *);
+template int rv_radix_sort_pairs<u32>(Workspace &, u64 *, u32 *, u64 *, u32 *, int64_t, int, int, int *, bool);
+template int rv_radix_sort_pairs<u64>(Workspace &, u64 *, u64 *, u64 *, u64 *, int64_t, int, int, int *, bool);
```

Result: no change. 22950, median of 3 (+2.2%).
